# TrevorS/voxtral-mini-realtime-rs

Hardware: AMD Instinct MI355X
Metric: decode_tok_per_s (higher is better)
Workload: dtype f32

## Files before the change

### include/voxtral_hip.h

```cpp
#ifndef VOXTRAL_HIP_H
#define VOXTRAL_HIP_H

#include <stddef.h>
#include <stdint.h>

#ifdef __cplusplus
extern "C" {
#endif

#define VOX_OK 0
#define VOX_ERR_INVALID 1
#define VOX_ERR_IO 2
#define VOX_ERR_HIP 3
#define VOX_ERR_NOTFOUND 4
#define VOX_ERR_UNSUPPORTED 5

#define VOX_MEM_HOST 0
#define VOX_MEM_DEVICE 1

typedef struct vox_ctx vox_ctx;
typedef struct vox_gguf vox_gguf;
typedef struct vox_q4 vox_q4;
typedef struct vox_model vox_model;
typedef struct vox_cache vox_cache;
typedef struct vox_graph vox_graph;

const char* vox_last_error(void);
int32_t vox_abi_version(void);
int32_t vox_device_count(int32_t* n);

int32_t vox_ctx_create(int32_t device, vox_ctx** out);
int32_t vox_ctx_destroy(vox_ctx* ctx);
int32_t vox_ctx_synchronize(vox_ctx* ctx);
int32_t vox_ctx_set_shared(vox_ctx* ctx, int32_t shared);
int32_t vox_ctx_stream(vox_ctx* ctx, void** hip_stream_out);
int32_t vox_dev_alloc(vox_ctx* ctx, size_t nbytes, void** out);
int32_t vox_dev_free(vox_ctx* ctx, void* p);
int32_t vox_dev_upload(vox_ctx* ctx, void* dst_dev, const void* src_host, size_t nbytes);
int32_t vox_dev_download(vox_ctx* ctx, void* dst_host, const void* src_dev, size_t nbytes);
int32_t vox_dev_copy(vox_ctx* ctx, void* dst_dev, const void* src_dev, size_t nbytes);

int32_t vox_resample_len(size_t n_in, uint32_t sr_in, uint32_t sr_out, size_t* n_out);
int32_t vox_resample(vox_ctx* ctx, const float* in, size_t n_in, uint32_t sr_in, uint32_t sr_out, float* out, size_t cap, size_t* n_out,
                     int32_t mem_kind);
int32_t vox_resample_plan(uint32_t sr_in, uint32_t sr_out, int32_t* fft_in, int32_t* fft_out, int32_t* delay, float* cutoff, float* taps_or_null, size_t cap);
int32_t vox_peak_normalize(float* samples, size_t n, float target_peak);

typedef struct {
    uint32_t sample_rate;
    uint32_t n_left_pad_tokens;
    float    frame_rate;
    uint32_t extra_right_pad_tokens;
} vox_pad_cfg;
int32_t vox_pad_cfg_voxtral(vox_pad_cfg* cfg);
int32_t vox_pad_len(size_t n, const vox_pad_cfg* cfg, size_t* out);
int32_t vox_pad_audio(const float* in, size_t n, const vox_pad_cfg* cfg, float* out);
int32_t vox_num_audio_tokens(size_t n, const vox_pad_cfg* cfg, size_t* out);

typedef struct {
    uint32_t max_mel_frames;
    uint32_t hop_length;
    uint32_t sample_rate;
    uint32_t overlap_frames;
} vox_chunk_cfg;
typedef struct { size_t start_sample, end_sample, index; int32_t is_last; } vox_chunk;
int32_t vox_needs_chunking(size_t n, const vox_chunk_cfg* cfg, int32_t* out);
int32_t vox_chunk_plan(size_t n, const vox_chunk_cfg* cfg, vox_chunk* out, size_t cap, size_t* n_chunks);

int32_t vox_mel_num_frames(size_t n_samples, size_t* out);
int32_t vox_mel_filterbank(float* out_128x201);
int32_t vox_hann_window(int32_t length, float* out);
int32_t vox_mel_compute_log(vox_ctx* ctx, const float* samples, size_t n, float* out_Tx128, int32_t mem_kind);

int32_t vox_time_embedding(float t, int32_t dim, float* out);

int32_t vox_gguf_open(const char* path, vox_gguf** out);
int32_t vox_gguf_open_memory(const void* data, size_t size, vox_gguf** out);
int32_t vox_gguf_open_shards(const void* const* shards, const size_t* sizes, int32_t n, vox_gguf** out);
int32_t vox_gguf_close(vox_gguf* g);
int32_t vox_gguf_version(const vox_gguf* g, uint32_t* out);
int32_t vox_gguf_tensor_count(const vox_gguf* g, uint64_t* out);
int32_t vox_gguf_tensor_name(const vox_gguf* g, uint64_t index, const char** out);
int32_t vox_gguf_tensor_info(const vox_gguf* g, const char* name, uint64_t dims[4], uint32_t* ndims,
                             uint32_t* dtype, uint64_t* nbytes);
int32_t vox_gguf_tensor_data(const vox_gguf* g, const char* name, void* dst, size_t cap);

int32_t vox_q4_tensor_from_bytes(vox_ctx* ctx, const uint8_t* raw, size_t nbytes, int64_t N, int64_t K, vox_q4** out);
int32_t vox_q4_tensor_shape(const vox_q4* q, int64_t* N, int64_t* K);
int32_t vox_q4_tensor_num_blocks(const vox_q4* q, int64_t* out);
int32_t vox_q4_tensor_dequantize(vox_ctx* ctx, const vox_q4* q, float* out_NxK);
int32_t vox_q4_tensor_free(vox_q4* q);
int32_t vox_q4_matmul(vox_ctx* ctx, const vox_q4* w, const float* x, int32_t B, int32_t M, float* out, int32_t mem_kind);
int32_t vox_q4_linear_forward(vox_ctx* ctx, const vox_q4* w, const float* bias_or_null, const float* x,
                              int32_t B, int32_t M, float* out, int32_t mem_kind);

int32_t vox_dense_tensor_from_f32(vox_ctx* ctx, const float* w_NxK, const float* w_other_or_null, int64_t N, int64_t K, vox_q4** out);
int32_t vox_linear_forward_ex(vox_ctx* ctx, const vox_q4* w, const float* bias_or_null, const float* x, int32_t B, int32_t M, float* out, int32_t epilogue, int32_t mem_kind);
int32_t vox_conv_downsample(vox_ctx* ctx, const float* x_CxL, int32_t C, int32_t L, const float* w1, const float* b1, const float* w2, const float* b2, int32_t O, float* out_OxL2);

typedef struct {
    int32_t enc_layers, enc_dim, enc_heads, enc_head_dim, enc_ffn, enc_window;
    int32_t dec_layers, dec_dim, dec_heads, dec_kv_heads, dec_head_dim, dec_ffn, dec_window, vocab;
    int32_t n_mels, reshape_factor, t_cond_dim;
    float rope_theta, norm_eps;
} vox_model_cfg;

int32_t vox_attention(vox_ctx* ctx, const float* q, const float* k, const float* v, int32_t M, int32_t kv_len, int32_t n_heads,
                      int32_t n_kv_heads, int32_t head_dim, int32_t offset, int32_t window, float* out, int32_t mem_kind);

int32_t vox_q4_model_load(vox_ctx* ctx, const char* gguf_path, vox_model** out);
#define VOX_LOAD_LAYOUT_ONLY 1u
int32_t vox_q4_model_load_ex(vox_ctx* ctx, const char* gguf_path, uint32_t flags, vox_model** out);
int32_t vox_q4_model_load_gguf(vox_ctx* ctx, vox_gguf* g, uint32_t flags, vox_model** out);
int32_t vox_f32_model_load(vox_ctx* ctx, const char* safetensors_path, vox_model** out);
int32_t vox_model_free(vox_model* m);
int32_t vox_model_config(const vox_model* m, vox_model_cfg* out);
int32_t vox_model_weight_bytes(const vox_model* m, uint64_t* out);
int32_t vox_model_arena(const vox_model* m, void** dev_ptr, uint64_t* nbytes);
int32_t vox_model_arena_finalize(vox_model* m);
int32_t vox_model_replicate(const vox_model* src, vox_ctx* dst_ctx, vox_model** out);
int32_t vox_model_memory(const vox_model* m, uint64_t out[4]);

int32_t vox_model_set_t_embed(vox_model* m, const float* t_embed_host);
int32_t vox_model_set_decode_engine(vox_model* m, int32_t on, int32_t* active_or_null);
int32_t vox_model_set_prefix_cache(vox_model* m, int32_t on, int32_t* active_or_null);
int32_t vox_model_prefix_info(const vox_model* m, int32_t out[4]);
int32_t vox_model_set_batch_engine(vox_model* m, int32_t on, int32_t* active_or_null, uint64_t* launches_or_null);

int32_t vox_encode_audio(vox_model* m, const float* mel_128xT, int32_t T, float* out, int32_t cap_rows,
                         int32_t* S, int32_t mem_kind);
int32_t vox_transcribe_streaming(vox_model* m, const float* mel_128xT, int32_t T, const float* t_embed,
                                 int32_t* out_ids, int32_t cap, int32_t* n_ids, float* logits_or_null,
                                 int32_t mem_kind);
int32_t vox_transcribe_audio(vox_model* m, const float* samples, size_t n, const float* t_embed,
                             int32_t* out_ids, int32_t cap, int32_t* n_ids, int32_t mem_kind);

int32_t vox_transcribe_batch(vox_model* m, int32_t n, const float* const* samples, const size_t* n_samples, const float* t_embed,
                             int32_t* const* out_ids, const int32_t* caps, int32_t* n_ids, int32_t mem_kind);
int32_t vox_transcribe_batch_ex(vox_model* m, int32_t n, const float* const* samples, const size_t* n_samples, const int32_t* norm_group_or_null, const float* t_embed,
                                int32_t* const* out_ids, const int32_t* caps, int32_t* n_ids, int32_t mem_kind);
int32_t vox_model_set_sessions(vox_model* m, int32_t sessions);

int32_t vox_decoder_cache_create(vox_model* m, int32_t max_seq, vox_cache** out);
int32_t vox_cache_free(vox_cache* c);
int32_t vox_cache_seq_len(const vox_cache* c, int32_t* out);
int32_t vox_cache_reset(vox_cache* c);
int32_t vox_cache_update(vox_cache* c, int32_t layer, int32_t pos, const float* k_HxNxhd, const float* v_HxNxhd, int32_t n_rows, int32_t mem_kind);
int32_t vox_cache_truncate(vox_cache* c, int32_t len);
int32_t vox_encoder_cache_create(vox_model* m, int32_t capacity_rows, vox_cache** out);
int32_t vox_encoder_cache_apply_sliding_window(vox_cache* enc_cache, int32_t window);
int32_t vox_cache_abs_pos(const vox_cache* c, int32_t* out);
int32_t vox_encode_audio_with_cache(vox_model* m, const float* mel_128xT, int32_t T, vox_cache* enc_cache, float* out, int32_t cap_rows,
                                    int32_t* S, int32_t mem_kind);
int32_t vox_embed_tokens_from_ids(vox_model* m, const int32_t* ids, int32_t n, float* out_nxD);
int32_t vox_forward_hidden_with_cache(vox_model* m, const float* x_MxD, int32_t M, const float* t_embed,
                                      vox_cache* cache, float* out_MxD);
int32_t vox_lm_head(vox_model* m, const float* hidden_MxD, int32_t M, float* logits_MxV);
int32_t vox_embed_tokens_from_ids_ex(vox_model* m, const int32_t* ids_host, int32_t n, float* out_nxD, int32_t mem_kind);
int32_t vox_tensor_add(vox_ctx* ctx, const float* a, const float* b, size_t n, float* out, int32_t mem_kind);
int32_t vox_forward_hidden_with_cache_ex(vox_model* m, const float* x_MxD, int32_t M, const float* t_embed, vox_cache* cache, float* out_MxD_or_null,
                                         const float** hidden_ws_or_null, int32_t mem_kind);
int32_t vox_lm_head_ex(vox_model* m, const float* hidden_MxD, int32_t M, float* logits_MxV, int32_t mem_kind);
int32_t vox_argmax_rows(vox_ctx* ctx, const float* logits_MxV, int32_t M, int32_t V, int32_t* ids_host, int32_t mem_kind);
int32_t vox_lm_head_argmax(vox_model* m, const float* hidden_MxD, int32_t M, int32_t* ids_host, int32_t mem_kind);
int32_t vox_generate_step_with_cache(vox_model* m, const int32_t* token_ids, int32_t n, const float* t_embed, vox_cache* cache, float* logits_nxV);

int32_t vox_forward(vox_model* m, const float* mel_128xT, int32_t T, const float* t_embed, float* logits_SxV, int32_t cap_rows, int32_t* S, int32_t mem_kind);
int32_t vox_forward_streaming(vox_model* m, const float* mel_128xT, int32_t T, const int32_t* token_ids, int32_t n_ids, const float* t_embed, float* logits_SxV,
                              int32_t cap_rows, int32_t* S, int32_t mem_kind);
int32_t vox_forward_with_cache(vox_model* m, const float* mel_128xT, int32_t T, const float* t_embed, vox_cache* enc_cache, vox_cache* dec_cache, float* logits_SxV,
                               int32_t cap_rows, int32_t* S, int32_t mem_kind);

typedef struct { double preprocess_ms, encode_ms, decode_ms, total_ms; int32_t decode_tokens; int32_t graph_replays; } vox_timings;
int32_t vox_get_stage_timings(const vox_model* m, vox_timings* out);

int32_t vox_debug_reload_knobs(void);
int32_t vox_debug_attn_launches(uint64_t* out, int32_t cap);
int32_t vox_debug_gemm_launches(uint64_t* out, int32_t cap);
int32_t vox_debug_occupy(vox_ctx* ctx, int32_t workgroups, int32_t micros);

int32_t vox_bench_decode_gemv(vox_model* m, int32_t which, int32_t iters, double* avg_us, double* bytes_per_launch,
                              const char** kernel_name);

int32_t vox_bench_wide(vox_model* m, int32_t which, int32_t mt, int32_t iters, double out_us[4]);

int32_t vox_debug_timeline_start(vox_ctx* ctx, int32_t n_slots, int32_t n_waves);
int32_t vox_debug_timeline_fetch(vox_ctx* ctx, uint64_t* out, size_t cap_words, int32_t* slots_used, int32_t* meta );
int32_t vox_debug_batch_tap_arm(vox_model* m, const int32_t* units, int32_t n_units, int32_t max_rows);
int32_t vox_debug_batch_tap_fetch(vox_model* m, float* out, int32_t* rows_per_unit);
int32_t vox_debug_encode_batch(vox_model* m, int32_t n, const float* const* mels, const int32_t* T, int32_t layout, float* out, int64_t cap_rows,
                               int32_t* rows_per_clip, int64_t* report);
int32_t vox_debug_step_costs(const double base[9], const double meas[9], int32_t calib, int32_t shared, double out[9]);
int32_t vox_debug_plan_slots(const int32_t* steps, int32_t n, int32_t force_G, int32_t max_groups, const double step_ms[9], int32_t* G, int32_t* job_slot,
                             int32_t* job_qpos, int32_t steps_g[8], int32_t run_g[8], double* cost_ms);

typedef struct vox_stream vox_stream;
int32_t vox_stream_create(vox_model* m, const float* t_embed, float gain, int32_t enc_capacity_rows, int32_t max_positions, vox_stream** out);
int32_t vox_stream_push(vox_stream* s, const float* samples, size_t n, int32_t mem_kind, int32_t* out_ids, int32_t cap, int32_t* n_ids);
int32_t vox_stream_finish(vox_stream* s, int32_t* out_ids, int32_t cap, int32_t* n_ids);
int32_t vox_stream_reset(vox_stream* s);
int32_t vox_stream_free(vox_stream* s);
int32_t vox_stream_info(const vox_stream* s, int64_t out[8]);
int32_t vox_stream_schedule(size_t n_samples, int32_t finished, int32_t* positions, int32_t* ids);
int32_t vox_debug_stream_tap_arm(vox_stream* s, int32_t max_rows);
int32_t vox_debug_stream_tap_fetch(vox_stream* s, float* out_rows_x_vocab, int32_t* rows);

#ifdef __cplusplus
}
#endif
#endif
```

### voxtral-mini-realtime-rs_amd/_lib.py

```python
from __future__ import annotations

import ctypes as C
import os

from .build import LIB_PATH


class VoxError(RuntimeError):
    def __init__(self, code, msg):
        super().__init__(f"[vox error {code}] {msg}")
        self.code = code


class PadCfg(C.Structure):
    _fields_ = [("sample_rate", C.c_uint32), ("n_left_pad_tokens", C.c_uint32), ("frame_rate", C.c_float),
                ("extra_right_pad_tokens", C.c_uint32)]


class ChunkCfg(C.Structure):
    _fields_ = [("max_mel_frames", C.c_uint32), ("hop_length", C.c_uint32), ("sample_rate", C.c_uint32),
                ("overlap_frames", C.c_uint32)]


class Chunk(C.Structure):
    _fields_ = [("start_sample", C.c_size_t), ("end_sample", C.c_size_t), ("index", C.c_size_t), ("is_last", C.c_int32)]


class ModelCfg(C.Structure):
    _fields_ = [(n, C.c_int32) for n in ("enc_layers", "enc_dim", "enc_heads", "enc_head_dim", "enc_ffn", "enc_window",
                                         "dec_layers", "dec_dim", "dec_heads", "dec_kv_heads", "dec_head_dim", "dec_ffn",
                                         "dec_window", "vocab", "n_mels", "reshape_factor", "t_cond_dim")] + \
               [("rope_theta", C.c_float), ("norm_eps", C.c_float)]


class Timings(C.Structure):
    _fields_ = [("preprocess_ms", C.c_double), ("encode_ms", C.c_double), ("decode_ms", C.c_double), ("total_ms", C.c_double),
                ("decode_tokens", C.c_int32), ("graph_replays", C.c_int32)]


vp, i32, i64, u32, u64, sz, f32 = C.c_void_p, C.c_int32, C.c_int64, C.c_uint32, C.c_uint64, C.c_size_t, C.c_float
P = C.POINTER

SIGNATURES = {
    "vox_last_error": (C.c_char_p, []),
    "vox_abi_version": (i32, []),
    "vox_device_count": (i32, [P(i32)]),
    "vox_ctx_create": (i32, [i32, P(vp)]),
    "vox_ctx_destroy": (i32, [vp]),
    "vox_debug_reload_knobs": (i32, []),
    "vox_ctx_synchronize": (i32, [vp]),
    "vox_ctx_set_shared": (i32, [vp, i32]),
    "vox_ctx_stream": (i32, [vp, P(vp)]),
    "vox_dev_alloc": (i32, [vp, sz, P(vp)]),
    "vox_dev_free": (i32, [vp, vp]),
    "vox_dev_upload": (i32, [vp, vp, vp, sz]),
    "vox_dev_download": (i32, [vp, vp, vp, sz]),
    "vox_dev_copy": (i32, [vp, vp, vp, sz]),
    "vox_peak_normalize": (i32, [vp, sz, f32]),
    "vox_pad_cfg_voxtral": (i32, [P(PadCfg)]),
    "vox_pad_len": (i32, [sz, P(PadCfg), P(sz)]),
    "vox_pad_audio": (i32, [vp, sz, P(PadCfg), vp]),
    "vox_num_audio_tokens": (i32, [sz, P(PadCfg), P(sz)]),
    "vox_needs_chunking": (i32, [sz, P(ChunkCfg), P(i32)]),
    "vox_chunk_plan": (i32, [sz, P(ChunkCfg), P(Chunk), sz, P(sz)]),
    "vox_mel_num_frames": (i32, [sz, P(sz)]),
    "vox_mel_filterbank": (i32, [vp]),
    "vox_hann_window": (i32, [i32, vp]),
    "vox_mel_compute_log": (i32, [vp, vp, sz, vp, i32]),
    "vox_time_embedding": (i32, [f32, i32, vp]),
    "vox_gguf_open": (i32, [C.c_char_p, P(vp)]),
    "vox_gguf_open_memory": (i32, [vp, C.c_size_t, P(vp)]),
    "vox_gguf_open_shards": (i32, [vp, vp, i32, P(vp)]),
    "vox_q4_model_load_gguf": (i32, [vp, vp, C.c_uint32, P(vp)]),
    "vox_gguf_close": (i32, [vp]),
    "vox_gguf_version": (i32, [vp, P(u32)]),
    "vox_gguf_tensor_count": (i32, [vp, P(u64)]),
    "vox_gguf_tensor_name": (i32, [vp, u64, P(C.c_char_p)]),
    "vox_gguf_tensor_info": (i32, [vp, C.c_char_p, P(u64 * 4), P(u32), P(u32), P(u64)]),
    "vox_gguf_tensor_data": (i32, [vp, C.c_char_p, vp, sz]),
    "vox_q4_tensor_from_bytes": (i32, [vp, vp, sz, i64, i64, P(vp)]),
    "vox_q4_tensor_shape": (i32, [vp, P(i64), P(i64)]),
    "vox_q4_tensor_num_blocks": (i32, [vp, P(i64)]),
    "vox_q4_tensor_dequantize": (i32, [vp, vp, vp]),
    "vox_q4_tensor_free": (i32, [vp]),
    "vox_q4_matmul": (i32, [vp, vp, vp, i32, i32, vp, i32]),
    "vox_q4_linear_forward": (i32, [vp, vp, vp, vp, i32, i32, vp, i32]),
    "vox_dense_tensor_from_f32": (i32, [vp, vp, vp, i64, i64, P(vp)]),
    "vox_linear_forward_ex": (i32, [vp, vp, vp, vp, i32, i32, vp, i32, i32]),
    "vox_conv_downsample": (i32, [vp, vp, i32, i32, vp, vp, vp, vp, i32, vp]),
    "vox_attention": (i32, [vp, vp, vp, vp, i32, i32, i32, i32, i32, i32, i32, vp, i32]),
    "vox_q4_model_load": (i32, [vp, C.c_char_p, P(vp)]),
    "vox_q4_model_load_ex": (i32, [vp, C.c_char_p, u32, P(vp)]),
    "vox_f32_model_load": (i32, [vp, C.c_char_p, P(vp)]),
    "vox_model_free": (i32, [vp]),
    "vox_model_config": (i32, [vp, P(ModelCfg)]),
    "vox_model_weight_bytes": (i32, [vp, P(u64)]),
    "vox_model_arena": (i32, [vp, P(vp), P(u64)]),
    "vox_model_set_t_embed": (i32, [vp, vp]),
    "vox_model_set_decode_engine": (i32, [vp, i32, P(i32)]),
    "vox_model_set_prefix_cache": (i32, [vp, i32, P(i32)]),
    "vox_model_prefix_info": (i32, [vp, P(i32 * 4)]),
    "vox_debug_occupy": (i32, [vp, i32, i32]),
    "vox_model_memory": (i32, [vp, P(C.c_uint64)]),
    "vox_model_set_batch_engine": (i32, [vp, i32, P(i32), P(C.c_uint64)]),
    "vox_model_arena_finalize": (i32, [vp]),
    "vox_model_replicate": (i32, [vp, vp, P(vp)]),
    "vox_model_set_sessions": (i32, [vp, i32]),
    "vox_generate_step_with_cache": (i32, [vp, vp, i32, vp, vp, vp]),
    "vox_encode_audio": (i32, [vp, vp, i32, vp, i32, P(i32), i32]),
    "vox_transcribe_streaming": (i32, [vp, vp, i32, vp, vp, i32, P(i32), vp, i32]),
    "vox_transcribe_audio": (i32, [vp, vp, sz, vp, vp, i32, P(i32), i32]),
    "vox_transcribe_batch": (i32, [vp, i32, P(vp), P(sz), vp, P(vp), P(i32), P(i32), i32]),
    "vox_transcribe_batch_ex": (i32, [vp, i32, P(vp), P(sz), vp, vp, P(vp), P(i32), P(i32), i32]),
    "vox_decoder_cache_create": (i32, [vp, i32, P(vp)]),
    "vox_cache_free": (i32, [vp]),
    "vox_cache_seq_len": (i32, [vp, P(i32)]),
    "vox_cache_reset": (i32, [vp]),
    "vox_cache_update": (i32, [vp, i32, i32, vp, vp, i32, i32]),
    "vox_cache_truncate": (i32, [vp, i32]),
    "vox_resample_len": (i32, [sz, C.c_uint32, C.c_uint32, P(sz)]),
    "vox_resample": (i32, [vp, vp, sz, C.c_uint32, C.c_uint32, vp, sz, P(sz), i32]),
    "vox_resample_plan": (i32, [C.c_uint32, C.c_uint32, P(i32), P(i32), P(i32), P(C.c_float), vp, sz]),
    "vox_encoder_cache_create": (i32, [vp, i32, P(vp)]),
    "vox_encoder_cache_apply_sliding_window": (i32, [vp, i32]),
    "vox_cache_abs_pos": (i32, [vp, P(i32)]),
    "vox_encode_audio_with_cache": (i32, [vp, vp, i32, vp, vp, i32, P(i32), i32]),
    "vox_embed_tokens_from_ids": (i32, [vp, vp, i32, vp]),
    "vox_forward_hidden_with_cache": (i32, [vp, vp, i32, vp, vp, vp]),
    "vox_lm_head": (i32, [vp, vp, i32, vp]),
    "vox_embed_tokens_from_ids_ex": (i32, [vp, vp, i32, vp, i32]),
    "vox_tensor_add": (i32, [vp, vp, vp, sz, vp, i32]),
    "vox_forward_hidden_with_cache_ex": (i32, [vp, vp, i32, vp, vp, vp, P(vp), i32]),
    "vox_lm_head_ex": (i32, [vp, vp, i32, vp, i32]),
    "vox_argmax_rows": (i32, [vp, vp, i32, i32, vp, i32]),
    "vox_lm_head_argmax": (i32, [vp, vp, i32, vp, i32]),
    "vox_forward": (i32, [vp, vp, i32, vp, vp, i32, P(i32), i32]),
    "vox_forward_streaming": (i32, [vp, vp, i32, vp, i32, vp, vp, i32, P(i32), i32]),
    "vox_forward_with_cache": (i32, [vp, vp, i32, vp, vp, vp, vp, i32, P(i32), i32]),
    "vox_get_stage_timings": (i32, [vp, P(Timings)]),
    "vox_bench_decode_gemv": (i32, [vp, i32, i32, P(C.c_double), P(C.c_double), P(C.c_char_p)]),
    "vox_bench_wide": (i32, [vp, i32, i32, i32, P(C.c_double)]),
    "vox_debug_attn_launches": (i32, [P(C.c_uint64), i32]),
    "vox_debug_gemm_launches": (i32, [P(C.c_uint64), i32]),
    "vox_debug_timeline_start": (i32, [vp, i32, i32]),
    "vox_debug_timeline_fetch": (i32, [vp, vp, sz, P(i32), vp]),
    "vox_debug_batch_tap_arm": (i32, [vp, P(i32), i32, i32]),
    "vox_debug_batch_tap_fetch": (i32, [vp, vp, P(i32)]),
    "vox_debug_encode_batch": (i32, [vp, i32, P(vp), P(i32), i32, vp, C.c_int64, P(i32), P(C.c_int64)]),
    "vox_stream_create": (i32, [vp, vp, f32, i32, i32, P(vp)]),
    "vox_stream_push": (i32, [vp, vp, sz, i32, vp, i32, P(i32)]),
    "vox_stream_finish": (i32, [vp, vp, i32, P(i32)]),
    "vox_stream_reset": (i32, [vp]),
    "vox_stream_free": (i32, [vp]),
    "vox_stream_info": (i32, [vp, P(i64 * 8)]),
    "vox_debug_step_costs": (i32, [P(C.c_double), P(C.c_double), i32, i32, P(C.c_double)]),
    "vox_debug_plan_slots": (i32, [P(i32), i32, i32, i32, P(C.c_double), P(i32), P(i32), P(i32), P(i32), P(i32), P(C.c_double)]),
    "vox_stream_schedule": (i32, [sz, i32, P(i32), P(i32)]),
    "vox_debug_stream_tap_arm": (i32, [vp, i32]),
    "vox_debug_stream_tap_fetch": (i32, [vp, vp, P(i32)]),
}

_LIB = None
_KNOBS = None


def _knob_env():
    return tuple(sorted((k, v) for k, v in os.environ.items() if k.startswith("VOX_")))


def lib():
    global _LIB, _KNOBS
    if _LIB is not None:
        k = _knob_env()
        if k != _KNOBS:
            _KNOBS = k; _LIB.vox_debug_reload_knobs()
        return _LIB
    if not os.path.exists(LIB_PATH):
        raise VoxError(-1, f"{LIB_PATH} not built: run `python __graft_entry__.py build` (hipcc, gfx950). "
                           "There is no CPU fallback for the HIP path.")
    L = C.CDLL(LIB_PATH)
    for name, (res, args) in SIGNATURES.items():
        fn = getattr(L, name)
        fn.restype = res
        fn.argtypes = args
    _LIB = L; _KNOBS = _knob_env()
    return L


def check(code: int):
    if code != 0:
        raise VoxError(code, (lib().vox_last_error() or b"").decode(errors="replace"))
```

### voxtral-mini-realtime-rs_amd/csrc/vox_api.cpp

```cpp
#include "../../include/voxtral_hip.h"
#include "vox_kernels.h"

#include <dlfcn.h>
#include <fcntl.h>
#include <sys/mman.h>
#include <sys/stat.h>
#include <unistd.h>

#include <algorithm>
#include <chrono>
#include <cmath>
#include <cstdarg>
#include <cstdio>
#include <cstdlib>
#include <cstring>
#include <map>
#include <mutex>
#include <string>
#include <unordered_map>
#include <thread>
#include <vector>

using namespace vox;

// ... 1151 lines not shown
    Loader fillr{m, src, Arena{m->arena, 0}, !layout_only, staging.p, max_q4}; fillr.fmt_cache = &fmt_cache; fillr.ar2 = Arena{m->arena + m->arena_primary_bytes, 0};
    if (!fillr.run(q4)) { std::string e = fillr.err; model_release(m); return fail(VOX_ERR_IO, "%s", e.c_str()); }
    const vox_model_cfg& c = m->cfg;
    const int qdim = c.dec_heads * c.dec_head_dim;
    if (m->tok.w.fmt == WFMT_BF16 || m->tok.w.fmt == WFMT_F32) { m->argmax_R = 2; m->n_parts = dense_gemv_grid(c.vocab); }
    else { m->argmax_R = q4_gemv_default_R(c.vocab, c.dec_dim, EPI_ARGMAX); m->n_parts = m->argmax_R > 0 ? q4_gemv_grid(c.vocab, m->argmax_R) : 1; }
    hipError_t e = hipSuccess;
    auto A = [&](void** p, size_t n) { if (e == hipSuccess) e = hipMalloc(p, n); };
    A((void**)&m->ada_mul, (size_t)c.dec_layers * c.dec_dim * 4); A((void**)&m->d_pos, 64); A((void**)&m->d_h, (size_t)c.dec_dim * 4 * 4);
    A((void**)&m->d_q, (size_t)qdim * 4 * 4); A((void**)&m->d_att, (size_t)qdim * 4 * 4); A((void**)&m->d_act, (size_t)c.dec_ffn * 4 * 4);
    A((void**)&m->d_h2, (size_t)c.dec_dim * 4); A((void**)&m->d_wo_acc, (size_t)c.dec_layers * c.dec_dim * 8);
    A((void**)&m->d_logits, (size_t)c.vocab * 4); A((void**)&m->d_part_val, (size_t)m->n_parts * 4 * 4); A((void**)&m->d_part_idx, (size_t)m->n_parts * 4 * 4);
    if (e != hipSuccess) { model_release(m); return fail(VOX_ERR_HIP, "hipMalloc of decode buffers failed: %s", hipGetErrorString(e)); }
    m->eng_offline.part_val = m->d_part_val; m->eng_offline.part_idx = m->d_part_idx;
    if (hipMemset(m->d_wo_acc, 0, (size_t)c.dec_layers * c.dec_dim * 8) != hipSuccess) { model_release(m); return fail(VOX_ERR_HIP, "hipMemset failed"); }
    for (int i = 0; i < c.dec_layers; i++) m->dec[i].ada_mul = m->ada_mul + (size_t)i * c.dec_dim;
    {
        const char* ev = knob_str("VOX_ENGINE"); bool ok = !(ev && ev[0] == '0') && c.dec_layers <= 32 && eng_geometry_ok(c.dec_dim, c.dec_heads, c.dec_kv_heads, c.dec_head_dim, c.dec_ffn, c.vocab, 256);
        hipDeviceProp_t prop; if (ok && (hipGetDeviceProperties(&prop, ctx->device) != hipSuccess || prop.multiProcessorCount != 256)) ok = false;
        for (int i = 0; ok && i < c.dec_layers; i++) { const DecLayer& L = m->dec[i]; for (const Lin* w : {&L.wqkv, &L.wo, &L.w13, &L.w2}) if (w->w.fmt != WFMT_Q4_0 || !w->w.qs || !w->w.sc || w->bias) ok = false; }
        if (ok && (m->tok.w.fmt != WFMT_Q4_0 || !m->tok.w.qs)) ok = false;
        if (ok) { int occ = 0; if (eng_occupancy(&occ) != hipSuccess || occ < 1) { ok = false; (void)hipGetLastError(); } }
        m->eng_ok = ok; m->eng_on = ok;
        {
            const char* bv = knob_str("VOX_BATCH_ENGINE"); int occ = 0;
            m->engb_ok = ok && !(bv && bv[0] == '0') && engb_occupancy(&occ) == hipSuccess && occ >= 1;
            (void)hipGetLastError();
            if (const char* f = knob_str("VOX_BATCH_ENGINE_FLAGS")) m->engb_flags = atoi(f);
            if (const char* f = knob_str("VOX_BATCH_ENGINE_FLAGS2")) m->engb_flags2 = atoi(f);
        }
        if (const char* f = knob_str("VOX_ENGINE_FLAGS")) m->eng_flags = atoi(f);
        if (const char* f = knob_str("VOX_ENGINE_PACE")) m->eng_pace = atoi(f);
    }
    m->manifest = std::move(rec.seen); m->is_q4 = q4;
    *out = m; return VOX_OK;
}

extern "C" int32_t vox_q4_model_load(vox_ctx* ctx, const char* path, vox_model** out) { return vox_q4_model_load_ex(ctx, path, 0, out); }

extern "C" int32_t vox_q4_model_load_gguf(vox_ctx* ctx, vox_gguf* g, uint32_t flags, vox_model** out) {
    ARGCHK(ctx && g && out, "null argument"); VOXCHK(ctx_bind(ctx));
    GgufSource src; src.g = g;
    const int32_t r = model_build(ctx, &src, true, (flags & VOX_LOAD_LAYOUT_ONLY) != 0, out);
    src.g = nullptr;
    return r;
}
extern "C" int32_t vox_q4_model_load_ex(vox_ctx* ctx, const char* path, uint32_t flags, vox_model** out) {
    ARGCHK(ctx && path && out, "null argument"); VOXCHK(ctx_bind(ctx));
    GgufSource src; VOXCHK(vox_gguf_open(path, &src.g));
    return model_build(ctx, &src, true, (flags & VOX_LOAD_LAYOUT_ONLY) != 0, out);
}

extern "C" int32_t vox_f32_model_load(vox_ctx* ctx, const char* path, vox_model** out) {
    ARGCHK(ctx && path && out, "null argument"); VOXCHK(ctx_bind(ctx));
    SafeTensorsSource src; VOXCHK(src.open(path));
    return model_build(ctx, &src, false, false, out);
}

extern "C" int32_t vox_model_config(const vox_model* m, vox_model_cfg* out) { ARGCHK(m && out, "null argument"); *out = m->cfg; return VOX_OK; }
extern "C" int32_t vox_model_weight_bytes(const vox_model* m, uint64_t* out) { ARGCHK(m && out, "null argument"); *out = m->arena_bytes; return VOX_OK; }
extern "C" int32_t vox_model_memory(const vox_model* m, uint64_t out[4]) {
    ARGCHK(m && out, "null argument");
    out[0] = m->arena_bytes; out[1] = m->arena_primary_bytes;
    out[2] = (m->eng_stream ? eng_stream_bytes(m->cfg.dec_layers, m->cfg.vocab) : 0) + (m->eng_wob ? engb_wo_stream_bytes(m->cfg.dec_layers) : 0);
    out[3] = m->eng_state ? eng_state_bytes() : 0;
    for (int gi = 0; gi < 4; gi++) if (m->engb_state[gi]) out[3] += engb_state_bytes();
    return VOX_OK;
}
extern "C" int32_t vox_model_arena(const vox_model* m, void** p, uint64_t* n) { ARGCHK(m && p && n, "null argument"); *p = m->arena; *n = m->arena_primary_bytes; return VOX_OK; }
extern "C" int32_t vox_model_arena_finalize(vox_model* m) {
    ARGCHK(m, "null argument"); VOXCHK(ctx_bind(m->ctx));
    for (Q4W* w : m->tiled) HIPCHK(launch_q4_tile_build(*w, const_cast<uint4*>(w->qt), const_cast<uint16_t*>(w->st), m->ctx->stream));
    HIPCHK(hipStreamSynchronize(m->ctx->stream));
    m->eng_ready = false; m->eng_offline.cache = nullptr;
    prefix_release(m);
    if (m->eng_wob) { HIPCHK(hipStreamSynchronize(m->ctx->stream)); (void)hipFree(m->eng_wob); m->eng_wob = nullptr; }
    graphs_destroy(m);
    return VOX_OK;
}

extern "C" int32_t vox_model_replicate(const vox_model* src, vox_ctx* dst_ctx, vox_model** out) {
    ARGCHK(src && dst_ctx && out, "null argument");
    if (!src->is_q4 || src->manifest.empty()) return fail(VOX_ERR_UNSUPPORTED, "vox_model_replicate: Q4 (GGUF) models only");
    VOXCHK(ctx_bind(src->ctx)); HIPCHK(hipStreamSynchronize(src->ctx->stream));
    VOXCHK(ctx_bind(dst_ctx));
    ManifestSource ms; ms.m = &src->manifest;
    vox_model* d = nullptr;
    VOXCHK(model_build(dst_ctx, &ms, true, true, &d));
    if (d->arena_primary_bytes != src->arena_primary_bytes || d->arena_bytes != src->arena_bytes) { model_release(d); return fail(VOX_ERR_INVALID, "internal: replica arena layout differs from the source's"); }
    hipError_t e = src->ctx->device == dst_ctx->device ? hipMemcpyAsync(d->arena, src->arena, src->arena_primary_bytes, hipMemcpyDeviceToDevice, dst_ctx->stream)
                                                       : hipMemcpyPeerAsync(d->arena, dst_ctx->device, src->arena, src->ctx->device, src->arena_primary_bytes, dst_ctx->stream);
    if (e == hipSuccess) e = hipStreamSynchronize(dst_ctx->stream);
    if (e != hipSuccess) { model_release(d); return fail(VOX_ERR_HIP, "vox_model_replicate: device copy failed: %s", hipGetErrorString(e)); }
    const int32_t r = vox_model_arena_finalize(d);
    if (r != VOX_OK) { model_release(d); return r; }
    *out = d; return VOX_OK;
}

extern "C" int32_t vox_model_set_t_embed(vox_model* m, const float* t_embed) {
    ARGCHK(m && t_embed, "null argument"); VOXCHK(ctx_bind(m->ctx));
    const vox_model_cfg& c = m->cfg; vox_ctx* cx = m->ctx;
    if (m->t_embed_set && m->t_embed_host.size() == (size_t)c.dec_dim && !std::memcmp(m->t_embed_host.data(), t_embed, (size_t)c.dec_dim * 4)) return VOX_OK;
    DevBuf dt, dh, ones; HIPCHK(dt.alloc((size_t)c.dec_dim * 4)); HIPCHK(dh.alloc((size_t)c.t_cond_dim * 4)); HIPCHK(ones.alloc((size_t)c.dec_dim * 4));
    std::vector<float> one(c.dec_dim, 1.0f);
    HIPCHK(hipMemcpyAsync(dt.p, t_embed, (size_t)c.dec_dim * 4, hipMemcpyHostToDevice, cx->stream));
    HIPCHK(hipMemcpyAsync(ones.p, one.data(), (size_t)c.dec_dim * 4, hipMemcpyHostToDevice, cx->stream));
    for (int i = 0; i < c.dec_layers; i++) {
        VOXCHK(q4_linear_dev(cx, m->dec[i].ada0.w, nullptr, dt.as<float>(), c.dec_dim, 1, dh.as<float>(), c.t_cond_dim, EPI_GELU));
        VOXCHK(q4_linear_dev(cx, m->dec[i].ada2.w, nullptr, dh.as<float>(), c.t_cond_dim, 1, m->dec[i].ada_mul, c.dec_dim, EPI_RESID, ones.as<float>(), c.dec_dim));
    }
    HIPCHK(hipStreamSynchronize(cx->stream));
    m->t_embed_host.assign(t_embed, t_embed + c.dec_dim); m->t_embed_set = true;
    m->pfx.dec_built = false;
    return VOX_OK;
}

static int conv_len(int L) { return (L + 2 - 3) / 2 + 1; }

static int32_t ensure(float** p, size_t* cap, size_t need) {
    if (*cap >= need) return VOX_OK;
    if (*p) HIPCHK(hipFree(*p));
    *p = nullptr; *cap = 0;
    HIPCHK(hipMalloc((void**)p, need * sizeof(float))); *cap = need; return VOX_OK;
}

static int enc_rows(int T) { return conv_len(conv_len(T)); }
static int enc_row_budget(const vox_model* m, const int* T, int n) {
    int mx = 0; for (int i = 0; i < n; i++) mx = std::max(mx, enc_rows(T[i]));
    const int r = m->cfg.reshape_factor; return n == 1 ? mx : (mx + r - 1) / r * r;
}
static size_t conv_scratch_floats(const vox_model* m, int T) {
    const int D = m->cfg.enc_dim, T1 = conv_len(T);
    return std::max((size_t)D * T1, (size_t)(T + 2) * m->cfg.n_mels + (size_t)(T1 + 2) * D) + 64;
}
static int32_t conv_stem_dev(vox_model* m, const float* d_mel, int T, float* c1, float* x) {
    const vox_model_cfg& c = m->cfg; hipStream_t s = m->ctx->stream; const int D = c.enc_dim, T1 = conv_len(T), S = conv_len(T1);
    const bool conv_mfma = m->conv1_g.qs && m->conv2_g.qs && !knob_str("VOX_CONV_VALU");
    if (conv_mfma) {
        const int Cm = c.n_mels;
        float* melT = c1; float* c1T = melT + (size_t)(T + 2) * Cm;
        HIPCHK(hipMemsetAsync(melT, 0, (size_t)Cm * 4, s)); HIPCHK(hipMemsetAsync(melT + (size_t)(T + 1) * Cm, 0, (size_t)Cm * 4, s));
        HIPCHK(hipMemsetAsync(c1T, 0, (size_t)D * 4, s)); HIPCHK(hipMemsetAsync(c1T + (size_t)(T1 + 1) * D, 0, (size_t)D * 4, s));
        HIPCHK(launch_transpose(d_mel, Cm, T, melT + Cm, s));
        { GemmParams g{}; g.w = m->conv1_g; g.x = melT; g.x_stride = 2 * Cm; g.M = T1; g.out = c1T + D; g.out_stride = D; g.bias = m->conv1_b; HIPCHK(launch_dense2_gemm(g, EPI_GELU, s)); }
        { GemmParams g{}; g.w = m->conv2_g; g.x = c1T; g.x_stride = 2 * D; g.M = S; g.out = x; g.out_stride = D; g.bias = m->conv2_b; HIPCHK(launch_dense2_gemm(g, EPI_GELU, s)); }
    } else {
        HIPCHK(launch_conv1d_gelu(d_mel, c.n_mels, T, m->conv1_w, m->conv1_b, D, c1, 0, s));
        HIPCHK(launch_conv1d_gelu(c1, D, T1, m->conv2_w, m->conv2_b, D, x, 1, s));
    }
    return VOX_OK;
}
static int enc_packed_rows_of(const vox_model* m, int T) { const int R = m->cfg.reshape_factor; return std::max((enc_rows(T) + R - 1) / R * R, R * 40); }
static long enc_packed_rows(const vox_model* m, const int* T, int n) { long r = 0; for (int i = 0; i < n; i++) r += enc_packed_rows_of(m, T[i]); return r; }
struct EncForms { long Mtot = 0; int ksp = 0, ksp_wo = 0, fused_rope = 0; };
static int32_t encode_batch_dev(vox_model* m, int n, const float* const* d_mels, const int* T, float* audio_out, int audio_rows, int* S4_out, long* audio_off_out = nullptr,
                                EncForms* forms = nullptr, int prefix_rows = 0) {
    const vox_model_cfg& c = m->cfg; vox_ctx* cx = m->ctx; hipStream_t s = cx->stream;
    const int D = c.enc_dim, H = c.enc_heads, hd = c.enc_head_dim, QD = H * hd, F = c.enc_ffn, R = c.reshape_factor;
    const bool packed = audio_off_out != nullptr;
    ARGCHK(n <= 128, "internal: encoder stack of %d utterances", n);
    const int S_pad = enc_row_budget(m, T, n);
    int T1max = 0; bool any = false;
    std::vector<int> S(n);
    for (int i = 0; i < n; i++) { S[i] = enc_rows(T[i]); S4_out[i] = S[i] / R; T1max = std::max(T1max, conv_len(T[i])); any = any || S4_out[i] > 0; }
    if (!any || S_pad <= 0) return VOX_OK;
    ARGCHK(S_pad <= m->enc_rope_len, "audio too long for the encoder RoPE table (%d > %d positions); chunk it (--max-mel-frames)", S_pad, m->enc_rope_len);
    std::vector<int> roff(n + 1, 0);
    if (packed) for (int i = 0; i < n; i++) roff[i + 1] = roff[i] + enc_packed_rows_of(m, T[i]);
    const int r0 = prefix_rows;
    ARGCHK(r0 == 0 || (n == 1 && !packed && r0 % R == 0 && r0 < S_pad && m->pfx.enc_built && r0 == m->pfx.RC), "internal: encoder prefix of %d rows", r0);
    const int Mfull = packed ? roff[n] : n * S_pad;
    const int Mtot = Mfull - r0, M4 = packed ? Mtot / R : n == 1 ? S4_out[0] - r0 / R : Mtot / R;
    ARGCHK(!m->pfx.capture || (n == 1 && !packed && r0 == 0 && m->pfx.capture_rows <= S_pad), "internal: prefix capture");
    ARGCHK(packed || n == 1 || audio_rows >= S_pad / R, "internal: audio row budget %d < %d", audio_rows, S_pad / R);
    int Tmax = 0; for (int i = 0; i < n; i++) Tmax = std::max(Tmax, T[i]);
    (void)T1max;
    const size_t c1_floats = conv_scratch_floats(m, Tmax);
    int ksp = 0;
    {
        const Q4W& w2 = m->enc[0].w2.w;
        const long wgs = (long)((w2.N + 127) / 128) * ((Mtot + 31) / 32);
        const bool geom_ok = w2.fmt == WFMT_Q4_0 && w2.qt && w2.st && w2.nb % 16 == 0 && Mtot > 48 && D % 4 == 0 && D <= 4096;
        if (geom_ok && wgs < 1024) ksp = 4;
        if (const char* e = knob_str("VOX_ENC_SPLITK")) ksp = geom_ok && atoi(e) > 1 ? std::min(atoi(e), w2.nb / 4) : 0;
        for (int l = 0; ksp && l < c.enc_layers; l++) if (m->enc[l].w2.w.fmt != WFMT_Q4_0 || !m->enc[l].w2.w.qt || m->enc[l].w2.w.nb / 4 < ksp) ksp = 0;
    }
    int ksp_wo = ksp ? 2 : 0;
    if (ksp) { if (const char* e = knob_str("VOX_ENC_SPLITK_WO")) ksp_wo = atoi(e) > 1 ? std::min(atoi(e), ksp) : 0; }
    for (int l = 0; ksp_wo && l < c.enc_layers; l++) if (m->enc[l].wo.w.fmt != WFMT_Q4_0 || !m->enc[l].wo.w.qt || m->enc[l].wo.w.nb / 4 < ksp_wo || m->enc[l].wo.w.nb % 4) ksp_wo = 0;
    const size_t need = c1_floats + (size_t)Mfull * D + (size_t)Mtot * D + (size_t)Mtot * QD * 4 + (size_t)Mtot * F + (size_t)(M4 + 1) * m->ad0.w.N + (size_t)ksp * Mtot * D + 1024;
    VOXCHK(ensure(&m->ws, &m->ws_floats, need));
    if (forms) { forms->Mtot = Mtot; forms->ksp = ksp; forms->ksp_wo = ksp_wo; forms->fused_rope = 0; }
    float* c1 = m->ws; float* x0 = c1 + c1_floats / 64 * 64; float* x = x0 + (size_t)r0 * D; float* xn = x0 + (size_t)Mfull * D; float* qkv = xn + (size_t)Mtot * D;
    float* att = qkv + (size_t)Mtot * QD * 3; float* ffn = att + (size_t)Mtot * QD; float* ah = ffn + (size_t)Mtot * F; float* w2p = ah + (size_t)(M4 + 1) * m->ad0.w.N;
    const int* d_len = nullptr; const int* d_roff = nullptr; const int* d_rpos = nullptr;
    if (n > 1 || packed) {
        HIPCHK(hipMemsetAsync(x, 0, (size_t)Mtot * D * 4, s));
        HIPCHK(hipMemsetAsync(att, 0, (size_t)Mtot * QD * 4, s));
        if (!m->d_seq_len) HIPCHK(hipMalloc((void**)&m->d_seq_len, 128 * sizeof(int)));
        m->h_seq_len.assign(S.begin(), S.end());
        HIPCHK(hipMemcpyAsync(m->d_seq_len, m->h_seq_len.data(), (size_t)n * 4, hipMemcpyHostToDevice, s));
        d_len = m->d_seq_len;
    }
    if (packed) {
        if (!m->d_seq_off) HIPCHK(hipMalloc((void**)&m->d_seq_off, 128 * sizeof(int)));
        if (m->row_pos_cap < (size_t)Mtot) { if (m->d_row_pos) { HIPCHK(hipStreamSynchronize(s)); HIPCHK(hipFree(m->d_row_pos)); } m->d_row_pos = nullptr; m->row_pos_cap = 0;
                                              HIPCHK(hipMalloc((void**)&m->d_row_pos, (size_t)Mtot * sizeof(int))); m->row_pos_cap = (size_t)Mtot; }
        HIPCHK(hipStreamSynchronize(s));
        m->h_seq_off.assign(roff.begin(), roff.begin() + n); m->h_row_pos.resize((size_t)Mtot);
        for (int i = 0; i < n; i++) for (int r = roff[i]; r < roff[i + 1]; r++) m->h_row_pos[(size_t)r] = std::min(r - roff[i], m->enc_rope_len - 1);
        HIPCHK(hipMemcpyAsync(m->d_seq_off, m->h_seq_off.data(), (size_t)n * 4, hipMemcpyHostToDevice, s)); HIPCHK(hipMemcpyAsync(m->d_row_pos, m->h_row_pos.data(), (size_t)Mtot * 4, hipMemcpyHostToDevice, s));
        d_roff = m->d_seq_off; d_rpos = m->d_row_pos;
    }
    for (int i = 0; i < n; i++) {
        if (S[i] <= 0) continue;
        VOXCHK(conv_stem_dev(m, d_mels[i], T[i], c1, x0 + (packed ? (size_t)roff[i] : (size_t)i * S_pad) * D));
    }
    const int seq_rows = packed ? 0 : n > 1 ? S_pad : 0;
    for (int l = 0; l < c.enc_layers; l++) {
        const EncLayer& L = m->enc[l];
        if (ksp && l > 0) HIPCHK(launch_rms_norm_sumk(x, D, Mtot, D, w2p, (size_t)Mtot * D, ksp, L.attn_norm, c.norm_eps, xn, D, s));
        else HIPCHK(launch_rms_norm(x, D, Mtot, D, L.attn_norm, nullptr, c.norm_eps, xn, D, s));
        if (Mtot > 48) {
            GemmParams g{}; g.w = L.wqkv.w; g.x = xn; g.x_stride = D; g.M = Mtot; g.out = qkv; g.out_stride = 3 * QD; g.bias = L.wqkv.bias;
            g.rope_cos = m->enc_cos + (size_t)r0 * (hd / 2); g.rope_sin = m->enc_sin + (size_t)r0 * (hd / 2);
            g.hd = hd; g.n_q = 2 * QD; g.pos = d_rpos; g.rope_seq_rows = seq_rows;
            bool fused = false; HIPCHK(launch_q4_gemm(g, EPI_ROPE_ROWS, s, &fused));
            if (forms && fused) forms->fused_rope++;
        } else {
            VOXCHK(q4_linear_dev(cx, L.wqkv.w, L.wqkv.bias, xn, D, Mtot, qkv, 3 * QD));
            HIPCHK(launch_rope(qkv, Mtot, 3 * QD, 2 * QD, hd, r0, m->enc_cos, m->enc_sin, s, seq_rows, d_rpos));
        }
        if (m->pfx.capture)
            HIPCHK(hipMemcpy2DAsync(m->pfx.capture + (size_t)l * m->pfx.capture_rows * 2 * QD, (size_t)2 * QD * 4, qkv + QD, (size_t)3 * QD * 4, (size_t)2 * QD * 4, (size_t)m->pfx.capture_rows,
                                    hipMemcpyDeviceToDevice, s));
        AttnParams ap{}; ap.q = qkv; ap.q_stride = 3 * QD; ap.k = qkv + QD; ap.v = qkv + 2 * QD; ap.kv_row_stride = 3 * QD; ap.kv_head_stride = hd;
        ap.out = att; ap.out_stride = QD; ap.M = S_pad - r0; ap.kv_len = S_pad; ap.n_heads = H; ap.n_kv_heads = H; ap.offset = r0; ap.window = c.enc_window;
        if (r0) { ap.prefix_k = m->pfx.enc_kv + (size_t)l * r0 * 2 * QD; ap.prefix_v = ap.prefix_k + QD; ap.prefix_len = r0; ap.prefix_row_stride = 2 * QD; ap.prefix_head_stride = hd; }
        ap.seq_len = d_len; ap.q_seq_stride = S_pad * 3 * QD; ap.out_seq_stride = S_pad * QD; ap.kv_seq_stride = (long)S_pad * 3 * QD; ap.seq_row_off = d_roff;
        HIPCHK(launch_attn_prefill(ap, hd, s, n));
        if (ksp_wo) {
            VOXCHK(q4_linear_dev(cx, L.wo.w, L.wo.bias, att, QD, Mtot, w2p, D, EPI_STORE, nullptr, 0, ksp_wo));
            HIPCHK(launch_rms_norm_sumk(x, D, Mtot, D, w2p, (size_t)Mtot * D, ksp_wo, L.ffn_norm, c.norm_eps, xn, D, s));
        } else {
            VOXCHK(q4_linear_dev(cx, L.wo.w, L.wo.bias, att, QD, Mtot, x, D, EPI_RESID, x, D));
            HIPCHK(launch_rms_norm(x, D, Mtot, D, L.ffn_norm, nullptr, c.norm_eps, xn, D, s));
        }
        VOXCHK(q4_linear_dev(cx, L.w13.w, nullptr, xn, D, Mtot, ffn, F, EPI_SWIGLU));
        if (ksp) VOXCHK(q4_linear_dev(cx, L.w2.w, L.w2.bias, ffn, F, Mtot, w2p, D, EPI_STORE, nullptr, 0, ksp));
        else VOXCHK(q4_linear_dev(cx, L.w2.w, L.w2.bias, ffn, F, Mtot, x, D, EPI_RESID, x, D));
    }
    if (ksp && c.enc_layers > 0) HIPCHK(launch_rms_norm_sumk(x, D, Mtot, D, w2p, (size_t)Mtot * D, ksp, m->enc_norm, c.norm_eps, xn, D, s));
    else HIPCHK(launch_rms_norm(x, D, Mtot, D, m->enc_norm, nullptr, c.norm_eps, xn, D, s));
    VOXCHK(q4_linear_dev(cx, m->ad0.w, nullptr, xn, D * R, M4, ah, m->ad0.w.N, EPI_GELU));
    if (packed) { for (int i = 0; i < n; i++) audio_off_out[i] = (long)(roff[i] / R) * c.dec_dim; }
    if (packed || n == 1 || audio_rows * R == S_pad) VOXCHK(q4_linear_dev(cx, m->ad2.w, nullptr, ah, m->ad0.w.N, M4, audio_out + (size_t)(r0 / R) * c.dec_dim, c.dec_dim));
    else for (int i = 0; i < n; i++)
        VOXCHK(q4_linear_dev(cx, m->ad2.w, nullptr, ah + (size_t)i * (S_pad / R) * m->ad0.w.N, m->ad0.w.N, S_pad / R, audio_out + (size_t)i * audio_rows * c.dec_dim, c.dec_dim));
    return VOX_OK;
}
static int32_t encode_dev(vox_model* m, const float* d_mel, int T, int* S4_out, int prefix_rows = 0) {
    const int S4 = enc_rows(T) / m->cfg.reshape_factor;
    if (S4 > 0) { size_t cap = (size_t)m->audio_cap * m->cfg.dec_dim; VOXCHK(ensure(&m->d_audio, &cap, (size_t)S4 * m->cfg.dec_dim)); m->audio_cap = (int)(cap / m->cfg.dec_dim); }
    return encode_batch_dev(m, 1, &d_mel, &T, m->d_audio, S4, S4_out, nullptr, nullptr, prefix_rows);
}

static int32_t cache_alloc(vox_model* m, int max_seq, vox_cache** out) {
    const vox_model_cfg& c = m->cfg;
    ARGCHK(max_seq > 0 && max_seq <= m->dec_rope_len, "max_seq %d out of range (1..%d)", max_seq, m->dec_rope_len);
    vox_cache* k = new vox_cache(); k->m = m; k->ctx = m->ctx; k->max_seq = max_seq;
    const size_t n = (size_t)c.dec_layers * c.dec_kv_heads * max_seq * c.dec_head_dim * 4;
    if (hipMalloc((void**)&k->k, n) != hipSuccess || hipMalloc((void**)&k->v, n) != hipSuccess) { if (k->k) (void)hipFree(k->k); delete k; return fail(VOX_ERR_HIP, "hipMalloc of KV cache failed"); }
    HIPCHK(hipMemsetAsync(k->k, 0, n, m->ctx->stream)); HIPCHK(hipMemsetAsync(k->v, 0, n, m->ctx->stream));
    k->layer_stride = (size_t)c.dec_kv_heads * max_seq * c.dec_head_dim;
    cache_register(k);
    *out = k; return VOX_OK;
}
extern "C" int32_t vox_decoder_cache_create(vox_model* m, int32_t max_seq, vox_cache** out) { ARGCHK(m && out, "null argument"); VOXCHK(ctx_bind(m->ctx)); return cache_alloc(m, max_seq, out); }
extern "C" int32_t vox_cache_free(vox_cache* k) {
    if (!k) return VOX_OK;
    (void)hipSetDevice(k->ctx->device); (void)hipStreamSynchronize(k->ctx->stream);
    cache_release(k); return VOX_OK;
}
static int32_t pw_sync(vox_model* m);
static int32_t cache_settle_pending(vox_cache* kc) {
    vox_model* m = kc->m;
    if (m && m->pw_pend_rows > 0 && m->pw_pend_cache == kc) { VOXCHK(ctx_bind(kc->ctx)); VOXCHK(pw_sync(m)); }
    return VOX_OK;
}
extern "C" int32_t vox_cache_update(vox_cache* kc, int32_t layer, int32_t pos, const float* k, const float* v, int32_t n_rows, int32_t mem_kind) {
    ARGCHK(kc && k && v && n_rows > 0 && pos >= 0, "bad argument"); VOXCHK(ctx_bind(kc->ctx)); VOXCHK(cache_settle_pending(kc));
    const vox_model_cfg& c = kc->m->cfg;
    const int L = kc->kind == 1 ? c.enc_layers : c.dec_layers, H = kc->kind == 1 ? c.enc_heads : c.dec_kv_heads, hd = kc->kind == 1 ? c.enc_head_dim : c.dec_head_dim;
    ARGCHK(layer >= 0 && layer < L, "layer %d out of range (0..%d)", layer, L - 1);
    ARGCHK(pos + n_rows <= kc->max_seq, "KV cache overflow: %d + %d > %d", pos, n_rows, kc->max_seq);
    hipStream_t s = kc->ctx->stream; const hipMemcpyKind kind = mem_kind == VOX_MEM_DEVICE ? hipMemcpyDeviceToDevice : hipMemcpyHostToDevice;
    for (int h = 0; h < H; h++) {
        const size_t dst = (size_t)layer * kc->layer_stride + ((size_t)h * kc->max_seq + pos) * hd, src = (size_t)h * n_rows * hd, nb = (size_t)n_rows * hd * 4;
        HIPCHK(hipMemcpyAsync(kc->k + dst, k + src, nb, kind, s)); HIPCHK(hipMemcpyAsync(kc->v + dst, v + src, nb, kind, s));
    }
    if (mem_kind != VOX_MEM_DEVICE) HIPCHK(hipStreamSynchronize(s));
    kc->len = std::max(kc->len, pos + n_rows);
    return VOX_OK;
}
extern "C" int32_t vox_cache_truncate(vox_cache* kc, int32_t len) {
    ARGCHK(kc, "null cache"); VOXCHK(cache_settle_pending(kc)); ARGCHK(len >= 0 && len <= kc->len, "truncate to %d: the cache holds %d rows", len, kc->len);
    if (kc->kind == 1) kc->abs_pos -= kc->len - len;
    kc->len = len; return VOX_OK;
}
extern "C" int32_t vox_cache_seq_len(const vox_cache* k, int32_t* out) { ARGCHK(k && out, "null argument"); *out = k->len; return VOX_OK; }
extern "C" int32_t vox_cache_reset(vox_cache* k) {
    ARGCHK(k, "null cache");
    (void)cache_settle_pending(k);
    k->len = 0; k->abs_pos = 0; return VOX_OK;
}

extern "C" int32_t vox_encoder_cache_create(vox_model* m, int32_t capacity_rows, vox_cache** out) {
    ARGCHK(m && out, "null argument"); VOXCHK(ctx_bind(m->ctx));
    const vox_model_cfg& c = m->cfg;
    if (capacity_rows <= 0) capacity_rows = 2 * c.enc_window + 512;
    ARGCHK(capacity_rows > c.enc_window, "encoder cache capacity %d must exceed the sliding window (%d)", capacity_rows, c.enc_window);
    vox_cache* k = new vox_cache(); k->m = m; k->ctx = m->ctx; k->max_seq = capacity_rows; k->kind = 1;
    const size_t n = (size_t)c.enc_layers * c.enc_heads * capacity_rows * c.enc_head_dim * 4;
    if (hipMalloc((void**)&k->k, n) != hipSuccess || hipMalloc((void**)&k->v, n) != hipSuccess) { if (k->k) (void)hipFree(k->k); delete k; return fail(VOX_ERR_HIP, "hipMalloc of encoder KV cache failed"); }
    HIPCHK(hipMemsetAsync(k->k, 0, n, m->ctx->stream)); HIPCHK(hipMemsetAsync(k->v, 0, n, m->ctx->stream));
    k->layer_stride = (size_t)c.enc_heads * capacity_rows * c.enc_head_dim;
    cache_register(k);
    *out = k; return VOX_OK;
}
extern "C" int32_t vox_cache_abs_pos(const vox_cache* k, int32_t* out) { ARGCHK(k && out, "null argument"); *out = k->kind == 1 ? k->abs_pos : k->len; return VOX_OK; }

static int32_t enc_cache_evict(vox_model* m, vox_cache* kc, int keep) {
    const vox_model_cfg& c = m->cfg; hipStream_t s = m->ctx->stream;
    if (keep >= kc->len) return VOX_OK;
    const size_t planes = (size_t)c.enc_layers * c.enc_heads, pitch = (size_t)kc->max_seq * c.enc_head_dim * 4, width = (size_t)keep * c.enc_head_dim * 4;
    VOXCHK(ensure(&m->ws, &m->ws_floats, planes * width / 4 + 64));
    for (float* base : {kc->k, kc->v}) {
        const char* src = reinterpret_cast<const char*>(base) + (size_t)(kc->len - keep) * c.enc_head_dim * 4;
        HIPCHK(hipMemcpy2DAsync(m->ws, width, src, pitch, width, planes, hipMemcpyDeviceToDevice, s));
        HIPCHK(hipMemcpy2DAsync(base, pitch, m->ws, width, width, planes, hipMemcpyDeviceToDevice, s));
    }
    kc->len = keep;
    return VOX_OK;
}
extern "C" int32_t vox_encoder_cache_apply_sliding_window(vox_cache* kc, int32_t window) {
    ARGCHK(kc && kc->kind == 1 && window > 0, "bad argument"); VOXCHK(ctx_bind(kc->ctx));
    VOXCHK(enc_cache_evict(kc->m, kc, window)); HIPCHK(hipStreamSynchronize(kc->ctx->stream)); return VOX_OK;
}

static int32_t enc_stream_rope_ensure(vox_model* m) {
    if (m->enc_cos_s) return VOX_OK;
    const vox_model_cfg& c = m->cfg; const int hd = c.enc_head_dim;
    const int len = 1 << 16, half = hd / 2; std::vector<float> ct((size_t)len * half), st((size_t)len * half);
    for (int i = 0; i < len; i++) for (int j = 0; j < half; j++) { const float inv = 1.0f / std::pow(c.rope_theta, (float)(2 * j) / (float)hd), fr = (float)i * inv; ct[(size_t)i * half + j] = std::cos(fr); st[(size_t)i * half + j] = std::sin(fr); }
    HIPCHK(hipMalloc((void**)&m->enc_cos_s, ct.size() * 4)); HIPCHK(hipMalloc((void**)&m->enc_sin_s, st.size() * 4));
    HIPCHK(hipMemcpy(m->enc_cos_s, ct.data(), ct.size() * 4, hipMemcpyHostToDevice)); HIPCHK(hipMemcpy(m->enc_sin_s, st.data(), st.size() * 4, hipMemcpyHostToDevice));
    m->enc_rope_s_len = len;
    return VOX_OK;
}
static int32_t encode_with_cache_dev(vox_model* m, const float* d_mel, int T, vox_cache* kc, int* S4_out) {
    const vox_model_cfg& c = m->cfg; vox_ctx* cx = m->ctx; hipStream_t s = cx->stream;
    const int D = c.enc_dim, H = c.enc_heads, hd = c.enc_head_dim, QD = H * hd, F = c.enc_ffn, R = c.reshape_factor;
    const int S = enc_rows(T), S4 = S / R; *S4_out = S4;
    if (S <= 0) return VOX_OK;
    ARGCHK(S <= kc->max_seq - std::min(c.enc_window, kc->max_seq - 1), "chunk of %d encoder rows does not fit a cache of %d rows next to the %d-row window", S, kc->max_seq, c.enc_window);
    if (kc->len + S > kc->max_seq) VOXCHK(enc_cache_evict(m, kc, std::min(kc->len, c.enc_window)));
    const float *cos_t = m->enc_cos, *sin_t = m->enc_sin;
    if (kc->abs_pos + S > m->enc_rope_len) {
        VOXCHK(enc_stream_rope_ensure(m));
        ARGCHK(kc->abs_pos + S <= m->enc_rope_s_len, "stream of %d encoder positions exceeds the streaming RoPE table (%d)", kc->abs_pos + S, m->enc_rope_s_len);
        cos_t = m->enc_cos_s; sin_t = m->enc_sin_s;
    }
    if (S4 > 0) { size_t cap = (size_t)m->audio_cap * c.dec_dim; VOXCHK(ensure(&m->d_audio, &cap, (size_t)S4 * c.dec_dim)); m->audio_cap = (int)(cap / c.dec_dim); }
    const size_t c1f = conv_scratch_floats(m, T);
    const size_t need = c1f + (size_t)S * D * 2 + (size_t)S * QD * 4 + (size_t)S * F + (size_t)(S4 + 1) * m->ad0.w.N + 1024;
    VOXCHK(ensure(&m->ws, &m->ws_floats, need));
    float* c1 = m->ws; float* x = c1 + c1f / 64 * 64; float* xn = x + (size_t)S * D; float* qkv = xn + (size_t)S * D;
    float* att = qkv + (size_t)S * QD * 3; float* ffn = att + (size_t)S * QD; float* ah = ffn + (size_t)S * F;
    VOXCHK(conv_stem_dev(m, d_mel, T, c1, x));
    const int off = kc->len; const size_t lf = kc->layer_stride;
    for (int l = 0; l < c.enc_layers; l++) {
        const EncLayer& L = m->enc[l]; float* kl = kc->k + (size_t)l * lf; float* vl = kc->v + (size_t)l * lf;
        HIPCHK(launch_rms_norm(x, D, S, D, L.attn_norm, nullptr, c.norm_eps, xn, D, s));
        VOXCHK(q4_linear_dev(cx, L.wqkv.w, L.wqkv.bias, xn, D, S, qkv, 3 * QD));
        HIPCHK(launch_rope(qkv, S, 3 * QD, 2 * QD, hd, kc->abs_pos, cos_t, sin_t, s, 0));
        HIPCHK(launch_kv_store(qkv, S, 3 * QD, QD, H, hd, off, kl, vl, kc->max_seq * hd, s));
        AttnParams ap{}; ap.q = qkv; ap.q_stride = 3 * QD; ap.k = kl; ap.v = vl; ap.kv_row_stride = hd; ap.kv_head_stride = kc->max_seq * hd;
        ap.out = att; ap.out_stride = QD; ap.M = S; ap.kv_len = off + S; ap.n_heads = H; ap.n_kv_heads = H; ap.offset = off; ap.window = c.enc_window;
        HIPCHK(launch_attn_prefill(ap, hd, s, 1));
        VOXCHK(q4_linear_dev(cx, L.wo.w, L.wo.bias, att, QD, S, x, D, EPI_RESID, x, D));
        HIPCHK(launch_rms_norm(x, D, S, D, L.ffn_norm, nullptr, c.norm_eps, xn, D, s));
// ... 1763 lines not shown
                else for (int gi = 0; gi < mt; gi++) { const GemmParams g = params(i, false, gi); HIPCHK(launch_q4_gemm(g, epis[which], s)); }
            }
            HIPCHK(hipEventRecord(e1, s)); HIPCHK(hipEventSynchronize(e1));
            float ms = 0.f; HIPCHK(hipEventElapsedTime(&ms, e0, e1)); *us = (double)ms * 1000.0 / iters;
        }
        return VOX_OK;
    };
    out_us[1] = 0.0;
    VOXCHK(timed(0, &out_us[0])); if (which != 4) VOXCHK(timed(1, &out_us[1])); VOXCHK(timed(2, &out_us[2])); VOXCHK(timed(3, &out_us[3]));
    (void)hipEventDestroy(e0); (void)hipEventDestroy(e1);
    HIPCHK(hipStreamSynchronize(s));
    return VOX_OK;
}

extern "C" int32_t vox_bench_decode_gemv(vox_model* m, int32_t which, int32_t iters, double* avg_us, double* bytes_per_launch, const char** kernel_name) {
    const bool warm = (which & 0x100) != 0;
    which &= 0xff;
    ARGCHK(m && avg_us && bytes_per_launch && iters > 0 && which >= 0 && which <= 5, "bad argument"); VOXCHK(ctx_bind(m->ctx));
    const vox_model_cfg& c = m->cfg; hipStream_t s = m->ctx->stream;
    VOXCHK(ensure_decode_state(m, 64));
    if (which == 5) {
        if (!m->t_embed_set) { std::vector<float> te(c.dec_dim); vox_time_embedding(6.0f, c.dec_dim, te.data()); VOXCHK(vox_model_set_t_embed(m, te.data())); }
        if (!engine_bind(m, m->eng_offline, m->cache)) return fail(VOX_ERR_UNSUPPORTED, "decode engine not active for this model / device");
        static const int bench_pos[4] = {40, 75, 110, 145};
        HIPCHK(hipMemcpyAsync(m->d_pos, &bench_pos[0], 4, hipMemcpyHostToDevice, s));
        HIPCHK(hipMemsetAsync(m->d_h, 0, (size_t)c.dec_dim * 4, s));
        double bytes = 0; for (const Q4W* w : {&m->dec[0].wqkv.w, &m->dec[0].wo.w, &m->dec[0].w13.w, &m->dec[0].w2.w}) bytes += (double)w->N * w->nb * 18.0;
        *bytes_per_launch = bytes * c.dec_layers + (double)m->tok.w.N * m->tok.w.nb * 18.0;
        if (kernel_name) *kernel_name = "decode_engine_kernel";
        const int per_q = std::max(iters / 4, 1);
        VOXCHK(engine_take_serials(m, 4ull * per_q + 3, s));
        const EngParams ep = engine_params(m, m->eng_offline, m->cache, m->d_h, m->d_pos, 0, nullptr);
        for (int i = 0; i < 3; i++) HIPCHK(launch_decode_engine(ep, s));
        hipEvent_t ev[8]; for (auto& e : ev) HIPCHK(hipEventCreate(&e));
        hipGraph_t gq = nullptr; hipGraphExec_t gx = nullptr;
        HIPCHK(hipStreamBeginCapture(s, hipStreamCaptureModeThreadLocal));
        hipError_t ce = hipSuccess; for (int i = 0; i < per_q && ce == hipSuccess; i++) ce = launch_decode_engine(ep, s);
        const hipError_t ee = hipStreamEndCapture(s, &gq);
        if (ce != hipSuccess || ee != hipSuccess || hipGraphInstantiate(&gx, gq, nullptr, nullptr, 0) != hipSuccess) { if (gq) (void)hipGraphDestroy(gq); for (auto& e : ev) (void)hipEventDestroy(e); return fail(VOX_ERR_HIP, "engine timing: graph capture failed"); }
        for (int q = 0; q < 4; q++) {
            const int pq = std::min(bench_pos[q], m->cache->max_seq - 2);
            HIPCHK(hipMemcpyAsync(m->d_pos, &pq, 4, hipMemcpyHostToDevice, s));
            HIPCHK(hipEventRecord(ev[2 * q], s));
            HIPCHK(hipGraphLaunch(gx, s));
            HIPCHK(hipEventRecord(ev[2 * q + 1], s));
        }
        HIPCHK(hipEventSynchronize(ev[7]));
        float ms = 0.f; for (int q = 0; q < 4; q++) { float mq = 0.f; HIPCHK(hipEventElapsedTime(&mq, ev[2 * q], ev[2 * q + 1])); ms += mq; }
        for (auto& e : ev) (void)hipEventDestroy(e);
        (void)hipGraphExecDestroy(gx); (void)hipGraphDestroy(gq);
        iters = 4 * per_q;
        *avg_us = (double)ms * 1000.0 / iters;
        unsigned err2[2] = {0, 0}; HIPCHK(hipMemcpy(err2, ep.err, 8, hipMemcpyDeviceToHost));
        if (err2[0]) return fail(VOX_ERR_HIP, "decode engine: %s", engine_timeout_text(err2[0], 0).c_str());
        return VOX_OK;
    }
    const int zero = 0; HIPCHK(hipMemcpyAsync(m->d_pos, &zero, 4, hipMemcpyHostToDevice, s));
    HIPCHK(hipMemsetAsync(m->d_h, 0, (size_t)c.dec_dim * 4, s)); HIPCHK(hipMemsetAsync(m->d_att, 0, (size_t)c.dec_heads * c.dec_head_dim * 4, s));
    HIPCHK(hipMemsetAsync(m->d_act, 0, (size_t)c.dec_ffn * 4, s));
    if (!m->t_embed_set) { std::vector<float> te(c.dec_dim); vox_time_embedding(6.0f, c.dec_dim, te.data()); VOXCHK(vox_model_set_t_embed(m, te.data())); }
    const int D = c.dec_dim, QD = c.dec_heads * c.dec_head_dim, KD = c.dec_kv_heads * c.dec_head_dim, F = c.dec_ffn, hd = c.dec_head_dim;
    const size_t lf = m->cache->layer_stride;
    bool fused = false;
    { AttnParams ap{}; ap.n_heads = c.dec_heads; ap.n_kv_heads = c.dec_kv_heads; ap.kv_row_stride = hd; ap.kv_head_stride = m->cache->max_seq * hd;
      fused = decode_layer_fuses_attn_wo(m, m->dec[0], ap, m->cache); if (fused) VOXCHK(wo_acc_clear(m, s)); }
    auto launch = [&](int l) -> int32_t {
        if (warm) l = 0;
        const DecLayer& L = m->dec[l % c.dec_layers]; GemvParams p{};
        switch (which) {
        case 0: p.w = L.wqkv.w; p.x = m->d_h; p.x_stride = D; p.out = m->d_q; p.out_stride = QD; p.gamma = L.attn_norm; p.eps = c.norm_eps; p.pos_ptr = m->d_pos;
                p.rope_cos = m->dec_cos; p.rope_sin = m->dec_sin; p.hd = hd; p.n_q = QD; p.n_k = KD; p.kcache = m->cache->k + (size_t)(l % c.dec_layers) * lf;
                p.vcache = m->cache->v + (size_t)(l % c.dec_layers) * lf; p.cache_head_stride = m->cache->max_seq * hd;
                HIPCHK(launch_q4_gemv(p, 1, PRO_RMS, EPI_ROPE_KV, q4_gemv_default_R(p.w.N, p.w.K, EPI_ROPE_KV), s)); break;
        case 1: p.w = L.wo.w; p.x = m->d_att; p.x_stride = QD; p.out = m->d_h; p.out_stride = D; p.resid = m->d_h; p.resid_stride = D;
                HIPCHK(launch_q4_gemv(p, 1, PRO_NONE, EPI_RESID, q4_gemv_default_R(p.w.N, p.w.K, EPI_RESID), s)); break;
        case 2: p.w = L.w13.w; p.x = m->d_h; p.x_stride = D; p.out = m->d_act; p.out_stride = F; p.gamma = L.ffn_norm; p.mul = L.ada_mul; p.eps = c.norm_eps;
                if (fused) { p.xacc = m->d_wo_acc + (size_t)(l % c.dec_layers) * D; p.x_out = m->d_h2; }
                HIPCHK(launch_q4_gemv(p, 1, fused ? PRO_RMS_MUL_SUM : PRO_RMS_MUL, EPI_SWIGLU, q4_gemv_default_R(p.w.N, p.w.K, EPI_SWIGLU), s)); break;
        case 3: p.w = L.w2.w; p.x = m->d_act; p.x_stride = F; p.out = m->d_h; p.out_stride = D; p.resid = m->d_h; p.resid_stride = D;
                HIPCHK(launch_q4_gemv(p, 1, PRO_NONE, EPI_RESID, q4_gemv_default_R(p.w.N, p.w.K, EPI_RESID), s)); break;
        default: VOXCHK(lm_head_argmax_dev(m, m->d_h, nullptr)); break;
        }
        return VOX_OK;
    };
    const Q4W* w = which == 0 ? &m->dec[0].wqkv.w : which == 1 ? &m->dec[0].wo.w : which == 2 ? &m->dec[0].w13.w : which == 3 ? &m->dec[0].w2.w : &m->tok.w;
    *bytes_per_launch = w->fmt == WFMT_BF16 ? (double)w->N * w->K * 2.0 : w->fmt == WFMT_F32 ? (double)w->N * w->K * 4.0 : (double)w->N * w->nb * 18.0;
    if (kernel_name) {
        const int epi = which == 0 ? EPI_ROPE_KV : which == 2 ? EPI_SWIGLU : which == 4 ? EPI_ARGMAX : EPI_RESID;
        const int pro = which == 2 ? (fused ? PRO_RMS_MUL_SUM : PRO_RMS_MUL) : (which == 0 || which == 4) ? PRO_RMS : PRO_NONE;
        if (w->fmt == WFMT_BF16 || w->fmt == WFMT_F32) { static thread_local char nb_[64]; snprintf(nb_, sizeof nb_, "dense_gemv_kernel<PRO=%d,EPI=%d>", pro, epi); *kernel_name = nb_; }
        else *kernel_name = q4_gemv_kernel_name(w->K, pro, epi, which == 4 ? m->argmax_R : q4_gemv_default_R(w->N, w->K, epi));
    }
    for (int i = 0; i < std::min(iters, 8); i++) VOXCHK(launch(i));
    hipEvent_t e0, e1; HIPCHK(hipEventCreate(&e0)); HIPCHK(hipEventCreate(&e1));
    HIPCHK(hipEventRecord(e0, s));
    for (int i = 0; i < iters; i++) VOXCHK(launch(i));
    HIPCHK(hipEventRecord(e1, s)); HIPCHK(hipEventSynchronize(e1));
    float ms = 0.f; HIPCHK(hipEventElapsedTime(&ms, e0, e1));
    (void)hipEventDestroy(e0); (void)hipEventDestroy(e1);
    *avg_us = (double)ms * 1000.0 / iters;
    return VOX_OK;
}

static unsigned long long* g_tl_dev = nullptr; static int g_tl_nslots = 0, g_tl_nwaves = 0;
extern "C" int32_t vox_debug_timeline_start(vox_ctx* c, int32_t n_slots, int32_t n_waves) {
    ARGCHK(c && n_slots > 0 && n_waves > 0, "bad argument"); VOXCHK(ctx_bind(c));
    if (g_tl_dev) { (void)tl_configure(nullptr, 0, 0); (void)hipFree(g_tl_dev); g_tl_dev = nullptr; }
    const size_t bytes = (size_t)n_slots * n_waves * 4 * sizeof(unsigned long long);
    HIPCHK(hipMalloc((void**)&g_tl_dev, bytes)); HIPCHK(hipMemset(g_tl_dev, 0, bytes));
    if (tl_configure(g_tl_dev, n_slots, n_waves) != hipSuccess) { (void)hipFree(g_tl_dev); g_tl_dev = nullptr; return fail(VOX_ERR_UNSUPPORTED, "library built without -DVOX_TIMELINE"); }
    g_tl_nslots = n_slots; g_tl_nwaves = n_waves; return VOX_OK;
}
extern "C" int32_t vox_debug_timeline_fetch(vox_ctx* c, uint64_t* out, size_t cap_words, int32_t* slots_used, int32_t* meta) {
    ARGCHK(c && out && slots_used, "null argument"); VOXCHK(ctx_bind(c));
    if (meta) for (int i = 0; i < g_tl_nslots; i++) tl_slot_meta(i, meta + 4 * i);
    ARGCHK(g_tl_dev, "timeline not started");
    const size_t words = (size_t)g_tl_nslots * g_tl_nwaves * 4;
    ARGCHK(cap_words >= words, "timeline output buffer too small (%zu < %zu words)", cap_words, words);
    HIPCHK(hipDeviceSynchronize());
    HIPCHK(hipMemcpy(out, g_tl_dev, words * 8, hipMemcpyDeviceToHost));
    *slots_used = tl_slots_used();
    (void)tl_configure(nullptr, 0, 0); (void)hipFree(g_tl_dev); g_tl_dev = nullptr;
    return VOX_OK;
}

static void tap_release(vox_model* m) {
    if (m->tap.out || m->tap.rows) (void)hipSetDevice(m->ctx->device);
    if (m->tap.out) (void)hipFree(m->tap.out);
    if (m->tap.rows) (void)hipFree(m->tap.rows);
    m->tap.out = nullptr; m->tap.rows = nullptr; m->tap.armed = m->tap.ready = false;
}
extern "C" int32_t vox_debug_batch_tap_arm(vox_model* m, const int32_t* units, int32_t n_units, int32_t max_rows) {
    ARGCHK(units && n_units > 0 && n_units <= 4096, "bad tap unit list (%d units)", n_units); ARGCHK(max_rows > 0 && max_rows <= 65536, "max_rows %d out of range (1..65536)", max_rows);
    ARGCHK(m, "null model");
    std::vector<int> u(units, units + n_units);
    for (int i = 0; i < n_units; i++) { ARGCHK(u[i] >= 0, "tapped unit %d < 0", u[i]); for (int j = 0; j < i; j++) ARGCHK(u[j] != u[i], "unit %d tapped twice", u[i]); }
    tap_release(m);
    m->tap.units = u; m->tap.max_rows = max_rows; m->tap.armed = true;
    return VOX_OK;
}
extern "C" int32_t vox_debug_batch_tap_fetch(vox_model* m, float* out, int32_t* rows_per_unit) {
    ARGCHK(m && out && rows_per_unit, "null argument");
    if (!m->tap.ready) { tap_release(m); return fail(VOX_ERR_INVALID, "no batch tap to fetch (arm one, then make one successful vox_transcribe_batch call)"); }
    VOXCHK(ctx_bind(m->ctx));
    const size_t nu = m->tap.units.size();
    HIPCHK(hipDeviceSynchronize());
    const hipError_t e1 = hipMemcpy(out, m->tap.out, nu * (size_t)m->tap.max_rows * m->cfg.vocab * 4, hipMemcpyDeviceToHost);
    const hipError_t e2 = hipMemcpy(rows_per_unit, m->tap.rows, nu * 4, hipMemcpyDeviceToHost);
    tap_release(m);
    if (e1 != hipSuccess || e2 != hipSuccess) return fail(VOX_ERR_HIP, "batch tap copy failed");
    return VOX_OK;
}

extern "C" int32_t vox_debug_encode_batch(vox_model* m, int32_t n, const float* const* mels, const int32_t* T, int32_t layout, float* out, int64_t cap_rows,
                                          int32_t* rows_per_clip, int64_t* report) {
    ARGCHK(m, "null model");
    ARGCHK(n > 0 && n <= 128, "encoder stack of %d clips out of range (1..128)", n);
    ARGCHK(layout == 0 || layout == 1, "layout %d: 0 padded, 1 packed", layout);
    ARGCHK(mels && T && out && rows_per_clip && report, "null argument");
    for (int i = 0; i < n; i++) ARGCHK(mels[i] && T[i] > 0, "clip %d: empty mel", i);
    const vox_model_cfg& c = m->cfg; const int R = c.reshape_factor, D = c.dec_dim, PREFIX_LEN = 38;
    const std::vector<int> Ti(T, T + n);
    long need_rows = 0; for (int i = 0; i < n; i++) need_rows += enc_rows(Ti[i]) / R;
    ARGCHK(cap_rows >= need_rows, "output capacity %lld rows < %ld", (long long)cap_rows, need_rows);
    VOXCHK(ctx_bind(m->ctx)); hipStream_t s = m->ctx->stream;
    size_t mel_floats = 0; for (int i = 0; i < n; i++) mel_floats += (size_t)c.n_mels * Ti[i];
    int audio_rows = 0; size_t audio_floats = 0; std::vector<long> off(n, 0);
    if (layout == 0) { audio_rows = std::max(enc_row_budget(m, Ti.data(), n) / R, PREFIX_LEN + 1); audio_floats = (size_t)n * audio_rows * D; for (int i = 0; i < n; i++) off[i] = (long)i * audio_rows * D; }
    else audio_floats = (size_t)(enc_packed_rows(m, Ti.data(), n) / R) * D;
    DevBuf b_mel, b_audio;
    HIPCHK(b_mel.alloc(mel_floats * 4)); HIPCHK(b_audio.alloc(audio_floats * 4));
    HIPCHK(hipMemsetAsync(b_audio.p, 0, audio_floats * 4, s));
    std::vector<const float*> d_mels(n); size_t mo = 0;
    for (int i = 0; i < n; i++) {
        float* d = b_mel.as<float>() + mo; mo += (size_t)c.n_mels * Ti[i];
        HIPCHK(hipMemcpyAsync(d, mels[i], (size_t)c.n_mels * Ti[i] * 4, hipMemcpyHostToDevice, s)); d_mels[i] = d;
    }
    std::vector<int> S4(n, 0); EncForms f;
    VOXCHK(encode_batch_dev(m, n, d_mels.data(), Ti.data(), b_audio.as<float>(), audio_rows, S4.data(), layout == 1 ? off.data() : nullptr, &f));
    HIPCHK(hipStreamSynchronize(s));
    size_t o = 0;
    for (int i = 0; i < n; i++) {
        if (S4[i] > 0) HIPCHK(hipMemcpy(out + o, b_audio.as<float>() + off[i], (size_t)S4[i] * D * 4, hipMemcpyDeviceToHost));
        o += (size_t)S4[i] * D; rows_per_clip[i] = S4[i];
    }
    report[0] = f.Mtot; report[1] = f.ksp; report[2] = f.ksp_wo; report[3] = f.fused_rope;
    return VOX_OK;
}

static const int STREAM_SAMPLE_RING = 1 << 16;
static const int STREAM_KEEP_ROWS = 1024;
struct vox_stream {
    vox_model* m = nullptr; vox_ctx* ctx = nullptr;
    std::vector<float> t_embed; float gain = 1.0f;
    int cap = 0, max_pos = 0, RC = 0, PC = 0; long left = 0;
    float *kring = nullptr, *vring = nullptr; size_t ring_layer = 0;
    vox_cache* dec = nullptr;
    float *samples = nullptr, *audio_keep = nullptr, *ws = nullptr;
    int *tokens = nullptr, *state = nullptr;
    MelTables mel{};
    int64_t n_pushed = 0, n_written = 0;
    int pos = 0, ids_out = 0, verified_pos = 0, verified_tap_rows = 0; bool finished = false, eng_unverified = false;
    uint64_t eng_steps = 0, op_steps = 0, verified_eng_steps = 0, verified_op_steps = 0, bytes = 0;
    EngBinding eng;
    float* tap = nullptr; int tap_max = 0, tap_rows = 0;
    int h_state[STRM_WORDS]; int h_pos_word = 0; std::vector<int32_t> h_prefix;
};

static long stream_spp(int R) { return 640L * R; }
static long stream_positions(long left, int R, int64_t n) { const int64_t a = left + n - 40; return a < 0 ? 0 : (long)(a / stream_spp(R)); }

extern "C" int32_t vox_stream_schedule(size_t n_samples, int32_t finished, int32_t* positions, int32_t* ids) {
    ARGCHK(positions && ids, "null argument"); ARGCHK(n_samples <= ((size_t)1 << 40), "sample count out of range");
    vox_pad_cfg pc; vox_pad_cfg_voxtral(&pc);
    const long left = (long)pad_left(&pc); const int R = 4;
    long P;
    if (finished) { size_t total; VOXCHK(vox_pad_len(n_samples, &pc, &total)); P = (long)(total / (size_t)stream_spp(R)); *ids = (int32_t)std::max(P - VOX_PREFIX_TOKENS, 0L); }
    else { P = stream_positions(left, R, (int64_t)n_samples); *ids = (int32_t)std::max(P - (VOX_PREFIX_TOKENS - 1), 0L); }
    *positions = (int32_t)P;
    return VOX_OK;
}

static int32_t stream_dec_alloc(vox_stream* st, int rows) {
    if (st->dec && st->dec->max_seq == rows) return VOX_OK;
    if (st->dec) { HIPCHK(hipStreamSynchronize(st->ctx->stream)); cache_release(st->dec); }
    return cache_alloc(st->m, rows, &st->dec);
}
static int32_t stream_dec_grow(vox_stream* st) {
    vox_model* m = st->m; const vox_model_cfg& c = m->cfg; hipStream_t s = st->ctx->stream; vox_cache* kc = st->dec;
    const int old = kc->max_seq, rows = std::min(st->max_pos, 2 * old), hd = c.dec_head_dim;
    ARGCHK(rows > old, "internal: decoder cache of %d rows cannot grow", old);
    const size_t planes = (size_t)c.dec_layers * c.dec_kv_heads, nb = planes * rows * hd * 4;
    float *nk = nullptr, *nv = nullptr;
    if (hipMalloc((void**)&nk, nb) != hipSuccess || hipMalloc((void**)&nv, nb) != hipSuccess) { (void)hipGetLastError(); if (nk) (void)hipFree(nk); return fail(VOX_ERR_HIP, "hipMalloc of a %d-row decoder cache failed", rows); }
    HIPCHK(hipMemsetAsync(nk, 0, nb, s)); HIPCHK(hipMemsetAsync(nv, 0, nb, s));
    HIPCHK(hipMemcpy2DAsync(nk, (size_t)rows * hd * 4, kc->k, (size_t)old * hd * 4, (size_t)old * hd * 4, planes, hipMemcpyDeviceToDevice, s));
    HIPCHK(hipMemcpy2DAsync(nv, (size_t)rows * hd * 4, kc->v, (size_t)old * hd * 4, (size_t)old * hd * 4, planes, hipMemcpyDeviceToDevice, s));
    HIPCHK(hipStreamSynchronize(s));
    (void)hipFree(kc->k); (void)hipFree(kc->v);
    cache_unregister(kc); kc->k = nk; kc->v = nv; kc->max_seq = rows; kc->layer_stride = (size_t)c.dec_kv_heads * rows * hd; cache_register(kc);
    return VOX_OK;
}

static int32_t stream_load_initial(vox_stream* st) {
    vox_model* m = st->m; const vox_model_cfg& c = m->cfg; hipStream_t s = st->ctx->stream; PrefixState& P = m->pfx;
    const bool was_on = P.on; P.on = true;
    int32_t r = prefix_build(m, st->t_embed.data());
    if (r == VOX_OK && !(P.enc_built && P.dec_built && P.RC == st->RC && P.PC == st->PC)) r = fail(VOX_ERR_HIP, "the prefix state a stream starts from could not be built");
    auto body = [&]() -> int32_t {
        VOXCHK(stream_dec_alloc(st, std::min(st->max_pos, ENGINE_MAX_ROWS)));
        const int H = c.enc_heads, hd = c.enc_head_dim, PC = st->PC, RC = st->RC;
        HIPCHK(launch_stream_ring_init(P.enc_kv, c.enc_layers, RC, H, hd, st->cap, st->kring, st->vring, s));
        VOXCHK(prefix_rows_into(m, st->dec, s));
        HIPCHK(engine_tab_enqueue(m, st->eng, st->dec));
        st->h_prefix.assign(VOX_PREFIX_TOKENS, VOX_TOK_STREAMING_PAD); st->h_prefix[0] = VOX_TOK_BOS;
        HIPCHK(hipMemcpyAsync(st->tokens, st->h_prefix.data(), st->h_prefix.size() * 4, hipMemcpyHostToDevice, s));
        std::memset(st->h_state, 0, sizeof st->h_state);
        st->h_state[STRM_POS] = PC; st->h_state[STRM_ENC_POS] = RC; st->h_state[STRM_FRAME] = 4 * RC; st->h_state[STRM_HEAD] = RC % st->cap;
        HIPCHK(hipMemcpyAsync(st->state, st->h_state, sizeof st->h_state, hipMemcpyHostToDevice, s));
        HIPCHK(hipStreamSynchronize(s));
        return VOX_OK;
    };
    if (r == VOX_OK) r = body();
    if (!was_on) { (void)hipStreamSynchronize(s); prefix_release(m); P.on = false; }
    if (r != VOX_OK) return r;
    st->n_pushed = st->n_written = 0; st->pos = st->verified_pos = st->PC; st->ids_out = 0; st->finished = false; st->eng_unverified = false;
    st->eng_steps = st->op_steps = st->verified_eng_steps = st->verified_op_steps = 0; st->tap_rows = st->verified_tap_rows = 0;
    return VOX_OK;
}

static void stream_release(vox_stream* st) {
    if (!st) return;
    (void)hipSetDevice(st->ctx->device); (void)hipStreamSynchronize(st->ctx->stream);
    cache_release(st->dec);
    for (void* p : {(void*)st->kring, (void*)st->vring, (void*)st->samples, (void*)st->audio_keep, (void*)st->ws, (void*)st->tokens, (void*)st->state, (void*)st->tap}) if (p) (void)hipFree(p);
    binding_release(st->eng);
    delete st;
}

extern "C" int32_t vox_stream_create(vox_model* m, const float* t_embed, float gain, int32_t enc_capacity_rows, int32_t max_positions, vox_stream** out) {
    ARGCHK(m && t_embed && out, "null argument"); ARGCHK(std::isfinite(gain), "gain is not finite");
    VOXCHK(ctx_bind(m->ctx));
    const vox_model_cfg& c = m->cfg; vox_ctx* cx = m->ctx;
    if (!m->is_q4) return fail(VOX_ERR_UNSUPPORTED, "live streaming sessions serve Q4 (GGUF) models");
    int RC, PC; prefix_bounds(m, &RC, &PC);
    ARGCHK(RC > 0 && c.reshape_factor == 4 && PC == VOX_PREFIX_TOKENS - 1, "this model geometry has no prefix state for a stream to start from");
    if (!m->conv1_g.qs || !m->conv2_g.qs) return fail(VOX_ERR_UNSUPPORTED, "the stream's conv stem runs as im2col GEMMs: 3 n_mels and 3 enc_dim must be multiples of 128");
    ARGCHK(c.enc_window + 1 <= 1024, "encoder window %d exceeds the stream attention's 1023 keys", c.enc_window);
    const int R = c.reshape_factor;
    int cap = enc_capacity_rows; if (cap == 0) cap = (std::max(c.enc_window + 8, RC) + 63) / 64 * 64;
    ARGCHK(cap > c.enc_window + 4 && cap >= RC, "encoder ring capacity %d must exceed the sliding window + 4 (%d)", cap, c.enc_window + 4);
    const int pos_limit = std::min(m->dec_rope_len, (1 << 16) / R);
    int maxp = max_positions; if (maxp == 0) maxp = pos_limit;
    ARGCHK(maxp > VOX_PREFIX_TOKENS && maxp <= pos_limit, "max_positions %d out of range (%d..%d)", maxp, VOX_PREFIX_TOKENS + 1, pos_limit);
    VOXCHK(enc_stream_rope_ensure(m));
    vox_stream* st = new vox_stream(); st->m = m; st->ctx = cx; st->t_embed.assign(t_embed, t_embed + c.dec_dim); st->gain = gain; st->cap = cap; st->max_pos = maxp; st->RC = RC; st->PC = PC;
    { vox_pad_cfg pc; vox_pad_cfg_voxtral(&pc); st->left = (long)pad_left(&pc); }
    const int D = c.enc_dim, QD = c.enc_heads * c.enc_head_dim, F = c.enc_ffn, DD = c.dec_dim;
    st->ring_layer = (size_t)c.enc_heads * cap * c.enc_head_dim;
    const size_t ring_b = (size_t)c.enc_layers * st->ring_layer * 4, keep_b = (size_t)STREAM_KEEP_ROWS * DD * 4;
    const size_t ws_f = (size_t)(4 * R + 3) * c.n_mels + (size_t)(2 * R + 1) * D + (size_t)2 * R * D + (size_t)R * QD * 4 + (size_t)R * F + m->ad0.w.N + (size_t)2 * DD + 256;
    hipError_t e = hipSuccess;
    auto A = [&](void** q, size_t n) { if (e == hipSuccess) { e = hipMalloc(q, n); if (e == hipSuccess) st->bytes += n; } };
    A((void**)&st->kring, ring_b); A((void**)&st->vring, ring_b); A((void**)&st->samples, (size_t)STREAM_SAMPLE_RING * 4); A((void**)&st->audio_keep, keep_b);
    A((void**)&st->ws, ws_f * 4); A((void**)&st->tokens, (size_t)(maxp + 2) * 4); A((void**)&st->state, sizeof(int) * STRM_WORDS);
    if (e == hipSuccess) e = binding_alloc(m, st->eng, &st->bytes);
// ... 195 lines not shown
```

### voxtral-mini-realtime-rs_amd/csrc/vox_kernels.h

```cpp
#pragma once
#include <hip/hip_runtime.h>
#include <atomic>
struct DevOnce {
    std::atomic<uint64_t> mask{0};
    bool done(int dev) const { return (mask.load(std::memory_order_acquire) >> (dev & 63)) & 1ull; }
    void set(int dev) { mask.fetch_or(1ull << (dev & 63), std::memory_order_release); }
};
static inline int vox_current_device() { int d = 0; if (hipGetDevice(&d) != hipSuccess) { (void)hipGetLastError(); d = 0; } return d; }
#include <stdint.h>

namespace vox {

struct Q4W {
    const uint4* qs;
    const uint16_t* sc;
    int N, K, nb;
    int fmt;
    const uint4* qt = nullptr; const uint16_t* st = nullptr;
};
enum WFmt { WFMT_Q4_0 = 0, WFMT_BF16 = 1, WFMT_BF16X2 = 2, WFMT_F32 = 3 };

enum Epi { EPI_STORE = 0, EPI_RESID = 1, EPI_SWIGLU = 2, EPI_ROPE_KV = 3, EPI_ARGMAX = 4, EPI_GELU = 5, EPI_SWIGLU_XF = 6, EPI_RESID_XF = 7,
           EPI_ROPE_ROWS = 8 };
enum Pro { PRO_NONE = 0, PRO_RMS = 1, PRO_RMS_MUL = 2,
           PRO_RMS_MUL_SUM = 3 };

struct GemvParams {
    Q4W w;
    const float* x; int x_stride;
    float* out; int out_stride;
    const float* bias;
    const float* resid; int resid_stride;
    const float* gamma; const float* mul; float eps;
    long long* zero_acc; int zero_n;
    const long long* xacc; float* x_out;
    const int* pos_ptr; int pos_off;
    const float* rope_cos; const float* rope_sin; int hd;
    int n_q, n_k;
    float* kcache; float* vcache; int cache_head_stride;
    float* part_val; int* part_idx;
    int tl_slot;
};
hipError_t launch_q4_gemv(const GemvParams& p, int n_rows_x, int pro, int epi, int R, hipStream_t s);
const char* q4_gemv_kernel_name(int K, int pro, int epi, int R);
int q4_gemv_default_R(int N, int K, int epi);
int q4_gemv_grid(int N, int R);
int q4_gemv_nwv(int K, int epi);
int q4_gemv_grid_k(int N, int K, int R, int epi);
int dense_gemv_grid(int N);

struct GemmParams {
    Q4W w;
    const float* x; int x_stride; int M;
    float* out; int out_stride;
    const float* bias;
    const float* resid; int resid_stride;
    const uint4* xf;
    uint16_t* xf_scratch; size_t xf_scratch_bytes;
    const float* ssq_part; int n_part; float norm_eps;
    uint16_t* xf_out; const float* xf_w; const float* xf_w2; float* ssq_out;
    const int* pos; const float* rope_cos; const float* rope_sin; int hd, n_q, n_kv; float* kc; float* vc; long kv_seq_stride; int kv_head_stride;
    const int* kv_row;
    int tl_slot;
    int ksplit;
    float* kz_scratch; size_t kz_scratch_bytes;
    int rope_seq_rows;
    int wide_mt; long xf_gstride , xf_out_gstride , ssq_part_gstride, ssq_out_gstride ;
    int wide_rows;
};
struct WidePlan { int kz, sps, ntw; };
bool q4_wide_plan(const Q4W& w, int mt, int epi, WidePlan* pl);
size_t q4_wide_planes_bytes(const Q4W& w, int mt, const WidePlan& pl);
hipError_t launch_q4_wide(const GemmParams& p, int epi, hipStream_t s);
hipError_t launch_q4_tile_build(Q4W w, uint4* qt, uint16_t* st, hipStream_t s);
hipError_t launch_q4_gemm(const GemmParams& p, int epi, hipStream_t s, bool* fused_rope = nullptr);
hipError_t launch_dense2_gemm(const GemmParams& p, int epi, hipStream_t s);
hipError_t launch_transpose(const float* in, int R, int C, float* out, hipStream_t s);
int q4_skinny_resid_xf_parts(int N);

hipError_t launch_q4_repack(const uint8_t* raw, uint4* qs, uint16_t* sc, int64_t n_blocks, int nb, int row_mul, int row_add, hipStream_t s);
hipError_t launch_q4_dequant(Q4W w, float* out, hipStream_t s);
hipError_t launch_rms_norm(const float* x, int x_stride, int rows, int dim, const float* gamma, const float* mul,
                           float eps, float* out, int out_stride, hipStream_t s);
hipError_t launch_rms_norm_sumk(float* x, int x_stride, int rows, int dim, const float* part, size_t part_stride, int ksplit, const float* gamma, float eps, float* out, int out_stride, hipStream_t s);
int q4_skinny_mt2_plan(const Q4W& w, int M);
hipError_t launch_xf_rows(const float* x, int x_stride, int M, int K, uint16_t* xf, hipStream_t s);
hipError_t launch_q4_skinny_mt2_planes(const GemmParams& p, int KZ, hipStream_t s);
hipError_t launch_splitk_finish_resid(const float* planes, int KZ, int M, int N, float* x, int x_stride, hipStream_t s);
hipError_t launch_splitk_finish_swiglu_xf(const float* planes, int KZ, int M, int N, const float* bias, uint16_t* xf, hipStream_t s);
hipError_t launch_splitk_finish_rope_kv(const float* planes, int KZ, int M, int N, float* q_out, int q_stride, int n_q, int n_kv, int hd, int pos_off,
                                        const float* cos_t, const float* sin_t, float* kc, float* vc, int head_stride, hipStream_t s);
hipError_t launch_rms_norm_xf_sumk(float* x, int x_stride, int rows, int dim, const float* planes, int kz, const float* gamma, const float* mul, float eps, uint16_t* xf, hipStream_t s);
hipError_t launch_rms_norm_xf(const float* x, int x_stride, int rows, int dim, const float* gamma, const float* mul,
                              float eps, uint16_t* xf, hipStream_t s);
hipError_t launch_rope(float* buf, int M, int stride, int n_rot, int hd, int pos_off, const float* cos_t,
                       const float* sin_t, hipStream_t s, int seq_rows = 0, const int* row_pos = nullptr);
hipError_t launch_kv_store(const float* buf, int M, int stride, int k_col, int n_kv, int hd, int pos_off,
                           float* kcache, float* vcache, int cache_head_stride, hipStream_t s, int seq_rows = 0, long kv_seq_stride = 0);

struct AttnParams {
    const float* q; int q_stride;
    const float* k; const float* v;
    int kv_row_stride, kv_head_stride;
    float* out; int out_stride;
    int M, kv_len, n_heads, n_kv_heads, offset, window;
    const int* pos_ptr;
    int pos_per_seq; int q_seq_stride, out_seq_stride; long kv_seq_stride;
    const int* kv_row;
    const int* seq_len;
    const int* seq_row_off;
    uint16_t* out_xf_tiles; long out_xf_tile_stride;
    uint16_t* out_xf;
    long out_xf_gstride;
    int prefer_gqa;
    int no_xcd_remap;
    int tl_slot;
    int spec_zero;
    int spec_rows;
    const float* prefix_k; const float* prefix_v; int prefix_len, prefix_row_stride, prefix_head_stride;
};
hipError_t launch_attn_prefill(const AttnParams& p, int hd, hipStream_t s, int n_seq = 1);
bool attn_prefill_prefix_ok(const AttnParams& p, int hd, int n_seq);
bool attn_prefill_small_ok(const AttnParams& p, int hd, int n_seq);
hipError_t launch_attn_decode(const AttnParams& p, int hd, int max_seq, hipStream_t s, int n_seq = 1);
bool attn_wo_supported(const AttnParams& p, const Q4W& wo, int hd, int max_seq);
hipError_t launch_attn_wo(const AttnParams& p, const Q4W& wo, long long* acc, int max_seq, hipStream_t s);
enum AttnForm { ATTN_FORM_PREFILL_SMALL, ATTN_FORM_PREFILL_MFMA, ATTN_FORM_PREFILL_F32, ATTN_FORM_DECODE, ATTN_FORM_DECODE_SPEC, ATTN_FORM_DECODE_GQA, ATTN_FORM_WO,
                ATTN_FORM_ENGINE, ATTN_FORM_STREAM_RING, ATTN_FORM_COUNT };
void attn_form_note(AttnForm f);
void attn_form_counts(unsigned long long out[ATTN_FORM_COUNT]);
enum GemmForm { GEMM_FORM_GEMV_R1, GEMM_FORM_GEMV_R2, GEMM_FORM_GEMV_R4, GEMM_FORM_DENSE_GEMV, GEMM_FORM_SKINNY, GEMM_FORM_SKINNY_MT, GEMM_FORM_SKINNY_MT2, GEMM_FORM_XF_ROWS,
                GEMM_FORM_SPLITK_FINISH, GEMM_FORM_TILE_11, GEMM_FORM_TILE_12, GEMM_FORM_TILE_21, GEMM_FORM_TILE_22, GEMM_FORM_TILE_21_TB, GEMM_FORM_TILE_22_TB, GEMM_FORM_K32,
                GEMM_FORM_BIG, GEMM_FORM_BIG_ROPE, GEMM_FORM_DENSE2, GEMM_FORM_WIDE, GEMM_FORM_COUNT };
void gemm_form_counts(unsigned long long out[GEMM_FORM_COUNT]);

hipError_t launch_conv1d_gelu(const float* in, int Cin, int L, const float* w, const float* b, int Cout, float* out,
                              int out_token_major, hipStream_t s);

struct MelTables { const float* window; const float* cos_t; const float* sin_t; const float* fb; const int* fb_lo; const int* fb_hi; };
hipError_t launch_mel(const float* audio, long n, long left, long right, const float* scale_ptr, MelTables t,
                      float* out, int T, int transposed, hipStream_t s);
hipError_t launch_resample_matrix(const double* H, int new_len, int fft_in, int fft_out, float* At, hipStream_t s);
hipError_t launch_resample(const float* x, long n_in, const float* At, int fft_in, int fft_out, int delay, float* out, long n_out, hipStream_t s);
hipError_t launch_absmax(const float* x, long n, float target_peak, float* scale_out, hipStream_t s);
hipError_t launch_absmax_group(const float* x, long n, unsigned* group_max_cell, hipStream_t s);
hipError_t launch_group_scale(const unsigned* group_max, const int* unit_group, int n, float target, float* unit_scale, hipStream_t s);

hipError_t launch_embed(Q4W tok, const int* ids, int n, const float* audio, int D, const int* pos_ptr, int id_off,
                        int a_off, float* out, hipStream_t s);
hipError_t launch_argmax_final(const float* part_val, const int* part_idx, int n_parts, int* tokens, int* pos_ptr,
                               int tok_off, int inc, hipStream_t s);
hipError_t launch_argmax_embed(const float* part_val, const int* part_idx, int n_parts, int* tokens, int* pos_ptr, Q4W tok,
                               const float* audio, int D, float* h, hipStream_t s);
hipError_t launch_rope_kv_batch(float* qkv, int n, int stride, int n_q, int n_kv, int hd, const int* pos, const float* cos_t, const float* sin_t,
                                float* kcache, float* vcache, long seq_stride, int head_stride, hipStream_t s);
hipError_t launch_argmax_embed_batch(const float* logits, int n, int vocab, int* tokens, int tok_stride, int* pos, const int* seq_len, Q4W tok,
                                     const float* audio, long audio_seq_stride, int D, float* h, hipStream_t s,
                                     uint16_t* xf = nullptr, const float* xf_w = nullptr, float* ssq_out = nullptr,
                                     long xf_group_stride = 0, int ssq_group_stride = 0,
                                     const long* audio_off = nullptr);
struct SlotStepParams {
    const float* logits; int vocab;
    int* tokens; int tok_stride; const int* clip_len;
    int* slot_clip; int* slot_qpos; const int* queue; int q_stride;
    int* pos; int* kv_row; int n_clips; int first_pos;
    Q4W tok; const float* audio; const long* audio_off; int D;
    const float* h0;
    float* h;
    uint16_t* xf; const float* xf_w; float* ssq_out; long xf_group_stride; int ssq_group_stride;
    int init;
};
hipError_t launch_argmax_embed_slots(const SlotStepParams& p, int n_slots, hipStream_t s);
struct BatchTapParams {
    const float* logits; int vocab;
    const int* slot_clip; int clip0; const int* pos; const int* seq_len;
    const int* clip_unit; int n_clips;
    float* out; int* rows; int n_units, max_rows, first_pos;
};
hipError_t launch_batch_tap(const BatchTapParams& p, int n_rows, hipStream_t s);
hipError_t launch_occupy(int workgroups, int micros, hipStream_t s);
hipError_t launch_add_rows(const float* a, const float* b, float* out, long n, hipStream_t s);
hipError_t launch_gelu(float* x, long n, hipStream_t s);
hipError_t launch_argmax_rows(const float* x, int rows, int V, int* out, hipStream_t s);

struct EngLayerTab { const float* attn_norm; const float* ffn_norm; const float* ada_mul; float* kc; float* vc; };
struct EngParams {
    const unsigned char* stream; size_t cu_stride;
    const EngLayerTab* layers; int n_layers;
    const float* h_in;
    const float* final_norm;
    const int* pos_ptr; int pos_off;
    const float* rope_cos; const float* rope_sin;
    int max_seq, window; float eps;
    unsigned long long *H0, *H1, *G, *PW, *A, *P2;
    unsigned long long *SS0, *SS1;
    unsigned long long* XC;
    unsigned* serial; unsigned* err;
    float* part_val; int* part_idx;
    int* tokens; int* pos_rw; const uint4* tok_qs; const uint16_t* tok_sc; int tok_nb; const float* audio;
    float* logits_out;
    int vocab;
    unsigned long long* tl; int tl_layer;
    int flags;
    int ag_delay_ticks;
    int pace_ticks;
};
bool eng_geometry_ok(int D, int n_heads, int n_kv, int hd, int ffn, int vocab, int max_seq);
size_t eng_stream_bytes(int n_layers, int vocab);
size_t eng_state_bytes();
hipError_t launch_eng_pack(const Q4W& w, int op, int layer, int n_layers, unsigned char* stream, int vocab, hipStream_t s);
void eng_state_carve(unsigned char* state, EngParams* p);
hipError_t launch_decode_engine(const EngParams& p, hipStream_t s);
hipError_t launch_eng_hidden(const EngParams& p, float* out, hipStream_t s);
hipError_t eng_occupancy(int* blocks_per_cu);
int eng_lds_bytes();

struct EngBParams {
    const unsigned char* stream;
    const unsigned char* stream_wo;
    const EngLayerTab* layers; int n_layers;
    long kv_seq_stride;
    const float* h_in; int h_stride; int n_rows;
    const float* final_norm;
    const int* pos;
    const int* kv_row;
    const float* rope_cos; const float* rope_sin;
    int max_seq, window; float eps;
    unsigned char *XH0, *XH1;
    float *SS0, *SS1;
    unsigned long long* G;
    unsigned char* XO;
    float* PW;
    unsigned char* XA;
    float* P2;
    unsigned *F0, *F1, *FO, *FW, *FA, *F2;
    unsigned long long* XC; unsigned* serial; unsigned* err;
    uint16_t* xf_out; float* ssq_out;
    unsigned long long* tl; int tl_layer;
    int flags;
};
size_t engb_state_bytes();
size_t engb_wo_stream_bytes(int n_layers);
void engb_state_carve(unsigned char* state, EngBParams* p);
hipError_t engb_state_init(unsigned char* state, hipStream_t s);
hipError_t launch_decode_engine_b16(const EngBParams& p, hipStream_t s);
hipError_t launch_decode_engine_b16x2(const EngBParams& a, const EngBParams& b, hipStream_t s);
hipError_t engb_occupancy(int* blocks_per_cu);
hipError_t engb_prepare_kernels();
hipError_t launch_engb_ssq_fold(const float* ssq256, float* ssq16, hipStream_t s);
int engb_lds_bytes();
int engb_lds_bytes2();

void knobs_load_once();
void knobs_reload();
#define VOX_NO_PK_F32 __attribute__((target("no-packed-fp32-ops")))
const char* knob_str(const char* name);

hipError_t tl_configure(unsigned long long* buf, int n_slots, int n_waves);
int tl_slots_used();
void tl_slot_meta(int slot, int out[4]);

enum StreamWord { STRM_POS = 0,
                  STRM_ENC_POS = 1,
                  STRM_FRAME = 2,
                  STRM_HEAD = 3,
                  STRM_TICKS = 4,
                  STRM_WORDS = 16 };
hipError_t launch_stream_mel(const float* ring, int ring_mask, long left, float gain, MelTables t, const int* state, int halo_back, int n_frames, float* out, hipStream_t s);
struct StreamAttnParams {
    const float* qkv; int qkv_stride;
    float* kring; float* vring; int cap;
    const float* cos_t; const float* sin_t;
    const int* state;
    float* out; int out_stride;
    int M, n_heads, window;
};
hipError_t launch_stream_attn(const StreamAttnParams& p, int hd, hipStream_t s);
hipError_t launch_stream_ring_init(const float* kv, int layers, int rows, int n_heads, int hd, int cap, float* kring, float* vring, hipStream_t s);
hipError_t launch_stream_embed(Q4W tok, const int* tokens, const float* audio_row, float* audio_keep, int keep_rows, int D, const int* state, float* h, hipStream_t s);
hipError_t launch_stream_embed_kept(Q4W tok, const int* tokens, const float* audio_keep, int keep_rows, int D, const int* state, float* h, hipStream_t s);
hipError_t launch_stream_advance(const float* part_val, const int* part_idx, int n_parts, int* tokens, int* state, int enc_rows, int frames, int cap, hipStream_t s);

}
```

### voxtral-mini-realtime-rs_amd/csrc/vox_kernels.hip

```cpp
#include "vox_kernels.h"

#include <hip/hip_fp16.h>

#include <unistd.h>

#include <algorithm>
#include <atomic>
#include <cstdio>
#include <cstdlib>
#include <cstring>
#include <string>
#include <mutex>
#include <unordered_map>

namespace vox {

static int g_tl_next = -1, g_tl_slots = 0;
#ifdef VOX_TIMELINE
__device__ unsigned long long* g_tl_buf = nullptr;
__device__ int g_tl_waves = 0;
__device__ __forceinline__ void tl_stamp(int slot, int wave_global, int k) {
    if (slot >= 0 && (wave_global & 3) == 0 && (threadIdx.x & 63) == 0 && g_tl_buf && wave_global < g_tl_waves)
        g_tl_buf[((size_t)slot * g_tl_waves + wave_global) * 4 + k] = wall_clock64();
}
// ... 2026 lines not shown
        const float bias = (p.bias && nok) ? p.bias[n] : 0.f;
#pragma unroll
        for (int i = 0; i < 4; i++)
#pragma unroll
            for (int r = 0; r < 4; r++) {
                const int m = m0 + i * 16 + 4 * g + r;
                float v = acc[t][i][r] + bias;
                if (EPI == EPI_SWIGLU) {
                    const float other = dpp_mov<0xB1>(v);
                    if (m < M && nok && !(n & 1)) p.out[(size_t)m * p.out_stride + (n >> 1)] = silu_f(v) * other;
                } else {
                    if (EPI == EPI_GELU) v = gelu_f(v);
                    if (EPI == EPI_RESID && m < M && nok) v = v + p.resid[(size_t)m * p.resid_stride + n];
                    if (m < M && nok) p.out[(size_t)m * p.out_stride + n] = v;
                }
            }
    }
}
hipError_t launch_dense2_gemm(const GemmParams& p, int epi, hipStream_t s) {
    if (p.w.fmt != WFMT_BF16X2 || p.w.K % 32 || (p.x_stride % 4) || p.M <= 0) return hipErrorInvalidValue;
    if (p.w.K % 128) {
        dim3 tgrid((p.w.N + 63) / 64, (p.M + 63) / 64);
        switch (epi) {
#define VOX_D2T(E_) case E_: gemm_form_note(GEMM_FORM_DENSE2); dense2_gemm_kernel<1, E_, true><<<tgrid, dim3(256), (size_t)2 * 4 * 4 * 64 * sizeof(uint4), s>>>(p); break;
        VOX_D2T(EPI_STORE) VOX_D2T(EPI_GELU) VOX_D2T(EPI_RESID) VOX_D2T(EPI_SWIGLU) default: return hipErrorInvalidValue;
#undef VOX_D2T
        }
        return hipGetLastError();
    }
    const long wg2 = (long)((p.w.N + 127) / 128) * ((p.M + 63) / 64);
    const size_t lds = (size_t)2 * 4 * 4 * 64 * sizeof(uint4);
    const bool wide = wg2 >= 400;
    dim3 grid(wide ? (p.w.N + 127) / 128 : (p.w.N + 63) / 64, (p.M + 63) / 64);
#define VOX_D2(E_) case E_: gemm_form_note(GEMM_FORM_DENSE2); if (wide) dense2_gemm_kernel<2, E_><<<grid, dim3(256), lds, s>>>(p); else dense2_gemm_kernel<1, E_><<<grid, dim3(256), lds, s>>>(p); break;
    switch (epi) { VOX_D2(EPI_STORE) VOX_D2(EPI_GELU) VOX_D2(EPI_RESID) VOX_D2(EPI_SWIGLU) default: return hipErrorInvalidValue; }
#undef VOX_D2
    return hipGetLastError();
}
__global__ void transpose_kernel(const float* __restrict__ in, int R, int C, float* __restrict__ out) {
    __shared__ float tile[32][33];
    const int c0 = blockIdx.x * 32, r0 = blockIdx.y * 32, tx = threadIdx.x & 31, ty = threadIdx.x >> 5;
    for (int k = ty; k < 32; k += 8) { const int r = r0 + k, c = c0 + tx; tile[k][tx] = (r < R && c < C) ? in[(size_t)r * C + c] : 0.f; }
    __syncthreads();
    for (int k = ty; k < 32; k += 8) { const int c = c0 + k, r = r0 + tx; if (c < C && r < R) out[(size_t)c * R + r] = tile[tx][k]; }
}
hipError_t launch_transpose(const float* in, int R, int C, float* out, hipStream_t s) {
    transpose_kernel<<<dim3((C + 31) / 32, (R + 31) / 32), dim3(256), 0, s>>>(in, R, C, out);
    return hipGetLastError();
}

template <int NTW, int TILED>
static hipError_t skinny_launch_n(const GemmParams& p, int epi, int ks, hipStream_t s) {
    dim3 grid((p.w.N + 16 * NTW - 1) / (16 * NTW));
    const size_t lds = (size_t)ks * NTW * 64 * 4 * sizeof(float);
    if (p.xf) {
        if (!TILED) return hipErrorInvalidValue;
        const bool pro = p.ssq_part != nullptr;
        if (pro && (p.n_part < 1 || p.n_part > 12 * (64 * ks / 16))) return hipErrorInvalidValue;
        const int nq = p.w.nb / 4, per = nq % ks == 0 ? nq / ks : 0;
        if (per) {
#define VOX_ST(N_, E_, P_, S_) if (NTW == N_ && epi == E_ && (int)pro == P_ && per == S_) { \
            if (E_ == EPI_RESID_XF && (!p.xf_out || !p.xf_w || !p.ssq_out)) return hipErrorInvalidValue; \
            q4_skinny_kernel<N_, E_, 1, 1, P_, S_><<<grid, dim3(64 * ks), lds, s>>>(p); return hipGetLastError(); }
            VOX_ST(2, EPI_ROPE_KV, 1, 3) VOX_ST(2, EPI_SWIGLU_XF, 1, 6) VOX_ST(1, EPI_SWIGLU_XF, 1, 6) VOX_ST(1, EPI_RESID_XF, 0, 4) VOX_ST(4, EPI_SWIGLU_XF, 1, 6) VOX_ST(1, EPI_RESID_XF, 0, 9) VOX_ST(4, EPI_STORE, 1, 6)
#undef VOX_ST
        }
        if (epi == EPI_RESID_XF) {
            if (NTW != 1 || pro || !p.xf_out || !p.xf_w || !p.ssq_out) return hipErrorInvalidValue;
            q4_skinny_kernel<1, EPI_RESID_XF, 1, 1, 0><<<grid, dim3(64 * ks), lds, s>>>(p);
        } else if (pro) {
            switch (epi) {
            case EPI_STORE: q4_skinny_kernel<NTW, EPI_STORE, 1, 1, 1><<<grid, dim3(64 * ks), lds, s>>>(p); break;
            case EPI_ROPE_KV: q4_skinny_kernel<NTW, EPI_ROPE_KV, 1, 1, 1><<<grid, dim3(64 * ks), lds, s>>>(p); break;
            case EPI_SWIGLU_XF: q4_skinny_kernel<NTW, EPI_SWIGLU_XF, 1, 1, 1><<<grid, dim3(64 * ks), lds, s>>>(p); break;
            default: return hipErrorInvalidValue;
            }
        } else {
            switch (epi) {
            case EPI_STORE: q4_skinny_kernel<NTW, EPI_STORE, 1, 1, 0><<<grid, dim3(64 * ks), lds, s>>>(p); break;
            case EPI_RESID: q4_skinny_kernel<NTW, EPI_RESID, 1, 1, 0><<<grid, dim3(64 * ks), lds, s>>>(p); break;
            case EPI_SWIGLU_XF: q4_skinny_kernel<NTW, EPI_SWIGLU_XF, 1, 1, 0><<<grid, dim3(64 * ks), lds, s>>>(p); break;
            default: return hipErrorInvalidValue;
            }
        }
        return hipGetLastError();
    }
    switch (epi) {
    case EPI_STORE: q4_skinny_kernel<NTW, EPI_STORE, TILED, 0, 0><<<grid, dim3(64 * ks), lds, s>>>(p); break;
    case EPI_RESID: q4_skinny_kernel<NTW, EPI_RESID, TILED, 0, 0><<<grid, dim3(64 * ks), lds, s>>>(p); break;
    case EPI_GELU: q4_skinny_kernel<NTW, EPI_GELU, TILED, 0, 0><<<grid, dim3(64 * ks), lds, s>>>(p); break;
    case EPI_SWIGLU: q4_skinny_kernel<NTW, EPI_SWIGLU, TILED, 0, 0><<<grid, dim3(64 * ks), lds, s>>>(p); break;
    default: return hipErrorInvalidValue;
    }
    return hipGetLastError();
}
int q4_skinny_resid_xf_parts(int N) { return (N + 15) / 16; }
static hipError_t launch_q4_skinny(const GemmParams& p_in, int epi, hipStream_t s) {
    GemmParams p = p_in; p.tl_slot = tl_take_slot(2, epi, p.w.N, p.w.K);
    const int nq = p.w.nb / 4, tiles = (p.w.N + 15) / 16;
    int ntw = tiles >= 4 * 192 ? 4 : (tiles >= 2 * 192 ? 2 : 1);
    int ks = nq >= 4 ? 4 : (nq >= 2 ? 2 : 1);
    if (tiles / ntw < 256 && nq >= 16) ks = 8;
    if (epi == EPI_RESID_XF) ntw = 1;
    const bool tiled = p.w.qt && p.w.st;
    hipError_t e;
    if (ntw == 4) e = tiled ? skinny_launch_n<4, 1>(p, epi, ks, s) : skinny_launch_n<4, 0>(p, epi, ks, s);
    else if (ntw == 2) e = tiled ? skinny_launch_n<2, 1>(p, epi, ks, s) : skinny_launch_n<2, 0>(p, epi, ks, s);
    else e = tiled ? skinny_launch_n<1, 1>(p, epi, ks, s) : skinny_launch_n<1, 0>(p, epi, ks, s);
    if (e == hipSuccess) gemm_form_note(GEMM_FORM_SKINNY);
    return e;
}

template <int MT, int NT, int FMT, int TB = 0>
static hipError_t gemm_launch_mn(const GemmParams& p, int epi, hipStream_t s) {
    if (p.ksplit > 1 && (epi != EPI_STORE || p.ksplit > p.w.nb / 4)) return hipErrorInvalidValue;
    dim3 grid((p.w.N + 64 * NT - 1) / (64 * NT), (p.M + 16 * MT - 1) / (16 * MT), p.ksplit > 1 ? p.ksplit : 1);
    const size_t lds = (size_t)2 * 2 * 4 * MT * 64 * sizeof(uint4);
#define VOX_E(E_) case E_: { auto kern = q4_gemm_kernel<MT, NT, E_, FMT, TB>; static DevOnce done;      \
        hipError_t e = ensure_dyn_lds(kern, lds, &done); if (e != hipSuccess) return e;                       \
        gemm_form_note(TB ? (NT == 2 ? GEMM_FORM_TILE_22_TB : GEMM_FORM_TILE_21_TB) : MT == 1 ? (NT == 2 ? GEMM_FORM_TILE_12 : GEMM_FORM_TILE_11) : (NT == 2 ? GEMM_FORM_TILE_22 : GEMM_FORM_TILE_21)); \
        kern<<<grid, dim3(256), lds, s>>>(p); break; }
    switch (epi) { VOX_E(EPI_STORE) VOX_E(EPI_RESID) VOX_E(EPI_GELU) VOX_E(EPI_SWIGLU) default: return hipErrorInvalidValue; }
#undef VOX_E
    return hipGetLastError();
}
template <int FMT>
static hipError_t gemm_launch_f(const GemmParams& p, int epi, hipStream_t s) {
    if (p.w.nb % 4) {
        dim3 grid((p.w.N + 63) / 64, (p.M + 63) / 64);
        if (epi != EPI_STORE && epi != EPI_RESID && epi != EPI_GELU && epi != EPI_SWIGLU) return hipErrorInvalidValue;
        gemm_form_note(GEMM_FORM_K32);
        switch (epi) {
        case EPI_STORE: q4_gemm_k32_kernel<EPI_STORE, FMT><<<grid, dim3(256), 0, s>>>(p); break;
        case EPI_RESID: q4_gemm_k32_kernel<EPI_RESID, FMT><<<grid, dim3(256), 0, s>>>(p); break;
        case EPI_GELU: q4_gemm_k32_kernel<EPI_GELU, FMT><<<grid, dim3(256), 0, s>>>(p); break;
        case EPI_SWIGLU: q4_gemm_k32_kernel<EPI_SWIGLU, FMT><<<grid, dim3(256), 0, s>>>(p); break;
        default: return hipErrorInvalidValue;
        }
        return hipGetLastError();
    }
    const int mt = p.M <= 48 ? 1 : 2;
    int nt = 2;
    auto wgs = [&](int mt_, int nt_) { return (long)((p.w.N + 64 * nt_ - 1) / (64 * nt_)) * ((p.M + 16 * mt_ - 1) / (16 * mt_)); };
    if (wgs(mt, 2) < 256) nt = 1;
    if (FMT == WFMT_Q4_0 && p.w.qt && p.w.st && mt == 2) {
        if (wgs(2, 2) >= 128) nt = 2;
        return nt == 2 ? gemm_launch_mn<2, 2, WFMT_Q4_0, 1>(p, epi, s) : gemm_launch_mn<2, 1, WFMT_Q4_0, 1>(p, epi, s);
    }
#define VOX_MN(M_, N_) if (mt == M_ && nt == N_) return gemm_launch_mn<M_, N_, FMT>(p, epi, s)
    VOX_MN(1, 1); VOX_MN(1, 2); VOX_MN(2, 1); VOX_MN(2, 2);
#undef VOX_MN
    return hipErrorInvalidValue;
}
hipError_t launch_rope(float* buf, int M, int stride, int n_rot, int hd, int pos_off, const float* cos_t, const float* sin_t, hipStream_t s, int seq_rows, const int* row_pos);
static hipError_t launch_q4_gemm_epi(const GemmParams& p, int epi, hipStream_t s, bool* fused_rope);
hipError_t launch_q4_gemm(const GemmParams& p, int epi, hipStream_t s, bool* fused_rope) {
    if (fused_rope) *fused_rope = false;
    if (epi != EPI_ROPE_ROWS) return launch_q4_gemm_epi(p, epi, s, nullptr);
    if (!p.rope_cos || !p.rope_sin || p.hd <= 0 || p.n_q <= 0 || p.n_q > p.w.N || p.n_q % 2) return hipErrorInvalidValue;
    bool fused = false;
    hipError_t e = launch_q4_gemm_epi(p, EPI_ROPE_ROWS, s, &fused);
    if (fused_rope) *fused_rope = fused;
    if (e != hipSuccess || fused) return e;
    return launch_rope(p.out, p.M, p.out_stride, p.n_q, p.hd, 0, p.rope_cos, p.rope_sin, s, p.rope_seq_rows, p.pos);
}
static hipError_t launch_q4_gemm_epi(const GemmParams& p, int epi_in, hipStream_t s, bool* fused_rope) {
    int epi = epi_in == EPI_ROPE_ROWS ? EPI_STORE : epi_in;
    if (p.w.K % 32 || p.M <= 0) return hipErrorInvalidValue;
    if (p.ksplit > 1 && (p.M <= 48 || p.xf || p.w.nb % 4 || p.w.fmt == WFMT_F32)) return hipErrorInvalidValue;
    if (p.w.fmt == WFMT_F32) {
        if (p.xf) return hipErrorInvalidValue;
        GemmParams v = p; v.w.fmt = WFMT_BF16X2; v.w.qt = nullptr; v.w.st = nullptr;
        return launch_dense2_gemm(v, epi, s);
    }
    if (p.xf && p.M > 16) return (p.M <= 48 && p.w.fmt == WFMT_Q4_0 && p.w.nb % 4 == 0 && p.w.qt && p.w.st && (epi == EPI_STORE || epi == EPI_RESID || epi == EPI_GELU || epi == EPI_SWIGLU))
                                     ? launch_q4_skinny_mt(p, epi, s) : hipErrorInvalidValue;
    if (p.xf) return (p.M <= 16 && p.w.fmt == WFMT_Q4_0 && p.w.nb % 4 == 0 && p.w.qt) ? launch_q4_skinny(p, epi, s) : hipErrorInvalidValue;
    if (p.M <= 16 && p.w.fmt == WFMT_Q4_0 && p.w.nb % 4 == 0 && !env_int("VOX_NO_SKINNY")) return launch_q4_skinny(p, epi, s);
    if (p.M > 16 && p.M <= 48 && p.w.fmt == WFMT_Q4_0 && p.w.qt && p.w.st && p.w.nb % 4 == 0 && (p.x_stride % 4) == 0 && (epi == EPI_STORE || epi == EPI_RESID || epi == EPI_GELU || epi == EPI_SWIGLU) &&
        !env_int("VOX_NO_SKINNY_MT")) {
        return launch_q4_skinny_mt(p, epi, s);
    }
    if (p.w.fmt == WFMT_Q4_0 && p.w.qt && p.w.st && p.w.nb % 4 == 0 && (p.x_stride % 4) == 0) {
        const int big = env_int("VOX_GEMM_BIG");
        const long wg14 = (long)((p.w.N + 255) / 256) * ((p.M + 63) / 64);
        const int big_min = 200;
        const bool fits32 = ((size_t)(p.M - 1) * p.x_stride + (size_t)p.w.K) * 4 < 0xFFFFFFF0ull && (size_t)((p.w.N + 15) / 16) * (p.w.nb / 4) * 1024 < 0xFFFFFFF0ull;
        if (p.ksplit <= 1 && fits32 && p.w.N % 256 == 0 && (big == 1 || (big == 0 && wg14 >= big_min))) {
            if (epi_in == EPI_ROPE_ROWS && wg14 >= 1024 && (p.hd & (p.hd - 1)) == 0 && !knob_str("VOX_NO_ROPE_FUSE")) { if (fused_rope) *fused_rope = true; return gemm_big_launch<1, 4>(p, EPI_ROPE_ROWS, s); }
            return gemm_big_launch<1, 4>(p, epi, s);
        }
    }
    return p.w.fmt == WFMT_BF16 ? gemm_launch_f<WFMT_BF16>(p, epi, s) : gemm_launch_f<WFMT_Q4_0>(p, epi, s);
}

__global__ __launch_bounds__(256) void rms_norm_kernel(const float* __restrict__ x, int x_stride, int rows, int dim,
                                                       const float* __restrict__ gamma, const float* __restrict__ mul,
                                                       float eps, float* __restrict__ out, int out_stride) {
    const int row = min(blockIdx.x * 4 + (threadIdx.x >> 6), rows - 1), lane = threadIdx.x & 63;
    const float4* xr = reinterpret_cast<const float4*>(x + (size_t)row * x_stride);
    const int n4 = dim >> 2;
    float4 v[16];
    float ss = 0.f;
#pragma unroll
    for (int i = 0; i < 16; i++) {
        const int c = lane + 64 * i;
        v[i] = xr[min(c, n4 - 1)];
        if (c < n4) ss += (v[i].x * v[i].x + v[i].y * v[i].y) + (v[i].z * v[i].z + v[i].w * v[i].w);
    }
    for (int c = lane + 1024; c < n4; c += 64) { const float4 t = xr[c]; ss += (t.x * t.x + t.y * t.y) + (t.z * t.z + t.w * t.w); }
    ss = wave_sum(ss);
    const float rms = sqrtf(ss / (float)dim + eps);
    float4* o = reinterpret_cast<float4*>(out + (size_t)row * out_stride);
    const float4* g4 = reinterpret_cast<const float4*>(gamma);
    const float4* m4 = reinterpret_cast<const float4*>(mul);
#define VOX_RMS_OUT(T_, C_)                                                                                     \
    { float4 t = (T_); const float4 gm = g4[C_];                                                                \
      t.x = (t.x / rms) * gm.x; t.y = (t.y / rms) * gm.y; t.z = (t.z / rms) * gm.z; t.w = (t.w / rms) * gm.w;   \
      if (mul) { const float4 mm = m4[C_]; t.x *= mm.x; t.y *= mm.y; t.z *= mm.z; t.w *= mm.w; }               \
      o[C_] = t; }
#pragma unroll
    for (int i = 0; i < 16; i++) {
        const int c = lane + 64 * i;
        if (c < n4) VOX_RMS_OUT(v[i], c)
    }
    for (int c = lane + 1024; c < n4; c += 64) VOX_RMS_OUT(xr[c], c)
#undef VOX_RMS_OUT
}
__global__ __launch_bounds__(256) void rms_norm_row_kernel(const float* __restrict__ x, int x_stride, int dim, const float* __restrict__ gamma,
                                                           const float* __restrict__ mul, float eps, float* __restrict__ out, int out_stride,
                                                           uint16_t* __restrict__ xf, const float* __restrict__ planes = nullptr, size_t plane_stride = 0, int kz = 0,
                                                           float* __restrict__ x_rw = nullptr) {
    __shared__ float red[4];
    const int row = blockIdx.x, tid = threadIdx.x, n4 = dim >> 2;
    const float4* xr = reinterpret_cast<const float4*>(x + (size_t)row * x_stride);
    float4 v[10]; float ss = 0.f;
#pragma unroll
    for (int i = 0; i < 10; i++) {
        const int c = tid + 256 * i;
        v[i] = xr[min(c, n4 - 1)];
        if (planes && c < n4) {
            plane_sum_add(v[i], reinterpret_cast<const float4*>(planes + (size_t)row * dim) + c, plane_stride >> 2, kz);
            reinterpret_cast<float4*>(x_rw + (size_t)row * x_stride)[c] = v[i];
        }
        if (c < n4) ss += (v[i].x * v[i].x + v[i].y * v[i].y) + (v[i].z * v[i].z + v[i].w * v[i].w);
    }
    ss = wave_sum(ss);
    if ((tid & 63) == 0) red[tid >> 6] = ss;
    __syncthreads();
    const float rms = sqrtf(((red[0] + red[1]) + (red[2] + red[3])) / (float)dim + eps);
    float4* o = reinterpret_cast<float4*>(out + (size_t)row * out_stride);
    const float4* g4 = reinterpret_cast<const float4*>(gamma);
    const float4* m4 = reinterpret_cast<const float4*>(mul);
#pragma unroll
    for (int i = 0; i < 10; i++) {
        const int c = tid + 256 * i;
        if (c < n4) {
            float4 t = v[i]; const float4 gm = g4[c];
            t.x = (t.x / rms) * gm.x; t.y = (t.y / rms) * gm.y; t.z = (t.z / rms) * gm.z; t.w = (t.w / rms) * gm.w;
            if (mul) { const float4 mm = m4[c]; t.x *= mm.x; t.y *= mm.y; t.z *= mm.z; t.w *= mm.w; }
            if (xf) xf_store4(xf + (size_t)(row >> 4) * ((size_t)2 * (dim >> 7) * 256 * 8), dim, row & 15, 4 * c, t); else o[c] = t;
        }
    }
}
__global__ __launch_bounds__(256) VOX_NO_PK_F32 void rms_norm_sumk_kernel(float* __restrict__ x, int x_stride, int rows, int dim, const float* __restrict__ part, size_t part_stride, int ks,
                                                            const float* __restrict__ gamma, float eps, float* __restrict__ out, int out_stride) {
    const int row = blockIdx.x * 4 + (threadIdx.x >> 6), lane = threadIdx.x & 63;
    if (row >= rows) return;
    float4* xr = reinterpret_cast<float4*>(x + (size_t)row * x_stride);
    const int n4 = dim >> 2;
    float4 v[16];
    float ss = 0.f;
#pragma unroll
    for (int i = 0; i < 16; i++) {
        const int c = lane + 64 * i;
        if (c < n4) {
            float4 a = xr[c];
            plane_sum_add(a, reinterpret_cast<const float4*>(part + (size_t)row * dim) + c, part_stride >> 2, ks);
            v[i] = a; xr[c] = a;
            ss += (a.x * a.x + a.y * a.y) + (a.z * a.z + a.w * a.w);
        } else v[i] = make_float4(0.f, 0.f, 0.f, 0.f);
    }
    ss = wave_sum(ss);
    const float rms = sqrtf(ss / (float)dim + eps);
    float4* o = reinterpret_cast<float4*>(out + (size_t)row * out_stride);
    const float4* g4 = reinterpret_cast<const float4*>(gamma);
#pragma unroll
    for (int i = 0; i < 16; i++) {
        const int c = lane + 64 * i;
        if (c < n4) { const float4 g = g4[c]; o[c] = make_float4((v[i].x / rms) * g.x, (v[i].y / rms) * g.y, (v[i].z / rms) * g.z, (v[i].w / rms) * g.w); }
    }
}
hipError_t launch_rms_norm_sumk(float* x, int x_stride, int rows, int dim, const float* part, size_t part_stride, int ksplit, const float* gamma, float eps, float* out, int out_stride, hipStream_t s) {
    if (dim % 4 || dim > 4096 || rows <= 0 || ksplit < 1) return hipErrorInvalidValue;
    rms_norm_sumk_kernel<<<dim3((rows + 3) / 4), dim3(256), 0, s>>>(x, x_stride, rows, dim, part, part_stride, ksplit, gamma, eps, out, out_stride);
    return hipGetLastError();
}
hipError_t launch_rms_norm_xf_sumk(float* x, int x_stride, int rows, int dim, const float* planes, int kz, const float* gamma, const float* mul, float eps,
                                   uint16_t* xf, hipStream_t s) {
    if (rows > 48 || dim > 10240 || dim % 128 || kz < 1 || !planes) return hipErrorInvalidValue;
    rms_norm_row_kernel<<<dim3(rows), dim3(256), 0, s>>>(x, x_stride, dim, gamma, mul, eps, nullptr, 0, xf, planes, (size_t)rows * dim, kz, x);
    return hipGetLastError();
}
hipError_t launch_rms_norm_xf(const float* x, int x_stride, int rows, int dim, const float* gamma, const float* mul, float eps,
                              uint16_t* xf, hipStream_t s) {
    if (rows > 48 || dim > 10240 || dim % 128) return hipErrorInvalidValue;
    rms_norm_row_kernel<<<dim3(rows), dim3(256), 0, s>>>(x, x_stride, dim, gamma, mul, eps, nullptr, 0, xf);
    return hipGetLastError();
}
hipError_t launch_rms_norm(const float* x, int x_stride, int rows, int dim, const float* gamma, const float* mul, float eps,
                           float* out, int out_stride, hipStream_t s) {
    if (rows <= 64 && dim <= 10240 && dim >= 1024)
        rms_norm_row_kernel<<<dim3(rows), dim3(256), 0, s>>>(x, x_stride, dim, gamma, mul, eps, out, out_stride, nullptr);
    else
        rms_norm_kernel<<<dim3((rows + 3) / 4), dim3(256), 0, s>>>(x, x_stride, rows, dim, gamma, mul, eps, out, out_stride);
    return hipGetLastError();
}

__global__ VOX_NO_PK_F32 void rope_kernel(float* __restrict__ buf, int M, int stride, int n_rot, int hd, int pos_off,
                            const float* __restrict__ cos_t, const float* __restrict__ sin_t, int seq_rows, const int* __restrict__ row_pos) {
    const int half_cols = n_rot >> 1;
    const long total = (long)M * half_cols;
    for (long i = (long)blockIdx.x * blockDim.x + threadIdx.x; i < total; i += (long)gridDim.x * blockDim.x) {
        const int m = (int)(i / half_cols), pc = (int)(i % half_cols);
        const int col = pc * 2, j = (col % hd) >> 1;
        const size_t ti = (size_t)(pos_off + (row_pos ? row_pos[m] : seq_rows > 0 ? m % seq_rows : m)) * (hd >> 1) + j;
        const float c = cos_t[ti], sn = sin_t[ti];
        float* p = buf + (size_t)m * stride + col;
        const float xr = p[0], xi = p[1];
        p[0] = xr * c - xi * sn; p[1] = xr * sn + xi * c;
    }
}
hipError_t launch_rope(float* buf, int M, int stride, int n_rot, int hd, int pos_off, const float* cos_t, const float* sin_t,
                       hipStream_t s, int seq_rows, const int* row_pos) {
    const long total = (long)M * (n_rot / 2);
    int blocks = (int)((total + 255) / 256); if (blocks > 2048) blocks = 2048; if (blocks < 1) blocks = 1;
    rope_kernel<<<dim3(blocks), dim3(256), 0, s>>>(buf, M, stride, n_rot, hd, pos_off, cos_t, sin_t, seq_rows, row_pos);
    return hipGetLastError();
}

__global__ void kv_store_kernel(const float* __restrict__ buf, int M, int stride, int k_col, int n_kv, int hd, int pos_off,
                                float* __restrict__ kc, float* __restrict__ vc, int head_stride, int seq_rows, long kv_seq_stride) {
    const int w = n_kv * hd;
    const long total = (long)M * w;
    for (long i = (long)blockIdx.x * blockDim.x + threadIdx.x; i < total; i += (long)gridDim.x * blockDim.x) {
        const int m = (int)(i / w), c = (int)(i % w), h = c / hd, d = c % hd;
        const int sq = seq_rows > 0 ? m / seq_rows : 0, mm = seq_rows > 0 ? m % seq_rows : m;
        const size_t dst = (size_t)sq * kv_seq_stride + (size_t)h * head_stride + (size_t)(pos_off + mm) * hd + d;
        kc[dst] = buf[(size_t)m * stride + k_col + c];
        vc[dst] = buf[(size_t)m * stride + k_col + w + c];
    }
}
hipError_t launch_kv_store(const float* buf, int M, int stride, int k_col, int n_kv, int hd, int pos_off, float* kc, float* vc,
                           int head_stride, hipStream_t s, int seq_rows, long kv_seq_stride) {
    const long total = (long)M * n_kv * hd;
    int blocks = (int)((total + 255) / 256); if (blocks > 2048) blocks = 2048; if (blocks < 1) blocks = 1;
    kv_store_kernel<<<dim3(blocks), dim3(256), 0, s>>>(buf, M, stride, k_col, n_kv, hd, pos_off, kc, vc, head_stride, seq_rows, kv_seq_stride);
    return hipGetLastError();
}

template <int HD>
__global__ __launch_bounds__(256) void attn_prefill_kernel(const AttnParams p) {
    constexpr int DP = HD / 4;
    extern __shared__ __attribute__((aligned(16))) float smem[];
    float* Ks = smem;
    float* Vs = smem + 64 * HD;
    const int tid = threadIdx.x, lane = tid & 63, wave = tid >> 6;
    const int h = blockIdx.y, kvh = h / (p.n_heads / p.n_kv_heads);
    const int m0 = blockIdx.x * 64;
    const int qi = lane & 15, part = lane >> 4;
    const int m = m0 + wave * 16 + qi;
    const bool q_ok = m < p.M;
    const int pos = p.offset + (q_ok ? m : (p.M - 1));
    const float scale = 1.0f / sqrtf((float)HD);

    float qv[DP], o[DP];
    {
        const float* qp = p.q + (size_t)(q_ok ? m : 0) * p.q_stride + h * HD + part * DP;
#pragma unroll
        for (int e = 0; e < DP; e += 4) {
            const float4 v = *reinterpret_cast<const float4*>(qp + e);
            qv[e] = v.x; qv[e + 1] = v.y; qv[e + 2] = v.z; qv[e + 3] = v.w;
        }
#pragma unroll
        for (int e = 0; e < DP; e++) o[e] = 0.f;
    }
    float mx = -INFINITY, l = 0.f;

    const int last_m = min(m0 + 63, p.M - 1);
    int j_lo = 0;
    if (p.window >= 0) j_lo = max(0, p.offset + m0 - p.window);
    const int j_hi = min(p.kv_len - 1, p.offset + last_m);
    const float* kbase = p.k + (size_t)kvh * p.kv_head_stride;
    const float* vbase = p.v + (size_t)kvh * p.kv_head_stride;

    for (int j0 = (j_lo / 64) * 64; j0 <= j_hi; j0 += 64) {
        __syncthreads();
        for (int i = tid; i < 64 * (HD / 4); i += 256) {
            const int jj = i / (HD / 4), d4 = i % (HD / 4), j = j0 + jj;
            const int jc = min(j, p.kv_len - 1);
            float4 kk = *reinterpret_cast<const float4*>(kbase + (size_t)jc * p.kv_row_stride + d4 * 4);
            float4 vv = *reinterpret_cast<const float4*>(vbase + (size_t)jc * p.kv_row_stride + d4 * 4);
            reinterpret_cast<float4*>(Ks)[i] = kk;
            reinterpret_cast<float4*>(Vs)[i] = vv;
        }
        __syncthreads();
        for (int jj = 0; jj < 64; jj += 4) {
            float sc[4];
#pragma unroll
            for (int kk = 0; kk < 4; kk++) {
                const float* kr = Ks + (jj + kk) * HD + part * DP;
                float s = 0.f;
#pragma unroll
                for (int e = 0; e < DP; e += 4) {
                    const float4 kv = *reinterpret_cast<const float4*>(kr + e);
                    s = fmaf(qv[e], kv.x, s); s = fmaf(qv[e + 1], kv.y, s); s = fmaf(qv[e + 2], kv.z, s); s = fmaf(qv[e + 3], kv.w, s);
                }
                s += __shfl_xor(s, 16, 64); s += __shfl_xor(s, 32, 64);
                const int j = j0 + jj + kk;
                bool vis = (j < p.kv_len) && (j <= pos);
                if (p.window >= 0) vis = vis && (pos - j <= p.window);
                sc[kk] = vis ? s * scale : -INFINITY;
            }
            const float mnew = fmaxf(fmaxf(fmaxf(sc[0], sc[1]), fmaxf(sc[2], sc[3])), mx);
            if (mnew > -INFINITY) {
                const float alpha = expf(mx - mnew);
                float pr[4];
#pragma unroll
                for (int kk = 0; kk < 4; kk++) pr[kk] = expf(sc[kk] - mnew);
                l = l * alpha + ((pr[0] + pr[1]) + (pr[2] + pr[3]));
#pragma unroll
                for (int e = 0; e < DP; e++) o[e] *= alpha;
#pragma unroll
                for (int kk = 0; kk < 4; kk++) {
                    const float* vr = Vs + (jj + kk) * HD + part * DP;
#pragma unroll
                    for (int e = 0; e < DP; e += 4) {
                        const float4 vv = *reinterpret_cast<const float4*>(vr + e);
                        o[e] = fmaf(pr[kk], vv.x, o[e]); o[e + 1] = fmaf(pr[kk], vv.y, o[e + 1]);
                        o[e + 2] = fmaf(pr[kk], vv.z, o[e + 2]); o[e + 3] = fmaf(pr[kk], vv.w, o[e + 3]);
                    }
                }
                mx = mnew;
            }
        }
    }
    if (q_ok) {
        float* op = p.out + (size_t)m * p.out_stride + h * HD + part * DP;
// ... 29 lines not shown
    const int mq = min(m, M - 1);
    const int pos = p.offset + mq;
    const int wave_pos_hi = p.offset + min(m0 + wave * 16 + 15, M - 1);
    const float scale = 1.0f / sqrtf((float)HD);

    bf16x8 qh[KS], ql[KS];
    {
        const float* qp = p.q + (p.seq_row_off ? (size_t)p.seq_row_off[sq] * p.q_stride : (size_t)sq * p.q_seq_stride) + (size_t)mq * p.q_stride + h * HD + 8 * g;
#pragma unroll
        for (int ks = 0; ks < KS; ks++) {
            const float4 a = *reinterpret_cast<const float4*>(qp + ks * 32), b = *reinterpret_cast<const float4*>(qp + ks * 32 + 4);
            uint4 hi, lo; split_bf16x8(a, b, hi, lo); qh[ks] = as_bf16x8(hi); ql[ks] = as_bf16x8(lo);
        }
    }
    f32x4 o[DT];
#pragma unroll
    for (int dt = 0; dt < DT; dt++) o[dt] = (f32x4){0.f, 0.f, 0.f, 0.f};
    float mx = -INFINITY, lsum = 0.f;

    const int last_m = min(m0 + 63, M - 1);
    int j_lo = 0;
    if (p.window >= 0) j_lo = max(0, p.offset + m0 - p.window);
    const int j_hi = min(kv_len - 1, p.offset + last_m);
    const size_t kvso = p.seq_row_off ? (size_t)p.seq_row_off[sq] * p.kv_row_stride : (size_t)sq * p.kv_seq_stride;
    const float* kbase = p.k + kvso + (size_t)kvh * p.kv_head_stride;
    const float* vbase = p.v + kvso + (size_t)kvh * p.kv_head_stride;
    const int n_pfx = PFX ? p.prefix_len : 0;
    const float* pkbase = PFX ? p.prefix_k + (size_t)kvh * p.prefix_head_stride : nullptr;
    const float* pvbase = PFX ? p.prefix_v + (size_t)kvh * p.prefix_head_stride : nullptr;
#define VOX_ATT_ROW(BASE_, PBASE_, J_) \
    ((PFX && (J_) < n_pfx) ? (PBASE_) + (size_t)(J_) * p.prefix_row_stride : (BASE_) + (size_t)((J_) - n_pfx) * p.kv_row_stride)

    constexpr int NK = (64 * (HD / 4)) / 256, NV = (32 * (HD / 4)) / 256;
    float4 kreg[NK], vra[NV], vrb[NV];
#define VOX_ATT_LOAD(J0_)                                                                                           \
    _Pragma("unroll") for (int u = 0; u < NK; u++) {                                                                \
        const int i = tid + 256 * u, key = i / (HD / 4), d4 = i % (HD / 4);                                         \
        const int jc = min((J0_) + key, kv_len - 1);      \
        kreg[u] = *reinterpret_cast<const float4*>(VOX_ATT_ROW(kbase, pkbase, jc) + d4 * 4);                        \
    }                                                                                                               \
    _Pragma("unroll") for (int u = 0; u < NV; u++) {                                                                \
        const int i = tid + 256 * u, kp = i / (HD / 4), d4 = i % (HD / 4);                                          \
        const int ja = min((J0_) + 2 * kp, kv_len - 1), jb = min((J0_) + 2 * kp + 1, kv_len - 1);               \
        vra[u] = *reinterpret_cast<const float4*>(VOX_ATT_ROW(vbase, pvbase, ja) + d4 * 4);                         \
        vrb[u] = *reinterpret_cast<const float4*>(VOX_ATT_ROW(vbase, pvbase, jb) + d4 * 4);                         \
    }
    const int j_first = (j_lo / 64) * 64, j_last = (j_hi / 64) * 64;
    VOX_ATT_LOAD(j_first)
    for (int j0 = j_first; j0 <= j_hi; j0 += 64) {
        __syncthreads();
#pragma unroll
        for (int u = 0; u < NK; u++) {
            const int i = tid + 256 * u, key = i / (HD / 4), d4 = i % (HD / 4);
            uint2 hi, lo; split_pair(kreg[u].x, kreg[u].y, hi.x, lo.x); split_pair(kreg[u].z, kreg[u].w, hi.y, lo.y);
            *reinterpret_cast<uint2*>(Kh + key * KROW + d4 * 4) = hi;
            *reinterpret_cast<uint2*>(Kl + key * KROW + d4 * 4) = lo;
        }
#pragma unroll
        for (int u = 0; u < NV; u++) {
            const int i = tid + 256 * u, kp = i / (HD / 4), d4 = i % (HD / 4);
            const float4 va = vra[u], vb = vrb[u];
            uint32_t hi, lo;
            split_pair(va.x, vb.x, hi, lo); *reinterpret_cast<uint32_t*>(Vh + (d4 * 4 + 0) * VROW + 2 * kp) = hi; *reinterpret_cast<uint32_t*>(Vl + (d4 * 4 + 0) * VROW + 2 * kp) = lo;
            split_pair(va.y, vb.y, hi, lo); *reinterpret_cast<uint32_t*>(Vh + (d4 * 4 + 1) * VROW + 2 * kp) = hi; *reinterpret_cast<uint32_t*>(Vl + (d4 * 4 + 1) * VROW + 2 * kp) = lo;
            split_pair(va.z, vb.z, hi, lo); *reinterpret_cast<uint32_t*>(Vh + (d4 * 4 + 2) * VROW + 2 * kp) = hi; *reinterpret_cast<uint32_t*>(Vl + (d4 * 4 + 2) * VROW + 2 * kp) = lo;
            split_pair(va.w, vb.w, hi, lo); *reinterpret_cast<uint32_t*>(Vh + (d4 * 4 + 3) * VROW + 2 * kp) = hi; *reinterpret_cast<uint32_t*>(Vl + (d4 * 4 + 3) * VROW + 2 * kp) = lo;
        }
        __syncthreads();
        { const int jn = min(j0 + 64, j_last); VOX_ATT_LOAD(jn) }
        __builtin_amdgcn_sched_barrier(0);
        if (j0 > wave_pos_hi) continue;

        f32x4 sc[4];
#pragma unroll
        for (int kt = 0; kt < 4; kt++) {
            sc[kt] = (f32x4){0.f, 0.f, 0.f, 0.f};
            if (j0 + kt * 16 <= wave_pos_hi) {
#pragma unroll
                for (int ks = 0; ks < KS; ks++) {
                    const bf16x8 ah = as_bf16x8(*reinterpret_cast<const uint4*>(Kh + (kt * 16 + c) * KROW + ks * 32 + 8 * g));
                    const bf16x8 al = as_bf16x8(*reinterpret_cast<const uint4*>(Kl + (kt * 16 + c) * KROW + ks * 32 + 8 * g));
                    sc[kt] = __builtin_amdgcn_mfma_f32_16x16x32_bf16(ah, qh[ks], sc[kt], 0, 0, 0);
                    sc[kt] = __builtin_amdgcn_mfma_f32_16x16x32_bf16(ah, ql[ks], sc[kt], 0, 0, 0);
                    sc[kt] = __builtin_amdgcn_mfma_f32_16x16x32_bf16(al, qh[ks], sc[kt], 0, 0, 0);
                }
            }
        }
        float mt = -INFINITY;
#pragma unroll
        for (int kt = 0; kt < 4; kt++)
#pragma unroll
            for (int r = 0; r < 4; r++) {
                const int j = j0 + kt * 16 + 4 * g + r;
                bool vis = (j < kv_len) && (j <= pos);
                if (p.window >= 0) vis = vis && (pos - j <= p.window);
                const float v = vis ? sc[kt][r] * scale : -INFINITY;
                sc[kt][r] = v; mt = fmaxf(mt, v);
            }
        mt = fmaxf(mt, __shfl_xor(mt, 16, 64)); mt = fmaxf(mt, __shfl_xor(mt, 32, 64));
        const float mnew = fmaxf(mx, mt);
        const float msafe = (mnew == -INFINITY) ? 0.f : mnew;
        const float alpha = __expf(mx - msafe);
        float ps = 0.f;
#pragma unroll
        for (int kt = 0; kt < 4; kt++)
#pragma unroll
            for (int r = 0; r < 4; r++) { const float e = __expf(sc[kt][r] - msafe); sc[kt][r] = e; ps += e; }
        lsum = lsum * alpha + ps; mx = mnew;
#pragma unroll
        for (int dt = 0; dt < DT; dt++) { o[dt][0] *= alpha; o[dt][1] *= alpha; o[dt][2] *= alpha; o[dt][3] *= alpha; }
#pragma unroll
        for (int kk = 0; kk < 2; kk++) {
            if (j0 + kk * 32 <= wave_pos_hi) {
                uint4 ph, pl;
                split_pair(sc[2 * kk][0], sc[2 * kk][1], ph.x, pl.x); split_pair(sc[2 * kk][2], sc[2 * kk][3], ph.y, pl.y);
                split_pair(sc[2 * kk + 1][0], sc[2 * kk + 1][1], ph.z, pl.z); split_pair(sc[2 * kk + 1][2], sc[2 * kk + 1][3], ph.w, pl.w);
                const bf16x8 bh = as_bf16x8(ph), bl = as_bf16x8(pl);
#pragma unroll
                for (int dt = 0; dt < DT; dt++) {
                    const uint16_t* vh = Vh + (dt * 16 + c) * VROW + kk * 32 + 4 * g;
                    const uint16_t* vl = Vl + (dt * 16 + c) * VROW + kk * 32 + 4 * g;
                    const uint2 h0 = *reinterpret_cast<const uint2*>(vh), h1 = *reinterpret_cast<const uint2*>(vh + 16);
                    const uint2 l0 = *reinterpret_cast<const uint2*>(vl), l1 = *reinterpret_cast<const uint2*>(vl + 16);
                    const bf16x8 ah = as_bf16x8(make_uint4(h0.x, h0.y, h1.x, h1.y)), al = as_bf16x8(make_uint4(l0.x, l0.y, l1.x, l1.y));
                    o[dt] = __builtin_amdgcn_mfma_f32_16x16x32_bf16(ah, bh, o[dt], 0, 0, 0);
                    o[dt] = __builtin_amdgcn_mfma_f32_16x16x32_bf16(ah, bl, o[dt], 0, 0, 0);
                    o[dt] = __builtin_amdgcn_mfma_f32_16x16x32_bf16(al, bh, o[dt], 0, 0, 0);
                }
            }
        }
    }
#undef VOX_ATT_LOAD
#undef VOX_ATT_ROW
    lsum += __shfl_xor(lsum, 16, 64); lsum += __shfl_xor(lsum, 32, 64);
    if (m < M) {
        const float inv = 1.0f / lsum;
        float* op = p.out + (p.seq_row_off ? (size_t)p.seq_row_off[sq] * p.out_stride : (size_t)sq * p.out_seq_stride) + (size_t)m * p.out_stride + h * HD + 4 * g;
#pragma unroll
        for (int dt = 0; dt < DT; dt++)
            *reinterpret_cast<float4*>(op + dt * 16) = make_float4(o[dt][0] * inv, o[dt][1] * inv, o[dt][2] * inv, o[dt][3] * inv);
    }
}
template <int HD, bool PFX>
static hipError_t attn_prefill_mfma_launch(const AttnParams& p, hipStream_t s, int n_seq) {
    constexpr size_t lds = ((size_t)2 * 64 * (HD + 8) + (size_t)2 * HD * 72) * sizeof(uint16_t);
    auto kern = attn_prefill_mfma_kernel<HD, PFX>;
    static DevOnce attr_done;
    hipError_t e = ensure_dyn_lds(kern, lds, &attr_done);
    if (e != hipSuccess) return e;
    kern<<<dim3((p.M + 63) / 64, p.n_heads, n_seq), dim3(256), lds, s>>>(p);
    attn_form_note(ATTN_FORM_PREFILL_MFMA);
    return hipGetLastError();
}
template <int HD>
__global__ __launch_bounds__(256) void attn_prefill_small_kernel(const AttnParams p) {
    constexpr int KROW = HD + 4, MAXR = 48;
    extern __shared__ __attribute__((aligned(16))) float sms[];
    float* Ks = sms; float* Vs = Ks + MAXR * KROW; float* Qs = Vs + MAXR * HD; float* Ps = Qs + 4 * HD;
    const int tid = threadIdx.x, lane = tid & 63, wave = tid >> 6;
    const int h = blockIdx.x, sq = blockIdx.y, kvh = h / (p.n_heads / p.n_kv_heads);
    const int M = p.seq_len ? p.seq_len[sq] : p.M;
    const int r = 4 * (int)blockIdx.z + wave;
    const int n_keys = min(M, 4 * (int)blockIdx.z + 4);
    if (4 * (int)blockIdx.z >= M) {
        if (p.out_xf_tiles && lane < 32) xf_store4(p.out_xf_tiles + (size_t)(r >> 4) * p.out_xf_tile_stride, p.n_heads * HD, r & 15, h * HD + 4 * lane, make_float4(0.f, 0.f, 0.f, 0.f));
        return;
    }
    const size_t kvso = (size_t)sq * p.kv_seq_stride;
    const float* kbase = p.k + kvso + (size_t)kvh * p.kv_head_stride; const float* vbase = p.v + kvso + (size_t)kvh * p.kv_head_stride;
    for (int i = tid; i < n_keys * (HD / 4); i += 256) {
        const int j = i / (HD / 4), d4 = i % (HD / 4);
        *reinterpret_cast<float4*>(Ks + j * KROW + 4 * d4) = *reinterpret_cast<const float4*>(kbase + (size_t)j * p.kv_row_stride + 4 * d4);
        *reinterpret_cast<float4*>(Vs + j * HD + 4 * d4) = *reinterpret_cast<const float4*>(vbase + (size_t)j * p.kv_row_stride + 4 * d4);
    }
    float* qs = Qs + wave * HD; float* ps = Ps + wave * 64;
    if (r < M) { const float* qp = p.q + (size_t)sq * p.q_seq_stride + (size_t)r * p.q_stride + h * HD; for (int d = lane; d < HD; d += 64) qs[d] = qp[d]; }
    __syncthreads();
    const float scale = 1.0f / sqrtf((float)HD);
    float4 o = make_float4(0.f, 0.f, 0.f, 0.f);
    if (r < M) {
        const float* kr = Ks + min(lane, n_keys - 1) * KROW;
        float s0 = 0.f, s1 = 0.f, s2 = 0.f, s3 = 0.f;
#pragma unroll 8
        for (int d = 0; d < HD; d += 4) {
            const float4 kv = *reinterpret_cast<const float4*>(kr + d), qv = *reinterpret_cast<const float4*>(qs + d);
            s0 = fmaf(qv.x, kv.x, s0); s1 = fmaf(qv.y, kv.y, s1); s2 = fmaf(qv.z, kv.z, s2); s3 = fmaf(qv.w, kv.w, s3);
        }
        const bool vis = lane <= r && (p.window < 0 || r - lane <= p.window);
        const float sc = vis ? ((s0 + s1) + (s2 + s3)) * scale : -INFINITY;
        const float mx = wave_max(sc);
        const float e = vis ? expf(sc - mx) : 0.f;
        const float sum = wave_sum(e);
        ps[lane] = e / sum;
        __builtin_amdgcn_wave_barrier();
        const int c = lane & 31, half = lane >> 5;
        for (int j = half; j <= r; j += 2) {
            const float pj = ps[j]; const float4 vv = *reinterpret_cast<const float4*>(Vs + j * HD + 4 * c);
            o.x = fmaf(pj, vv.x, o.x); o.y = fmaf(pj, vv.y, o.y); o.z = fmaf(pj, vv.z, o.z); o.w = fmaf(pj, vv.w, o.w);
        }
        o.x += __shfl_xor(o.x, 32, 64); o.y += __shfl_xor(o.y, 32, 64); o.z += __shfl_xor(o.z, 32, 64); o.w += __shfl_xor(o.w, 32, 64);
    }
    if (lane < 32) {
        const int col = h * HD + 4 * lane;
        if (p.out_xf_tiles) xf_store4(p.out_xf_tiles + (size_t)(r >> 4) * p.out_xf_tile_stride, p.n_heads * HD, r & 15, col, o);
        else if (r < M) *reinterpret_cast<float4*>(p.out + (size_t)sq * p.out_seq_stride + (size_t)r * p.out_stride + col) = o;
    }
}
bool attn_prefill_small_ok(const AttnParams& p, int hd, int n_seq) {
    return hd == 128 && p.M >= 1 && p.M <= 48 && p.offset == 0 && p.kv_len == p.M && !p.seq_row_off && (p.window < 0 || p.window >= p.M) && (p.q_stride % 4) == 0 && (p.kv_row_stride % 4) == 0 &&
           n_seq == 1  &&
           !env_int("VOX_ATTN_F32");
}
static hipError_t attn_prefill_small_launch(const AttnParams& p, hipStream_t s, int n_seq) {
    constexpr int HD = 128;
    const size_t lds = (size_t)(48 * (HD + 4) + 48 * HD + 4 * HD + 4 * 64) * sizeof(float);
    auto kern = attn_prefill_small_kernel<HD>; static DevOnce done;
    hipError_t e = ensure_dyn_lds(kern, lds, &done); if (e != hipSuccess) return e;
    const int rows = p.out_xf_tiles ? ((p.M + 15) / 16) * 16 : p.M;
    kern<<<dim3(p.n_heads, n_seq, (rows + 3) / 4), dim3(256), lds, s>>>(p);
    attn_form_note(ATTN_FORM_PREFILL_SMALL);
    return hipGetLastError();
}
bool attn_prefill_prefix_ok(const AttnParams& p, int hd, int n_seq) {
    return (hd == 64 || hd == 128) && n_seq == 1 && !p.seq_len && !p.seq_row_off && !p.out_xf_tiles && p.prefix_k && p.prefix_v && p.prefix_len > 0 && p.offset == p.prefix_len &&
           p.M >= 1 && p.kv_len == p.prefix_len + p.M && (p.q_stride % 4) == 0 && (p.kv_row_stride % 4) == 0 && (p.prefix_row_stride % 4) == 0 && (p.prefix_head_stride % 4) == 0 &&
           !env_int("VOX_ATTN_F32");
}
hipError_t launch_attn_prefill(const AttnParams& p, int hd, hipStream_t s, int n_seq) {
    if (attn_prefill_small_ok(p, hd, n_seq)) return attn_prefill_small_launch(p, s, n_seq);
    if (p.out_xf_tiles) return hipErrorInvalidValue;
    const int f32_only = env_int("VOX_ATTN_F32");
    if (p.prefix_len > 0) {
        if (!attn_prefill_prefix_ok(p, hd, n_seq)) return hipErrorInvalidValue;
        return hd == 64 ? attn_prefill_mfma_launch<64, true>(p, s, 1) : attn_prefill_mfma_launch<128, true>(p, s, 1);
    }
    if (!f32_only && (p.q_stride % 4) == 0 && (p.kv_row_stride % 4) == 0) {
        if (hd == 64) return attn_prefill_mfma_launch<64, false>(p, s, n_seq);
        if (hd == 128) return attn_prefill_mfma_launch<128, false>(p, s, n_seq);
    }
    if (n_seq != 1 || p.seq_len) return hipErrorInvalidValue;
    dim3 grid((p.M + 63) / 64, p.n_heads);
    const size_t lds = (size_t)2 * 64 * hd * sizeof(float);
    if (hd == 64) {
        attn_prefill_kernel<64><<<grid, dim3(256), lds, s>>>(p);
    } else if (hd == 128) {
        auto kern = attn_prefill_kernel<128>;
        static DevOnce attr_done;
        hipError_t e = ensure_dyn_lds(kern, lds, &attr_done);
        if (e != hipSuccess) return e;
        kern<<<grid, dim3(256), lds, s>>>(p);
    } else return hipErrorInvalidValue;
    attn_form_note(ATTN_FORM_PREFILL_F32);
    return hipGetLastError();
}

template <bool NT>
__device__ __forceinline__ float4 ldf4(const float* p) {
    if (NT) { const u32x4_t v = __builtin_nontemporal_load(reinterpret_cast<const u32x4_t*>(p)); return make_float4(__uint_as_float(v.x), __uint_as_float(v.y), __uint_as_float(v.z), __uint_as_float(v.w)); }
    return *reinterpret_cast<const float4*>(p);
}
template <int HD, bool NT, bool LATE_V, bool SPEC, class Hook>
__device__ __forceinline__ float4 attn_decode_core(const float* __restrict__ qh, const float* __restrict__ kb, const float* __restrict__ vb, int kv_row_stride,
                                                   int pos_in, int window, float* __restrict__ sc, float* __restrict__ red, float4* __restrict__ osum, int tl_slot, int tlw,
                                                   int spec_rows, Hook after_issue) {
    static_assert(HD == 128 || HD == 64, "head_dim");
    constexpr int PER = HD / 8;
    const int tid = threadIdx.x, lane = tid & 63, wave = tid >> 6;
    const float scale = 1.0f / sqrtf((float)HD);
    const int ks = tid >> 3, part = tid & 7;
    (void)tl_slot; (void)tlw;
    float qv[PER];
#pragma unroll
    for (int e = 0; e < PER; e += 4) {
        const float4 v = ldf4<NT>(qh + part * PER + e);
        qv[e] = v.x; qv[e + 1] = v.y; qv[e + 2] = v.z; qv[e + 3] = v.w;
    }
    constexpr int NPRE = LATE_V ? 4 : 5, COLS = HD / 4, GROUPS = 256 / COLS;
    static_assert(4 * GROUPS == 32 || HD != 128, "prefetch tiling assumes 32 keys per P.V iteration for HD = 128");
    const int grp = tid / COLS, col = tid % COLS;
    float4 kpre[NPRE][PER / 4], vpre[NPRE][4];
#define VOX_KPRE(ROW_)                                                                                        \
    _Pragma("unroll") for (int u = 0; u < NPRE; u++) {                                                        \
        const int jc = (ROW_);                                                                                \
        const float* kr = kb + (size_t)jc * kv_row_stride + part * PER;                                       \
        _Pragma("unroll") for (int e = 0; e < PER / 4; e++) kpre[u][e] = ldf4<NT>(kr + 4 * e);                \
    }
#define VOX_VPRE_AT(ROW_)                                                                                     \
    _Pragma("unroll") for (int u = 0; u < NPRE; u++)                                                          \
        _Pragma("unroll") for (int w = 0; w < 4; w++) {                                                       \
            const int iv = u * 4 * GROUPS + grp + w * GROUPS;                                                 \
            vpre[u][w] = ldf4<NT>(vb + (size_t)(ROW_) * kv_row_stride + col * 4);                             \
        }
#define VOX_VPRE VOX_VPRE_AT(j_lo + min(iv, n - 1))
    static_assert(!SPEC || !LATE_V, "speculative rows: K and V are both requested up front");
    if (SPEC) {
        VOX_KPRE(min(32 * u + ks, spec_rows - 1))
        VOX_VPRE_AT(min(iv, spec_rows - 1))
        __builtin_amdgcn_sched_barrier(0);
    }
    const int pos = SPEC ? __builtin_amdgcn_readfirstlane(pos_in) : pos_in;
    const int len = pos + 1;
    const int j_lo = window >= 0 ? max(0, pos - window) : 0;
    const int n = len - j_lo;
    if (SPEC) {
        if (j_lo != 0) {
            VOX_KPRE(j_lo + min(32 * u + ks, n - 1))
            VOX_VPRE
        }
    } else {
        VOX_KPRE(j_lo + min(32 * u + ks, n - 1))
        if (!LATE_V) { VOX_VPRE }
    }
    __builtin_amdgcn_sched_barrier(0);
    after_issue();
    __builtin_amdgcn_sched_barrier(0);
#undef VOX_KPRE
#pragma unroll
    for (int u = 0; u < NPRE; u++) {
        float s = 0.f;
#pragma unroll
        for (int e = 0; e < PER / 4; e++) {
            const float4 kv = kpre[u][e];
            s = fmaf(qv[4 * e], kv.x, s); s = fmaf(qv[4 * e + 1], kv.y, s); s = fmaf(qv[4 * e + 2], kv.z, s); s = fmaf(qv[4 * e + 3], kv.w, s);
        }
        s = group8_sum(s);
        const int i = 32 * u + ks;
        if (part == 0 && i < n) sc[i] = s * scale;
    }
    if (LATE_V) { VOX_VPRE }
#undef VOX_VPRE
#undef VOX_VPRE_AT
    for (int i0 = 32 * NPRE; i0 < n; i0 += 64) {
        float s2[2];
#pragma unroll
        for (int u = 0; u < 2; u++) {
            const int i = i0 + 32 * u + ks, jc = j_lo + min(i, n - 1);
            const float* kr = kb + (size_t)jc * kv_row_stride + part * PER;
            float s = 0.f;
#pragma unroll
            for (int e = 0; e < PER; e += 4) {
                const float4 kv = ldf4<NT>(kr + e);
                s = fmaf(qv[e], kv.x, s); s = fmaf(qv[e + 1], kv.y, s); s = fmaf(qv[e + 2], kv.z, s); s = fmaf(qv[e + 3], kv.w, s);
            }
            s2[u] = s;
        }
#pragma unroll
        for (int u = 0; u < 2; u++) {
            const float s = group8_sum(s2[u]);
            const int i = i0 + 32 * u + ks;
            if (part == 0 && i < n) sc[i] = s * scale;
        }
    }
    __syncthreads();
    VOX_TL(tl_slot, tlw, 1);
    float mx = -INFINITY;
    for (int i = tid; i < n; i += 256) mx = fmaxf(mx, sc[i]);
    mx = wave_max(mx);
    if (lane == 0) red[wave] = mx;
    __syncthreads();
    mx = fmaxf(fmaxf(red[0], red[1]), fmaxf(red[2], red[3]));
    float sum = 0.f;
    for (int i = tid; i < n; i += 256) { const float e = expf(sc[i] - mx); sc[i] = e; sum += e; }
    sum = wave_sum(sum);
    if (lane == 0) red[4 + wave] = sum;
    __syncthreads();
    VOX_TL(tl_slot, tlw, 2);
    sum = (red[4] + red[5]) + (red[6] + red[7]);
    float4 o = make_float4(0.f, 0.f, 0.f, 0.f);
    if (4 * GROUPS == 32) {
#pragma unroll
        for (int u = 0; u < NPRE; u++)
#pragma unroll
            for (int w = 0; w < 4; w++) {
                const int i = u * 32 + grp + w * GROUPS;
                const float pr = i < n ? sc[min(i, n - 1)] : 0.f;
                float4 vv = vpre[u][w];
                if (SPEC && i >= n) vv = make_float4(0.f, 0.f, 0.f, 0.f);
                o.x = fmaf(pr, vv.x, o.x); o.y = fmaf(pr, vv.y, o.y); o.z = fmaf(pr, vv.z, o.z); o.w = fmaf(pr, vv.w, o.w);
            }
    }
    for (int i0 = (4 * GROUPS == 32 ? 32 * NPRE : 0) + grp; i0 < n; i0 += 4 * GROUPS) {
        float4 vv[4]; float pr[4];
#pragma unroll
        for (int u = 0; u < 4; u++) {
            const int i = i0 + u * GROUPS, ic = min(i, n - 1);
            vv[u] = ldf4<NT>(vb + (size_t)(j_lo + ic) * kv_row_stride + col * 4);
            pr[u] = i < n ? sc[ic] : 0.f;
        }
// ... 1050 lines not shown
```

Before: 1499.

## Add split-KV prefill attention, occupancy-planned encoder split-K, and per-row sumk norm

Adds a prefill attention kernel for head_dim 64 that splits the key range across two wave groups and merges their softmax partials in LDS. It is used for single-clip encoder attention with a prefix when there are fewer query blocks than CUs. The encoder split-K factor for w2 and wo is now chosen from measured tile occupancy, and the workspace is sized for the larger of the two. A one-row-per-block rms_norm_sumk kernel is added for small row counts to raise parallelism. These target the streaming encoder, so their effect on decode throughput is indirect, and they add kernel complexity and extra merge work.

```diff
diff --git a/include/voxtral_hip.h b/include/voxtral_hip.h
--- a/include/voxtral_hip.h
+++ b/include/voxtral_hip.h
@@ -176,7 +176,10 @@
 
 int32_t vox_debug_reload_knobs(void);
 int32_t vox_debug_attn_launches(uint64_t* out, int32_t cap);
+int32_t vox_debug_attention_prefix(vox_ctx* ctx, const float* q, const float* k, const float* v, int32_t M, const float* prefix_k, const float* prefix_v, int32_t prefix_len,
+                                   int32_t n_heads, int32_t head_dim, int32_t window, int32_t split2, float* out);
 int32_t vox_debug_gemm_launches(uint64_t* out, int32_t cap);
+int32_t vox_debug_rms_norm_sumk(vox_ctx* ctx, float* x, int32_t rows, int32_t dim, const float* planes, int32_t ks, const float* gamma, float eps, float* out, int32_t form);
 int32_t vox_debug_occupy(vox_ctx* ctx, int32_t workgroups, int32_t micros);
 
 int32_t vox_bench_decode_gemv(vox_model* m, int32_t which, int32_t iters, double* avg_us, double* bytes_per_launch,
diff --git a/voxtral-mini-realtime-rs_amd/_lib.py b/voxtral-mini-realtime-rs_amd/_lib.py
--- a/voxtral-mini-realtime-rs_amd/_lib.py
+++ b/voxtral-mini-realtime-rs_amd/_lib.py
@@ -142,6 +142,8 @@
     "vox_bench_wide": (i32, [vp, i32, i32, i32, P(C.c_double)]),
     "vox_debug_attn_launches": (i32, [P(C.c_uint64), i32]),
     "vox_debug_gemm_launches": (i32, [P(C.c_uint64), i32]),
+    "vox_debug_attention_prefix": (i32, [vp, vp, vp, vp, i32, vp, vp, i32, i32, i32, i32, i32, vp]),
+    "vox_debug_rms_norm_sumk": (i32, [vp, vp, i32, i32, vp, i32, vp, f32, vp, i32]),
     "vox_debug_timeline_start": (i32, [vp, i32, i32]),
     "vox_debug_timeline_fetch": (i32, [vp, vp, sz, P(i32), vp]),
     "vox_debug_batch_tap_arm": (i32, [vp, P(i32), i32, i32]),
diff --git a/voxtral-mini-realtime-rs_amd/csrc/vox_api.cpp b/voxtral-mini-realtime-rs_amd/csrc/vox_api.cpp
--- a/voxtral-mini-realtime-rs_amd/csrc/vox_api.cpp
+++ b/voxtral-mini-realtime-rs_amd/csrc/vox_api.cpp
@@ -1327,6 +1327,15 @@
 }
 static int enc_packed_rows_of(const vox_model* m, int T) { const int R = m->cfg.reshape_factor; return std::max((enc_rows(T) + R - 1) / R * R, R * 40); }
 static long enc_packed_rows(const vox_model* m, const int* T, int n) { long r = 0; for (int i = 0; i < n; i++) r += enc_packed_rows_of(m, T[i]); return r; }
+static int enc_plan_slices(int rows, int N, int nq, int resident) {
+    const long base = (long)((N + 127) / 128) * ((rows + 31) / 32);
+    int best = 2; long best_cost = -1;
+    for (int ks = 2; ks <= 4 && ks <= nq; ks++) {
+        const long rounds = (base * ks + resident - 1) / resident, cost = rounds * ((nq + ks - 1) / ks);
+        if (best_cost < 0 || cost <= best_cost) { best = ks; best_cost = cost; }
+    }
+    return best;
+}
 struct EncForms { long Mtot = 0; int ksp = 0, ksp_wo = 0, fused_rope = 0; };
 static int32_t encode_batch_dev(vox_model* m, int n, const float* const* d_mels, const int* T, float* audio_out, int audio_rows, int* S4_out, long* audio_off_out = nullptr,
                                 EncForms* forms = nullptr, int prefix_rows = 0) {
@@ -1362,8 +1371,17 @@
     }
     int ksp_wo = ksp ? 2 : 0;
     if (ksp) { if (const char* e = knob_str("VOX_ENC_SPLITK_WO")) ksp_wo = atoi(e) > 1 ? std::min(atoi(e), ksp) : 0; }
+    if (n == 1 && !packed && ksp) {
+        const int resident = q4_gemm_tile_resident(2);
+        if (resident > 0) {
+            if (!knob_str("VOX_ENC_SPLITK")) ksp = enc_plan_slices(Mtot, m->enc[0].w2.w.N, m->enc[0].w2.w.nb / 4, resident);
+            if (ksp_wo && !knob_str("VOX_ENC_SPLITK_WO")) ksp_wo = enc_plan_slices(Mtot, m->enc[0].wo.w.N, m->enc[0].wo.w.nb / 4, resident);
+        }
+    }
+    bool attn_split2 = n == 1 && !packed && prefix_rows > 0 && (long)((Mtot + 63) / 64) * H < device_cu_count();
+    if (const char* e = knob_str("VOX_ENC_ATTN_SPLIT2")) attn_split2 = n == 1 && !packed && atoi(e) != 0;
     for (int l = 0; ksp_wo && l < c.enc_layers; l++) if (m->enc[l].wo.w.fmt != WFMT_Q4_0 || !m->enc[l].wo.w.qt || m->enc[l].wo.w.nb / 4 < ksp_wo || m->enc[l].wo.w.nb % 4) ksp_wo = 0;
-    const size_t need = c1_floats + (size_t)Mfull * D + (size_t)Mtot * D + (size_t)Mtot * QD * 4 + (size_t)Mtot * F + (size_t)(M4 + 1) * m->ad0.w.N + (size_t)ksp * Mtot * D + 1024;
+    const size_t need = c1_floats + (size_t)Mfull * D + (size_t)Mtot * D + (size_t)Mtot * QD * 4 + (size_t)Mtot * F + (size_t)(M4 + 1) * m->ad0.w.N + (size_t)std::max(ksp, ksp_wo) * Mtot * D + 1024;
     VOXCHK(ensure(&m->ws, &m->ws_floats, need));
     if (forms) { forms->Mtot = Mtot; forms->ksp = ksp; forms->ksp_wo = ksp_wo; forms->fused_rope = 0; }
     float* c1 = m->ws; float* x0 = c1 + c1_floats / 64 * 64; float* x = x0 + (size_t)r0 * D; float* xn = x0 + (size_t)Mfull * D; float* qkv = xn + (size_t)Mtot * D;
@@ -1412,6 +1430,7 @@
         AttnParams ap{}; ap.q = qkv; ap.q_stride = 3 * QD; ap.k = qkv + QD; ap.v = qkv + 2 * QD; ap.kv_row_stride = 3 * QD; ap.kv_head_stride = hd;
         ap.out = att; ap.out_stride = QD; ap.M = S_pad - r0; ap.kv_len = S_pad; ap.n_heads = H; ap.n_kv_heads = H; ap.offset = r0; ap.window = c.enc_window;
         if (r0) { ap.prefix_k = m->pfx.enc_kv + (size_t)l * r0 * 2 * QD; ap.prefix_v = ap.prefix_k + QD; ap.prefix_len = r0; ap.prefix_row_stride = 2 * QD; ap.prefix_head_stride = hd; }
+        ap.split2 = attn_split2 ? 1 : 0;
         ap.seq_len = d_len; ap.q_seq_stride = S_pad * 3 * QD; ap.out_seq_stride = S_pad * QD; ap.kv_seq_stride = (long)S_pad * 3 * QD; ap.seq_row_off = d_roff;
         HIPCHK(launch_attn_prefill(ap, hd, s, n));
         if (ksp_wo) {
@@ -3481,6 +3500,36 @@
     return VOX_OK;
 }
 
+extern "C" int32_t vox_debug_rms_norm_sumk(vox_ctx* c, float* x, int32_t rows, int32_t dim, const float* planes, int32_t ks, const float* gamma, float eps, float* out, int32_t form) {
+    ARGCHK(c && x && planes && gamma && out, "null argument"); ARGCHK(rows > 0 && dim > 0 && dim % 4 == 0 && dim <= 4096 && ks >= 1 && form >= 0 && form <= 2, "bad shape or form"); VOXCHK(ctx_bind(c));
+    const size_t nx = (size_t)rows * dim * 4;
+    DevBuf dx, dp, dg, dy; HIPCHK(dx.alloc(nx)); HIPCHK(dp.alloc(nx * ks)); HIPCHK(dg.alloc((size_t)dim * 4)); HIPCHK(dy.alloc(nx));
+    HIPCHK(hipMemcpyAsync(dx.p, x, nx, hipMemcpyHostToDevice, c->stream)); HIPCHK(hipMemcpyAsync(dp.p, planes, nx * ks, hipMemcpyHostToDevice, c->stream));
+    HIPCHK(hipMemcpyAsync(dg.p, gamma, (size_t)dim * 4, hipMemcpyHostToDevice, c->stream));
+    HIPCHK(launch_rms_norm_sumk(dx.as<float>(), dim, rows, dim, dp.as<float>(), (size_t)rows * dim, ks, dg.as<float>(), eps, dy.as<float>(), dim, c->stream, form));
+    HIPCHK(hipMemcpyAsync(x, dx.p, nx, hipMemcpyDeviceToHost, c->stream)); HIPCHK(hipMemcpyAsync(out, dy.p, nx, hipMemcpyDeviceToHost, c->stream));
+    HIPCHK(hipStreamSynchronize(c->stream));
+    return VOX_OK;
+}
+extern "C" int32_t vox_debug_attention_prefix(vox_ctx* c, const float* q, const float* k, const float* v, int32_t M, const float* prefix_k, const float* prefix_v, int32_t prefix_len,
+                                              int32_t n_heads, int32_t head_dim, int32_t window, int32_t split2, float* out) {
+    ARGCHK(c && q && k && v && out && M > 0 && n_heads > 0 && prefix_len >= 0 && (prefix_len == 0 || (prefix_k && prefix_v)), "bad argument");
+    ARGCHK(head_dim == 64 || head_dim == 128, "head_dim must be 64 or 128"); VOXCHK(ctx_bind(c));
+    const size_t row = (size_t)n_heads * head_dim * 4, qn = (size_t)M * row, pn = (size_t)prefix_len * row;
+    DevBuf dq, dk, dv, dpk, dpv, dout;
+    HIPCHK(dq.alloc(qn)); HIPCHK(dk.alloc(qn)); HIPCHK(dv.alloc(qn)); HIPCHK(dout.alloc(qn)); HIPCHK(dpk.alloc(pn)); HIPCHK(dpv.alloc(pn));
+    HIPCHK(hipMemcpyAsync(dq.p, q, qn, hipMemcpyHostToDevice, c->stream)); HIPCHK(hipMemcpyAsync(dk.p, k, qn, hipMemcpyHostToDevice, c->stream));
+    HIPCHK(hipMemcpyAsync(dv.p, v, qn, hipMemcpyHostToDevice, c->stream));
+    if (prefix_len) { HIPCHK(hipMemcpyAsync(dpk.p, prefix_k, pn, hipMemcpyHostToDevice, c->stream)); HIPCHK(hipMemcpyAsync(dpv.p, prefix_v, pn, hipMemcpyHostToDevice, c->stream)); }
+    const int QD = n_heads * head_dim;
+    AttnParams ap{}; ap.q = dq.as<float>(); ap.q_stride = QD; ap.k = dk.as<float>(); ap.v = dv.as<float>(); ap.kv_row_stride = QD; ap.kv_head_stride = head_dim;
+    ap.out = dout.as<float>(); ap.out_stride = QD; ap.M = M; ap.kv_len = prefix_len + M; ap.n_heads = n_heads; ap.n_kv_heads = n_heads; ap.offset = prefix_len; ap.window = window;
+    if (prefix_len) { ap.prefix_k = dpk.as<float>(); ap.prefix_v = dpv.as<float>(); ap.prefix_len = prefix_len; ap.prefix_row_stride = QD; ap.prefix_head_stride = head_dim; }
+    ap.split2 = split2 ? 1 : 0;
+    HIPCHK(launch_attn_prefill(ap, head_dim, c->stream));
+    HIPCHK(hipMemcpyAsync(out, dout.p, qn, hipMemcpyDeviceToHost, c->stream)); HIPCHK(hipStreamSynchronize(c->stream));
+    return VOX_OK;
+}
 extern "C" int32_t vox_debug_encode_batch(vox_model* m, int32_t n, const float* const* mels, const int32_t* T, int32_t layout, float* out, int64_t cap_rows,
                                           int32_t* rows_per_clip, int64_t* report) {
     ARGCHK(m, "null model");
diff --git a/voxtral-mini-realtime-rs_amd/csrc/vox_kernels.h b/voxtral-mini-realtime-rs_amd/csrc/vox_kernels.h
--- a/voxtral-mini-realtime-rs_amd/csrc/vox_kernels.h
+++ b/voxtral-mini-realtime-rs_amd/csrc/vox_kernels.h
@@ -72,6 +72,8 @@
 bool q4_wide_plan(const Q4W& w, int mt, int epi, WidePlan* pl);
 size_t q4_wide_planes_bytes(const Q4W& w, int mt, const WidePlan& pl);
 hipError_t launch_q4_wide(const GemmParams& p, int epi, hipStream_t s);
+int q4_gemm_tile_resident(int nt);
+int device_cu_count();
 hipError_t launch_q4_tile_build(Q4W w, uint4* qt, uint16_t* st, hipStream_t s);
 hipError_t launch_q4_gemm(const GemmParams& p, int epi, hipStream_t s, bool* fused_rope = nullptr);
 hipError_t launch_dense2_gemm(const GemmParams& p, int epi, hipStream_t s);
@@ -82,7 +84,8 @@
 hipError_t launch_q4_dequant(Q4W w, float* out, hipStream_t s);
 hipError_t launch_rms_norm(const float* x, int x_stride, int rows, int dim, const float* gamma, const float* mul,
                            float eps, float* out, int out_stride, hipStream_t s);
-hipError_t launch_rms_norm_sumk(float* x, int x_stride, int rows, int dim, const float* part, size_t part_stride, int ksplit, const float* gamma, float eps, float* out, int out_stride, hipStream_t s);
+hipError_t launch_rms_norm_sumk(float* x, int x_stride, int rows, int dim, const float* part, size_t part_stride, int ksplit, const float* gamma, float eps, float* out, int out_stride, hipStream_t s,
+                                int form = 0);
 int q4_skinny_mt2_plan(const Q4W& w, int M);
 hipError_t launch_xf_rows(const float* x, int x_stride, int M, int K, uint16_t* xf, hipStream_t s);
 hipError_t launch_q4_skinny_mt2_planes(const GemmParams& p, int KZ, hipStream_t s);
@@ -118,6 +121,7 @@
     int spec_zero;
     int spec_rows;
     const float* prefix_k; const float* prefix_v; int prefix_len, prefix_row_stride, prefix_head_stride;
+    int split2;
 };
 hipError_t launch_attn_prefill(const AttnParams& p, int hd, hipStream_t s, int n_seq = 1);
 bool attn_prefill_prefix_ok(const AttnParams& p, int hd, int n_seq);
@@ -126,12 +130,14 @@
 bool attn_wo_supported(const AttnParams& p, const Q4W& wo, int hd, int max_seq);
 hipError_t launch_attn_wo(const AttnParams& p, const Q4W& wo, long long* acc, int max_seq, hipStream_t s);
 enum AttnForm { ATTN_FORM_PREFILL_SMALL, ATTN_FORM_PREFILL_MFMA, ATTN_FORM_PREFILL_F32, ATTN_FORM_DECODE, ATTN_FORM_DECODE_SPEC, ATTN_FORM_DECODE_GQA, ATTN_FORM_WO,
-                ATTN_FORM_ENGINE, ATTN_FORM_STREAM_RING, ATTN_FORM_COUNT };
+                ATTN_FORM_ENGINE, ATTN_FORM_STREAM_RING, ATTN_FORM_PREFILL_SPLIT2, ATTN_FORM_COUNT };
 void attn_form_note(AttnForm f);
 void attn_form_counts(unsigned long long out[ATTN_FORM_COUNT]);
 enum GemmForm { GEMM_FORM_GEMV_R1, GEMM_FORM_GEMV_R2, GEMM_FORM_GEMV_R4, GEMM_FORM_DENSE_GEMV, GEMM_FORM_SKINNY, GEMM_FORM_SKINNY_MT, GEMM_FORM_SKINNY_MT2, GEMM_FORM_XF_ROWS,
                 GEMM_FORM_SPLITK_FINISH, GEMM_FORM_TILE_11, GEMM_FORM_TILE_12, GEMM_FORM_TILE_21, GEMM_FORM_TILE_22, GEMM_FORM_TILE_21_TB, GEMM_FORM_TILE_22_TB, GEMM_FORM_K32,
-                GEMM_FORM_BIG, GEMM_FORM_BIG_ROPE, GEMM_FORM_DENSE2, GEMM_FORM_WIDE, GEMM_FORM_COUNT };
+                GEMM_FORM_BIG, GEMM_FORM_BIG_ROPE, GEMM_FORM_DENSE2, GEMM_FORM_WIDE,
+                GEMM_FORM_SUMK_WAVE, GEMM_FORM_SUMK_ROW,
+                GEMM_FORM_COUNT };
 void gemm_form_counts(unsigned long long out[GEMM_FORM_COUNT]);
 
 hipError_t launch_conv1d_gelu(const float* in, int Cin, int L, const float* w, const float* b, int Cout, float* out,
diff --git a/voxtral-mini-realtime-rs_amd/csrc/vox_kernels.hip b/voxtral-mini-realtime-rs_amd/csrc/vox_kernels.hip
--- a/voxtral-mini-realtime-rs_amd/csrc/vox_kernels.hip
+++ b/voxtral-mini-realtime-rs_amd/csrc/vox_kernels.hip
@@ -2202,6 +2202,25 @@
 #undef VOX_MN
     return hipErrorInvalidValue;
 }
+int device_cu_count() {
+    int dev = 0, cus = 0;
+    if (hipGetDevice(&dev) != hipSuccess || hipDeviceGetAttribute(&cus, hipDeviceAttributeMultiprocessorCount, dev) != hipSuccess) { (void)hipGetLastError(); return 0; }
+    return cus;
+}
+int q4_gemm_tile_resident(int nt) {
+    static std::atomic<int> cached[2];
+    if (nt != 1 && nt != 2) return 0;
+    int r = cached[nt - 1].load(std::memory_order_relaxed);
+    if (r > 0) return r;
+    int per_cu = 0;
+    const int cus = device_cu_count();
+    const size_t lds = (size_t)2 * 2 * 4 * 2 * 64 * sizeof(uint4);
+    const hipError_t e = nt == 2 ? hipOccupancyMaxActiveBlocksPerMultiprocessor(&per_cu, q4_gemm_kernel<2, 2, EPI_STORE, WFMT_Q4_0, 1>, 256, lds)
+                                 : hipOccupancyMaxActiveBlocksPerMultiprocessor(&per_cu, q4_gemm_kernel<2, 1, EPI_STORE, WFMT_Q4_0, 1>, 256, lds);
+    if (e != hipSuccess || per_cu <= 0 || cus <= 0) return 0;
+    r = per_cu * cus; cached[nt - 1].store(r, std::memory_order_relaxed);
+    return r;
+}
 hipError_t launch_rope(float* buf, int M, int stride, int n_rot, int hd, int pos_off, const float* cos_t, const float* sin_t, hipStream_t s, int seq_rows, const int* row_pos);
 static hipError_t launch_q4_gemm_epi(const GemmParams& p, int epi, hipStream_t s, bool* fused_rope);
 hipError_t launch_q4_gemm(const GemmParams& p, int epi, hipStream_t s, bool* fused_rope) {
@@ -2341,9 +2360,44 @@
         if (c < n4) { const float4 g = g4[c]; o[c] = make_float4((v[i].x / rms) * g.x, (v[i].y / rms) * g.y, (v[i].z / rms) * g.z, (v[i].w / rms) * g.w); }
     }
 }
-hipError_t launch_rms_norm_sumk(float* x, int x_stride, int rows, int dim, const float* part, size_t part_stride, int ksplit, const float* gamma, float eps, float* out, int out_stride, hipStream_t s) {
-    if (dim % 4 || dim > 4096 || rows <= 0 || ksplit < 1) return hipErrorInvalidValue;
-    rms_norm_sumk_kernel<<<dim3((rows + 3) / 4), dim3(256), 0, s>>>(x, x_stride, rows, dim, part, part_stride, ksplit, gamma, eps, out, out_stride);
+__global__ __launch_bounds__(256) VOX_NO_PK_F32 void rms_norm_sumk_row_kernel(float* __restrict__ x, int x_stride, int dim, const float* __restrict__ part, size_t part_stride, int ks,
+                                                                const float* __restrict__ gamma, float eps, float* __restrict__ out, int out_stride) {
+    __shared__ float sq[16][64];
+    const int row = blockIdx.x, wave = threadIdx.x >> 6, lane = threadIdx.x & 63;
+    float4* xr = reinterpret_cast<float4*>(x + (size_t)row * x_stride);
+    const int n4 = dim >> 2;
+    float4 v[4];
+#pragma unroll
+    for (int j = 0; j < 4; j++) {
+        const int c = threadIdx.x + 256 * j;
+        if (c < n4) {
+            float4 a = xr[c];
+            plane_sum_add(a, reinterpret_cast<const float4*>(part + (size_t)row * dim) + c, part_stride >> 2, ks);
+            v[j] = a; xr[c] = a;
+            sq[wave + 4 * j][lane] = (a.x * a.x + a.y * a.y) + (a.z * a.z + a.w * a.w);
+        } else v[j] = make_float4(0.f, 0.f, 0.f, 0.f);
+    }
+    __syncthreads();
+    float ss = 0.f;
+#pragma unroll
+    for (int i = 0; i < 16; i++) if (lane + 64 * i < n4) ss += sq[i][lane];
+    ss = wave_sum(ss);
+    const float rms = sqrtf(ss / (float)dim + eps);
+    float4* o = reinterpret_cast<float4*>(out + (size_t)row * out_stride);
+    const float4* g4 = reinterpret_cast<const float4*>(gamma);
+#pragma unroll
+    for (int j = 0; j < 4; j++) {
+        const int c = threadIdx.x + 256 * j;
+        if (c < n4) { const float4 g = g4[c]; o[c] = make_float4((v[j].x / rms) * g.x, (v[j].y / rms) * g.y, (v[j].z / rms) * g.z, (v[j].w / rms) * g.w); }
+    }
+}
+hipError_t launch_rms_norm_sumk(float* x, int x_stride, int rows, int dim, const float* part, size_t part_stride, int ksplit, const float* gamma, float eps, float* out, int out_stride, hipStream_t s,
+                                int form) {
+    if (dim % 4 || dim > 4096 || rows <= 0 || ksplit < 1 || form < 0 || form > 2) return hipErrorInvalidValue;
+    const bool per_row = form ? form == 2 : rows < 1024;
+    gemm_form_note(per_row ? GEMM_FORM_SUMK_ROW : GEMM_FORM_SUMK_WAVE);
+    if (per_row) rms_norm_sumk_row_kernel<<<dim3(rows), dim3(256), 0, s>>>(x, x_stride, dim, part, part_stride, ksplit, gamma, eps, out, out_stride);
+    else rms_norm_sumk_kernel<<<dim3((rows + 3) / 4), dim3(256), 0, s>>>(x, x_stride, rows, dim, part, part_stride, ksplit, gamma, eps, out, out_stride);
     return hipGetLastError();
 }
 hipError_t launch_rms_norm_xf_sumk(float* x, int x_stride, int rows, int dim, const float* planes, int kz, const float* gamma, const float* mul, float eps,
@@ -2679,6 +2733,206 @@
     attn_form_note(ATTN_FORM_PREFILL_MFMA);
     return hipGetLastError();
 }
+template <int HD, bool PFX, int QG>
+__global__ __launch_bounds__(128 * QG) __attribute__((amdgpu_waves_per_eu(2))) void attn_prefill_mfma_split2_kernel(const AttnParams p) {
+    constexpr int KS = HD / 32, DT = HD / 16, KROW = HD + 8, VROW = 72;
+    constexpr int TILE = 2 * 64 * KROW + 2 * HD * VROW;
+    extern __shared__ __attribute__((aligned(16))) uint16_t smh[];
+    const int tid = threadIdx.x, lane = tid & 63, wave = tid >> 6, c = lane & 15, g = lane >> 4;
+    const int qg = wave % QG, kpar = wave / QG;
+    constexpr int NT = 128 * QG, QB = 16 * QG;
+    int bx = blockIdx.x, h = blockIdx.y;
+    {
+        const int nblk = gridDim.x, pairs = gridDim.y;
+        if (nblk > 1 && pairs % 8 == 0) {
+            const int lin = blockIdx.y * nblk + blockIdx.x, xcd = lin & 7, slot = lin >> 3;
+            h = xcd * (pairs >> 3) + slot / nblk; bx = slot % nblk;
+        }
+    }
+    const int kvh = h / (p.n_heads / p.n_kv_heads);
+    const int M = p.M, kv_len = p.kv_len;
+    const int m0 = ((int)gridDim.x - 1 - bx) * QB;
+    const int m = m0 + qg * 16 + c;
+    const int mq = min(m, M - 1);
+    const int pos = p.offset + mq;
+    const int wave_pos_hi = p.offset + min(m0 + qg * 16 + 15, M - 1);
+    const float scale = 1.0f / sqrtf((float)HD);
+
+    bf16x8 qh[KS], ql[KS];
+    {
+        const float* qp = p.q + (size_t)mq * p.q_stride + h * HD + 8 * g;
+#pragma unroll
+        for (int ks = 0; ks < KS; ks++) {
+            const float4 a = *reinterpret_cast<const float4*>(qp + ks * 32), b = *reinterpret_cast<const float4*>(qp + ks * 32 + 4);
+            uint4 hi, lo; split_bf16x8(a, b, hi, lo); qh[ks] = as_bf16x8(hi); ql[ks] = as_bf16x8(lo);
+        }
+    }
+    f32x4 o[DT];
+#pragma unroll
+    for (int dt = 0; dt < DT; dt++) o[dt] = (f32x4){0.f, 0.f, 0.f, 0.f};
+    float mx = -INFINITY, lsum = 0.f;
+
+    const int last_m = min(m0 + QB - 1, M - 1);
+    int j_lo = 0;
+    if (p.window >= 0) j_lo = max(0, p.offset + m0 - p.window);
+    const int j_hi = min(kv_len - 1, p.offset + last_m);
+    const float* kbase = p.k + (size_t)kvh * p.kv_head_stride;
+    const float* vbase = p.v + (size_t)kvh * p.kv_head_stride;
+    const int n_pfx = PFX ? p.prefix_len : 0;
+    const float* pkbase = PFX ? p.prefix_k + (size_t)kvh * p.prefix_head_stride : nullptr;
+    const float* pvbase = PFX ? p.prefix_v + (size_t)kvh * p.prefix_head_stride : nullptr;
+#define VOX_ATT_ROW(BASE_, PBASE_, J_) \
+    ((PFX && (J_) < n_pfx) ? (PBASE_) + (size_t)(J_) * p.prefix_row_stride : (BASE_) + (size_t)((J_) - n_pfx) * p.kv_row_stride)
+
+    constexpr int NK = (128 * (HD / 4)) / NT, NV = (64 * (HD / 4)) / NT;
+    float4 kreg[NK], vra[NV], vrb[NV];
+#define VOX_ATT_LOAD(J0_)                                                                                           \
+    _Pragma("unroll") for (int u = 0; u < NK; u++) {                                                                \
+        const int i = tid + NT * u, key = i / (HD / 4), d4 = i % (HD / 4);                                         \
+        const int jc = min((J0_) + key, kv_len - 1);      \
+        kreg[u] = *reinterpret_cast<const float4*>(VOX_ATT_ROW(kbase, pkbase, jc) + d4 * 4);                        \
+    }                                                                                                               \
+    _Pragma("unroll") for (int u = 0; u < NV; u++) {                                                                \
+        const int i = tid + NT * u, kp = i / (HD / 4), d4 = i % (HD / 4);                                          \
+        const int ja = min((J0_) + 2 * kp, kv_len - 1), jb = min((J0_) + 2 * kp + 1, kv_len - 1);               \
+        vra[u] = *reinterpret_cast<const float4*>(VOX_ATT_ROW(vbase, pvbase, ja) + d4 * 4);                         \
+        vrb[u] = *reinterpret_cast<const float4*>(VOX_ATT_ROW(vbase, pvbase, jb) + d4 * 4);                         \
+    }
+    const int j_first = (j_lo / 64) * 64, j_last = j_first + ((j_hi - j_first) / 128) * 128;
+    const uint16_t* Kh = smh + kpar * TILE;
+    const uint16_t* Kl = Kh + 64 * KROW;
+    const uint16_t* Vh = Kl + 64 * KROW;
+    const uint16_t* Vl = Vh + HD * VROW;
+    VOX_ATT_LOAD(j_first)
+    for (int j0 = j_first; j0 <= j_hi; j0 += 128) {
+        __syncthreads();
+#pragma unroll
+        for (int u = 0; u < NK; u++) {
+            const int i = tid + NT * u, key = i / (HD / 4), d4 = i % (HD / 4);
+            uint16_t* kh = smh + (key >> 6) * TILE + (key & 63) * KROW + d4 * 4;
+            uint2 hi, lo; split_pair(kreg[u].x, kreg[u].y, hi.x, lo.x); split_pair(kreg[u].z, kreg[u].w, hi.y, lo.y);
+            *reinterpret_cast<uint2*>(kh) = hi;
+            *reinterpret_cast<uint2*>(kh + 64 * KROW) = lo;
+        }
+#pragma unroll
+        for (int u = 0; u < NV; u++) {
+            const int i = tid + NT * u, kp = i / (HD / 4), d4 = i % (HD / 4);
+            uint16_t* vh = smh + (kp >> 5) * TILE + 2 * 64 * KROW + (d4 * 4) * VROW + 2 * (kp & 31);
+            uint16_t* vl = vh + HD * VROW;
+            const float4 va = vra[u], vb = vrb[u];
+            uint32_t hi, lo;
+            split_pair(va.x, vb.x, hi, lo); *reinterpret_cast<uint32_t*>(vh + 0 * VROW) = hi; *reinterpret_cast<uint32_t*>(vl + 0 * VROW) = lo;
+            split_pair(va.y, vb.y, hi, lo); *reinterpret_cast<uint32_t*>(vh + 1 * VROW) = hi; *reinterpret_cast<uint32_t*>(vl + 1 * VROW) = lo;
+            split_pair(va.z, vb.z, hi, lo); *reinterpret_cast<uint32_t*>(vh + 2 * VROW) = hi; *reinterpret_cast<uint32_t*>(vl + 2 * VROW) = lo;
+            split_pair(va.w, vb.w, hi, lo); *reinterpret_cast<uint32_t*>(vh + 3 * VROW) = hi; *reinterpret_cast<uint32_t*>(vl + 3 * VROW) = lo;
+        }
+        __syncthreads();
+        { const int jn = min(j0 + 128, j_last); VOX_ATT_LOAD(jn) }
+        __builtin_amdgcn_sched_barrier(0);
+        const int jt = j0 + 64 * kpar;
+        if (jt > wave_pos_hi) continue;
+
+        f32x4 sc[4];
+#pragma unroll
+        for (int kt = 0; kt < 4; kt++) {
+            sc[kt] = (f32x4){0.f, 0.f, 0.f, 0.f};
+            if (jt + kt * 16 <= wave_pos_hi) {
+#pragma unroll
+                for (int ks = 0; ks < KS; ks++) {
+                    const bf16x8 ah = as_bf16x8(*reinterpret_cast<const uint4*>(Kh + (kt * 16 + c) * KROW + ks * 32 + 8 * g));
+                    const bf16x8 al = as_bf16x8(*reinterpret_cast<const uint4*>(Kl + (kt * 16 + c) * KROW + ks * 32 + 8 * g));
+                    sc[kt] = __builtin_amdgcn_mfma_f32_16x16x32_bf16(ah, qh[ks], sc[kt], 0, 0, 0);
+                    sc[kt] = __builtin_amdgcn_mfma_f32_16x16x32_bf16(ah, ql[ks], sc[kt], 0, 0, 0);
+                    sc[kt] = __builtin_amdgcn_mfma_f32_16x16x32_bf16(al, qh[ks], sc[kt], 0, 0, 0);
+                }
+            }
+        }
+        float mt = -INFINITY;
+#pragma unroll
+        for (int kt = 0; kt < 4; kt++)
+#pragma unroll
+            for (int r = 0; r < 4; r++) {
+                const int j = jt + kt * 16 + 4 * g + r;
+                bool vis = (j < kv_len) && (j <= pos);
+                if (p.window >= 0) vis = vis && (pos - j <= p.window);
+                const float v = vis ? sc[kt][r] * scale : -INFINITY;
+                sc[kt][r] = v; mt = fmaxf(mt, v);
+            }
+        mt = fmaxf(mt, __shfl_xor(mt, 16, 64)); mt = fmaxf(mt, __shfl_xor(mt, 32, 64));
+        const float mnew = fmaxf(mx, mt);
+        const float msafe = (mnew == -INFINITY) ? 0.f : mnew;
+        const float alpha = __expf(mx - msafe);
+        float ps = 0.f;
+#pragma unroll
+        for (int kt = 0; kt < 4; kt++)
+#pragma unroll
+            for (int r = 0; r < 4; r++) { const float e = __expf(sc[kt][r] - msafe); sc[kt][r] = e; ps += e; }
+        lsum = lsum * alpha + ps; mx = mnew;
+#pragma unroll
+        for (int dt = 0; dt < DT; dt++) { o[dt][0] *= alpha; o[dt][1] *= alpha; o[dt][2] *= alpha; o[dt][3] *= alpha; }
+#pragma unroll
+        for (int kk = 0; kk < 2; kk++) {
+            if (jt + kk * 32 <= wave_pos_hi) {
+                uint4 ph, pl;
+                split_pair(sc[2 * kk][0], sc[2 * kk][1], ph.x, pl.x); split_pair(sc[2 * kk][2], sc[2 * kk][3], ph.y, pl.y);
+                split_pair(sc[2 * kk + 1][0], sc[2 * kk + 1][1], ph.z, pl.z); split_pair(sc[2 * kk + 1][2], sc[2 * kk + 1][3], ph.w, pl.w);
+                const bf16x8 bh = as_bf16x8(ph), bl = as_bf16x8(pl);
+#pragma unroll
+                for (int dt = 0; dt < DT; dt++) {
+                    const uint16_t* vh = Vh + (dt * 16 + c) * VROW + kk * 32 + 4 * g;
+                    const uint16_t* vl = Vl + (dt * 16 + c) * VROW + kk * 32 + 4 * g;
+                    const uint2 h0 = *reinterpret_cast<const uint2*>(vh), h1 = *reinterpret_cast<const uint2*>(vh + 16);
+                    const uint2 l0 = *reinterpret_cast<const uint2*>(vl), l1 = *reinterpret_cast<const uint2*>(vl + 16);
+                    const bf16x8 ah = as_bf16x8(make_uint4(h0.x, h0.y, h1.x, h1.y)), al = as_bf16x8(make_uint4(l0.x, l0.y, l1.x, l1.y));
+                    o[dt] = __builtin_amdgcn_mfma_f32_16x16x32_bf16(ah, bh, o[dt], 0, 0, 0);
+                    o[dt] = __builtin_amdgcn_mfma_f32_16x16x32_bf16(ah, bl, o[dt], 0, 0, 0);
+                    o[dt] = __builtin_amdgcn_mfma_f32_16x16x32_bf16(al, bh, o[dt], 0, 0, 0);
+                }
+            }
+        }
+    }
+#undef VOX_ATT_LOAD
+#undef VOX_ATT_ROW
+    lsum += __shfl_xor(lsum, 16, 64); lsum += __shfl_xor(lsum, 32, 64);
+    __syncthreads();
+    constexpr int XS = 64 * QG;
+    float* xb = reinterpret_cast<float*>(smh) + qg * 64 + lane;
+    if (kpar == 1) {
+#pragma unroll
+        for (int dt = 0; dt < DT; dt++)
+#pragma unroll
+            for (int r = 0; r < 4; r++) xb[(dt * 4 + r) * XS] = o[dt][r];
+        xb[(4 * DT) * XS] = mx; xb[(4 * DT + 1) * XS] = lsum;
+    }
+    __syncthreads();
+    if (kpar == 0 && m < M) {
+        const float m1 = xb[(4 * DT) * XS], l1 = xb[(4 * DT + 1) * XS];
+        const float mnew = fmaxf(mx, m1);
+        const float msafe = (mnew == -INFINITY) ? 0.f : mnew;
+        const float a0 = __expf(mx - msafe), a1 = __expf(m1 - msafe);
+        const float inv = 1.0f / (lsum * a0 + l1 * a1);
+        float* op = p.out + (size_t)m * p.out_stride + h * HD + 4 * g;
+#pragma unroll
+        for (int dt = 0; dt < DT; dt++)
+            *reinterpret_cast<float4*>(op + dt * 16) = make_float4((o[dt][0] * a0 + xb[(dt * 4 + 0) * XS] * a1) * inv, (o[dt][1] * a0 + xb[(dt * 4 + 1) * XS] * a1) * inv,
+                                                                   (o[dt][2] * a0 + xb[(dt * 4 + 2) * XS] * a1) * inv, (o[dt][3] * a0 + xb[(dt * 4 + 3) * XS] * a1) * inv);
+    }
+}
+static bool attn_prefill_split2_ok(const AttnParams& p, int hd, int n_seq) {
+    return hd == 64 && n_seq == 1 && !p.seq_len && !p.seq_row_off && !p.out_xf_tiles && p.M >= 1 && (p.q_stride % 4) == 0 && (p.kv_row_stride % 4) == 0 && !env_int("VOX_ATTN_F32");
+}
+template <bool PFX>
+static hipError_t attn_prefill_split2_launch(const AttnParams& p, hipStream_t s) {
+    constexpr int HD = 64, QG = 4;
+    constexpr size_t lds = (size_t)2 * ((size_t)2 * 64 * (HD + 8) + (size_t)2 * HD * 72) * sizeof(uint16_t);
+    auto kern = attn_prefill_mfma_split2_kernel<HD, PFX, QG>;
+    static DevOnce attr_done;
+    hipError_t e = ensure_dyn_lds(kern, lds, &attr_done);
+    if (e != hipSuccess) return e;
+    kern<<<dim3((p.M + 16 * QG - 1) / (16 * QG), p.n_heads, 1), dim3(128 * QG), lds, s>>>(p);
+    attn_form_note(ATTN_FORM_PREFILL_MFMA); attn_form_note(ATTN_FORM_PREFILL_SPLIT2);
+    return hipGetLastError();
+}
 template <int HD>
 __global__ __launch_bounds__(256) void attn_prefill_small_kernel(const AttnParams p) {
     constexpr int KROW = HD + 4, MAXR = 48;
@@ -2759,8 +3013,10 @@
     const int f32_only = env_int("VOX_ATTN_F32");
     if (p.prefix_len > 0) {
         if (!attn_prefill_prefix_ok(p, hd, n_seq)) return hipErrorInvalidValue;
+        if (p.split2 && attn_prefill_split2_ok(p, hd, n_seq)) return attn_prefill_split2_launch<true>(p, s);
         return hd == 64 ? attn_prefill_mfma_launch<64, true>(p, s, 1) : attn_prefill_mfma_launch<128, true>(p, s, 1);
     }
+    if (p.split2 && attn_prefill_split2_ok(p, hd, n_seq)) return attn_prefill_split2_launch<false>(p, s);
     if (!f32_only && (p.q_stride % 4) == 0 && (p.kv_row_stride % 4) == 0) {
         if (hd == 64) return attn_prefill_mfma_launch<64, false>(p, s, n_seq);
         if (hd == 128) return attn_prefill_mfma_launch<128, false>(p, s, n_seq);
```

Result: no change. 1511, median of 6 (+0.8%).
